# luigiba/OpenKEonSpark

Hardware: AMD Instinct MI355X
Metric: positive triples/sec (training step) (higher is better)
Workload: dtype f32

## Files before the change

### include/kge_mi355.h

```cpp
#ifndef KGE_MI355_H
#define KGE_MI355_H

#include <stddef.h>
#include <stdint.h>

#ifdef __cplusplus
extern "C" {
#endif

#ifndef INT
#define INT long
#endif
#ifndef REAL
#define REAL float
#endif

void setInPath(char *path);
void setOutPath(char *path);
void setWorkThreads(INT threads);
INT getWorkThreads(void);
void setBern(INT con);
void randReset(void);
void importTrainFiles(void);
INT getEntityTotal(void);
INT getRelationTotal(void);
INT getTripleTotal(void);
INT getTrainTotal(void);
INT getTrainTotal_(void);
INT getBatchTotal(void);
INT getTestTotal(void);
INT getValidTotal(void);
void sampling(INT *batch_h, INT *batch_t, INT *batch_r, REAL *batch_y, INT batchSize, INT negRate, INT negRelRate);

void importTestFiles(void);
void importTypeFiles(void);
void importOntologyFiles(void);
void getHeadBatch(INT index, INT *ph, INT *pt, INT *pr);
void getTailBatch(INT index, INT *ph, INT *pt, INT *pr);
INT *testHead(INT index, REAL *con);
INT *testTail(INT index, REAL *con);
void getTestBatch(INT *ph, INT *pt, INT *pr, INT *nh, INT *nt, INT *nr);
void getValidBatch(INT *ph, INT *pt, INT *pr, INT *nh, INT *nt, INT *nr);
void getBestThreshold(REAL *relThresh, REAL *score_pos, REAL *score_neg);
void test_triple_classification(REAL *relThresh, REAL *score_pos, REAL *score_neg, REAL *acc);
INT get_n_interval(INT r, REAL *score_pos, REAL *score_neg);
INT *get_TPFP(INT r, REAL *score_pos, REAL *score_neg, REAL *threshold, REAL *unused);

enum {
    KGE_OK = 0,
    KGE_NO_EVENT = 1,
    KGE_ERR_NO_DEVICE = -1,
    KGE_ERR_NO_DATASET = -2,
    KGE_ERR_BAD_ARG = -3,
    KGE_ERR_UNSUPPORTED = -4
};

enum { KGE_TRANSE = 0, KGE_TRANSH = 1, KGE_TRANSR = 2, KGE_TRANSD = 3 };

size_t kge_last_error(char *buf, size_t n);
void kge_clear_error(void);
int kge_device_available(void);
const char *kge_version(void);

int kge_set_option(const char *name, INT value);
int kge_last_kernel_ms(const char *name, float *ms);
int kge_kernel_ms_mean(const char *name, float *mean_ms, INT *launches);

int kge_import_train_arrays(INT ent_total, INT rel_total, INT n, const INT *h, const INT *t, const INT *r,
                            INT new_batch_total);

int64_t kge_index_copy(const char *what, void *dst, int64_t bytes);

int kge_get_stream_states(uint64_t *dst, INT n);
int kge_set_stream_states(const uint64_t *src, INT n);

int kge_sampling_device(int32_t *d_h, int32_t *d_t, int32_t *d_r, INT batchSize, INT negRate, INT negRelRate,
                        INT thread_lo, INT thread_hi, INT out_stride, INT *n_local, void *stream);

int kge_sampling_attach(int32_t *d_h, int32_t *d_t, int32_t *d_r, INT batchSize, INT negRate, INT negRelRate,
                        INT thread_lo, INT thread_hi, INT out_stride, INT *n_local, void *stream);
int kge_sampling_flush(void *stream);
INT kge_slice_positions(INT batchSize, INT thread_lo, INT thread_hi, INT *first_position);

typedef struct kge_model_desc {
    int32_t model;
    int32_t negative_rel;
    int64_t ent_total, rel_total;
    int32_t ent_dim, rel_dim;
    float margin;
    int32_t reserved;
} kge_model_desc;

#define KGE_MAX_TABLES 4
int kge_table_shape(const kge_model_desc *m, int table, int64_t *rows, int64_t *cols);

int kge_forward_backward(const kge_model_desc *m, const float *const tables[KGE_MAX_TABLES],
                         const int32_t *d_h, const int32_t *d_t, const int32_t *d_r,
                         INT n_pos, INT n_neg, INT stride, INT denom,
                         float *const grads[KGE_MAX_TABLES], float *d_loss, void *stream);

int kge_stream_wait_emit(void *stream);
int kge_forward_backward_sgd_rows(const kge_model_desc *m, float *const tables[KGE_MAX_TABLES], const int32_t *d_h, const int32_t *d_t,
                                  const int32_t *d_r, INT n_pos, INT n_neg, INT stride, INT denom, float lr, float *d_loss, void *stream);
int kge_sgd_rows_skipped(int32_t *n_negatives);
int kge_forward_backward_records(const kge_model_desc *m, const float *const tables[KGE_MAX_TABLES], const int32_t *d_h, const int32_t *d_t,
                                 const int32_t *d_r, INT n_pos, INT n_neg, INT stride, INT denom, INT n_pos_total, float *d_rec,
                                 int32_t *d_dst, INT rec_offset, INT rec_slice, float *d_loss, void *stream);
int kge_float_records_apply(const kge_model_desc *m, float *const tables[KGE_MAX_TABLES], const float *d_rec, int32_t *d_dst, INT n_records,
                            INT n_pos_total, INT n_neg, float lr, void *stream);
int kge_forward_backward_adam_rows(const kge_model_desc *m, float *const tables[KGE_MAX_TABLES], float *const adam_m[KGE_MAX_TABLES],
                                   float *const adam_v[KGE_MAX_TABLES], const int32_t *d_h, const int32_t *d_t, const int32_t *d_r, INT n_pos,
                                   INT n_neg, INT stride, INT denom, float lr_t, float beta1, float beta2, float eps, float *d_loss, void *stream);
int kge_float_records_apply_adam(const kge_model_desc *m, float *const tables[KGE_MAX_TABLES], float *const adam_m[KGE_MAX_TABLES],
                                 float *const adam_v[KGE_MAX_TABLES], const float *d_rec, int32_t *d_dst, INT n_records, INT n_pos_total,
                                 INT n_neg, float lr_t, float beta1, float beta2, float eps, void *stream);
int kge_pair_path_active(const kge_model_desc *m, INT n_pos, INT n_neg);
int kge_transr_group_layout_active(const kge_model_desc *m, INT n_pos, INT n_neg);

int kge_forward_backward_sampled(const kge_model_desc *m, const float *const tables[KGE_MAX_TABLES],
                                 const int32_t *d_h, const int32_t *d_t, const int32_t *d_r,
                                 INT n_pos, INT n_neg, INT stride, INT denom,
                                 float *const grads[KGE_MAX_TABLES], float *d_loss, void *stream);

int kge_loss_to_limbs(const float *d_loss, int32_t *d_limbs4, void *stream);
int kge_limbs_to_loss(const int32_t *d_limbs4, float *d_out, void *stream);
int kge_loss_limbs_target(int32_t *d_limbs4);

int kge_sgd_update(float *d_p, float *d_g, int64_t n, float lr, void *stream);
int kge_adam_update(float *d_p, float *d_m, float *d_v, float *d_g, int64_t n, float lr_t, float beta1,
                    float beta2, float eps, void *stream);

int kge_sgd_update_tables(int32_t n_tables, float *const d_p[KGE_MAX_TABLES], float *const d_g[KGE_MAX_TABLES],
                          const INT numel[KGE_MAX_TABLES], float lr, void *stream);
int kge_adam_update_tables(int32_t n_tables, float *const d_p[KGE_MAX_TABLES], float *const d_m[KGE_MAX_TABLES],
                           float *const d_v[KGE_MAX_TABLES], float *const d_g[KGE_MAX_TABLES], const INT numel[KGE_MAX_TABLES],
                           float lr_t, float beta1, float beta2, float eps, void *stream);

int kge_transe_counts_supported(const kge_model_desc *m, INT n_neg);
int kge_transe_forward_counts(const kge_model_desc *m, const float *d_ent, const float *d_rel, const int32_t *d_h,
                              const int32_t *d_t, const int32_t *d_r, INT n_pos, INT n_neg, INT stride, INT denom,
                              int32_t *d_counts, float *d_resid_ent, float *d_resid_rel, float *d_loss, void *stream);
int kge_transe_apply_counts(float *d_p, float *d_m, float *d_v, int32_t *d_counts, float *d_resid, int64_t rows, int32_t dim,
                            INT denom, int32_t adam, float lr, float beta1, float beta2, float eps, void *stream);
int kge_transe_train_step_counts(const kge_model_desc *m, float *const d_p[2], float *const d_m[2], float *const d_v[2], const int32_t *d_h,
                                 const int32_t *d_t, const int32_t *d_r, INT n_pos, INT n_neg, INT stride, INT denom, int32_t *d_counts,
                                 float *const d_resid[2], int32_t sampler_shaped, int32_t adam, float lr, float beta1, float beta2, float eps,
                                 float *d_loss, void *stream);
int kge_transe_apply_counts_tables(const kge_model_desc *m, float *const d_p[2], float *const d_m[2], float *const d_v[2],
                                   int32_t *d_counts, float *const d_resid[2], INT denom, int32_t adam, float lr, float beta1,
                                   float beta2, float eps, void *stream);

int kge_transe_apply_counts_range(const kge_model_desc *m, float *const d_p[2], float *const d_m[2], float *const d_v[2],
                                  int32_t *d_counts_chunk, float *const d_resid[2], INT row_lo, INT row_hi, INT denom, int32_t adam,
                                  float lr, float beta1, float beta2, float eps, void *stream);

INT kge_transe_record_dwords(const kge_model_desc *m);
int kge_transe_deferred_groups(int32_t *n_groups);
int kge_transe_step_scratch_read(int which, INT offset, INT count, void *host_out);
int kge_transe_emit_records(const kge_model_desc *m, const float *d_ent, const float *d_rel, const int32_t *d_h, const int32_t *d_t,
                            const int32_t *d_r, INT n_pos, INT n_neg, INT stride, INT denom, uint32_t *d_rec, int32_t *d_dst,
                            float *d_resid_ent, float *d_resid_rel, float *d_loss, void *stream);
int kge_transe_reduce_records(const kge_model_desc *m, const uint32_t *d_rec, int32_t *d_dst, INT n_records, int32_t *d_rows,
                              int32_t *d_row_counts, int32_t *d_n_rows, void *stream);
int kge_transe_apply_rows_sgd(const kge_model_desc *m, float *d_ent, float *d_rel, const int32_t *d_rows, const int32_t *d_row_counts,
                              const int32_t *d_n_rows, INT max_rows, INT denom, float lr, void *stream);
int kge_transe_lazy_row_live(const int32_t *d_row_live);
int kge_transe_apply_rows_adam_lazy(const kge_model_desc *m, float *d_ent, float *d_rel, float *d_m_ent, float *d_m_rel, float *d_v_ent,
                                    float *d_v_rel, const int32_t *d_rows, const int32_t *d_row_counts, const int32_t *d_n_rows,
                                    INT max_rows, INT denom, float lr_t, float beta1, float beta2, float eps, void *stream);
int kge_transe_reduce_apply_records_sgd(const kge_model_desc *m, const uint32_t *d_rec, int32_t *d_dst, INT n_records, float *d_ent,
                                        float *d_rel, int32_t *d_rows, int32_t *d_row_counts, int32_t *d_n_rows, INT denom, float lr,
                                        void *stream);

int kge_shard_requests(const int32_t *d_h, const int32_t *d_t, const int32_t *d_r, INT n_pos, INT n_neg, INT stride, int32_t *d_req,
                       void *stream);
int kge_shard_count(const int32_t *d_ids, INT n, INT chunk, INT n_owners, int32_t *d_counts, void *stream);
int kge_shard_scatter(const int32_t *d_ids, INT n, INT chunk, INT n_owners, const INT *h_counts, int32_t *d_cursor, int32_t *d_sorted,
                      int32_t *d_slot_of, void *stream);
int kge_shard_remap_batch(const int32_t *d_h, const int32_t *d_t, INT n_pos, INT n_neg, INT stride, const int32_t *d_slot_of, int32_t *d_h2,
                          int32_t *d_t2, void *stream);
int kge_shard_gather_rows(const float *d_table, const int32_t *d_ids, INT n, INT row_lo, INT rows, INT dim, float *d_out, void *stream);
int kge_shard_record_ids(const int32_t *d_dst, INT n_records, INT cache_rows, const int32_t *d_cache_ids, int32_t *d_ids, void *stream);
int kge_shard_pack_records(const uint32_t *d_rec, const int32_t *d_slot_of, INT n_records, INT dwords, uint32_t *d_out, void *stream);
int kge_shard_scatter_count_rows(const int32_t *d_rows, const int32_t *d_row_counts, const int32_t *d_n_rows, INT max_rows, INT base,
                                 INT rel_total, INT dim, int32_t *d_image, void *stream);
int kge_shard_relation_counts(const uint32_t *d_rec, const int32_t *d_dst, INT n_records, INT cache_rows, INT rel_total, INT dwords, INT dim,
                              int32_t *d_counts, void *stream);

int kge_train_steps_persistent(const kge_model_desc *m, float *const tables[KGE_MAX_TABLES], float *const grads[KGE_MAX_TABLES],
                               float *const adam_m[KGE_MAX_TABLES], float *const adam_v[KGE_MAX_TABLES], INT batchSize, INT negRate,
                               INT negRelRate, INT n_steps, int32_t adam, const float *h_lr, float beta1, float beta2, float eps,
                               float *d_losses, void *stream);
int kge_persistent_aborted(int32_t *flag);
int kge_persistent_trace(uint64_t *h_out, INT n_steps);

int kge_link_prediction(const kge_model_desc *m, const float *const tables[KGE_MAX_TABLES], INT first, INT count,
                        INT test_head, int64_t *h_out, void *stream);

int kge_link_prediction_range(const kge_model_desc *m, const float *const tables[KGE_MAX_TABLES], INT row_lo, INT rows,
                              const float *d_query_rows, INT first, INT count, INT test_head, int64_t *d_counts, int64_t *d_keys,
                              void *stream);
int kge_link_prediction_finish(INT first, INT count, INT test_head, const int64_t *d_counts, const int64_t *d_keys, int64_t *h_out,
                               void *stream);
int kge_test_entity_ids(INT first, INT count, int32_t *d_ids, void *stream);

int kge_rank_triples(const kge_model_desc *m, const float *const tables[KGE_MAX_TABLES], const int32_t *d_h, const int32_t *d_t,
                     const int32_t *d_r, INT n, INT test_head, int64_t *d_counts, void *stream);

#define KGE_TOPK_FILTERED 1
#define KGE_TOPK_TYPED 2
int kge_topk_entities(const kge_model_desc *m, const float *const tables[KGE_MAX_TABLES], const int32_t *d_fixed, const int32_t *d_rel,
                      const int32_t *d_head, INT n, INT k, INT flags, int32_t *d_ids, float *d_scores, void *stream);
#define KGE_TOPK_NO_KEY 0xFFFFFFFFFFFFFFFFull
int kge_topk_entities_range(const kge_model_desc *m, const float *const tables[KGE_MAX_TABLES], INT row_lo, INT rows,
                            const float *d_query_rows, const int32_t *d_fixed, const int32_t *d_rel, const int32_t *d_head, INT n,
                            INT k, INT flags, uint64_t *d_keys, void *stream);
int kge_topk_merge_keys(const uint64_t *d_keys, INT n, INT parts, INT k, int32_t *d_ids, float *d_scores, void *stream);

int kge_topk_relations(const kge_model_desc *m, const float *const tables[KGE_MAX_TABLES], const int32_t *d_h,
                       const int32_t *d_t, INT n, INT k, INT flags, int32_t *d_ids, float *d_scores, void *stream);
int kge_relation_prediction(const kge_model_desc *m, const float *const tables[KGE_MAX_TABLES], INT first, INT count,
                            int64_t *h_out, void *stream);
int kge_relation_prediction_rows(const kge_model_desc *m, const float *const tables[KGE_MAX_TABLES], const float *d_query_rows,
                                 INT first, INT count, int64_t *d_counts, void *stream);

int kge_tc_fit(const float *d_pos, const float *d_neg, INT n_valid, float *d_thresh, int32_t *d_n_interval, void *stream);
int kge_tc_apply(INT split, const float *d_thresh, const float *d_pos, const float *d_neg, INT n, int64_t *d_counts, int64_t *d_rel,
                 void *stream);

int kge_tc_roc(const float *d_vpos, const float *d_vneg, INT n_valid, INT split, const float *d_pos, const float *d_neg, INT n,
// ... 10 lines not shown
```

### openkeonspark_amd/Config.py

```python
import ctypes
import json
import os

import numpy as np

from . import _lib, shard_eval
from ._lib import KgeError


class Config(object):

    def __init__(self, cpp_lib_path=None, init_new_entities=False):
        self.init_new_entities = init_new_entities
        if init_new_entities == False:
            if cpp_lib_path is None:
                cpp_lib_path = _lib.LIB_PATH
            self.lib = _lib.load(os.path.abspath(cpp_lib_path))
            self.in_path = None
            self.out_path = None
            self.bern = 0
            self.hidden_size = 64
            self.ent_size = self.hidden_size
            self.rel_size = self.hidden_size
            self.train_times = 0
# ... 128 lines not shown

    def set_bern(self, bern):
        self.bern = bern

    def set_dimension(self, dim):
        self.hidden_size = dim
        self.ent_size = dim
        self.rel_size = dim

    def set_ent_dimension(self, dim):
        self.ent_size = dim

    def set_rel_dimension(self, dim):
        self.rel_size = dim

    def set_train_times(self, times):
        self.train_times = times

    def set_nbatches(self, nbatches):
        self.nbatches = nbatches

    def set_margin(self, margin):
        self.margin = margin

    def set_ent_neg_rate(self, rate):
        self.negative_ent = rate

    def set_rel_neg_rate(self, rate):
        self.negative_rel = rate

    def set_import_files(self, path):
        self.importName = path

    def set_export_files(self, path):
        self.exportName = path

    def set_work_threads(self, threads):
        self.workThreads = threads

    def set_model(self, model):
        self.model = model

    def sampling(self):
        self.lib.kge_clear_error()
        self.lib.sampling(self.batch_h_addr, self.batch_t_addr, self.batch_r_addr, self.batch_y_addr,
                          self.batch_size, self.negative_ent, self.negative_rel)
        _lib.raise_if_error(self.lib)

    def set_model_and_session(self, model):
        import torch
        self.model = model
        self._shard_plan = self._plan_entity_shard(model)
        self.trainModel = self.model(config=self, define=True)
        m = self.trainModel
        self._desc = m.descriptor()
        self._tables = [m.parameter_lists[n] for n in m.table_names]
        self._adam = self.opt_method in ("Adam", "adam")
        self._lazy_adam = self.opt_method in ("LazyAdam", "lazyadam", "lazy_adam")
        self._has_slots = self._adam or self._lazy_adam
        n_neg = self.negative_ent + self.negative_rel
        self.use_counts = bool(getattr(self, "use_counts", True)) and bool(
            self.lib.kge_transe_counts_supported(ctypes.byref(self._desc), n_neg))
        requested = getattr(self, "sparse_rows", None)
        table_bytes, sparse = self._wants_sparse_rows(n_neg)
        self.sparse_rows = (bool(sparse) or self._lazy_adam) and self.use_counts and not self._adam
        vector_model = m.model_id in (_lib.TRANSE, _lib.TRANSH, _lib.TRANSD)
        self.sparse_inplace = bool(not self.sparse_rows and vector_model and not self._adam and
                                   (self._lazy_adam or requested or (requested is None and table_bytes > (2 << 30))))
        if self._lazy_adam and not (self.sparse_rows or self.sparse_inplace):
            raise KgeError("LazyAdam (touched rows only, NON-PARITY) needs TransE, TransH or TransD: TransR's gradient is a whole "
                           "matrix per relation and has no record path")
        if requested and not (self.sparse_rows or self.sparse_inplace):
            raise KgeError("sparse_rows needs TransE / TransH / TransD with SGD or LazyAdam")
        self._grads = [] if (self.sparse_rows or self.sparse_inplace) else [torch.zeros_like(t) for t in self._tables]
        if self._has_slots:
            self._adam_m = [torch.zeros_like(t) for t in self._tables]
            self._adam_v = [torch.zeros_like(t) for t in self._tables]
            self._beta1_power = np.float32(self.adam_beta1)
            self._beta2_power = np.float32(self.adam_beta2)
        self._loss = torch.zeros(1, dtype=torch.float32, device=self.device)
        self._refresh_pointers()
        self._dist_ready = 0
        self._dev_batch = None
        self._dev_batch2 = None
        self._side_stream = None
        self._prefetched = None
        self.global_step = 0
        self._sparse_buf = None
        self.counts_min_records = int(getattr(self, "counts_min_records",
                                              os.environ.get("KGE_COUNTS_MIN_RECORDS", 1 << 16)))
        self.prefetch_sampling = getattr(self, "prefetch_sampling", None)
        self._prefetch_auto = self.prefetch_sampling is None
        if self._prefetch_auto:
            self.prefetch_sampling = self._prefetch_default()
        if self.use_counts and not self.sparse_rows:
            self._counts = torch.zeros((self.entTotal + self.relTotal, self.hidden_size), dtype=torch.int32,
                                       device=self.device)
        self._setup_partition()

    def _wants_sparse_rows(self, n_neg):
        table_bytes = (self.entTotal + self.relTotal) * self.hidden_size * 4
        sparse = getattr(self, "sparse_rows", None)
        if sparse is None:
            touched_bytes = self.batch_size * (3 + n_neg) * self.hidden_size * 4
            threshold = getattr(self, "sparse_threshold_bytes", None)
            if threshold is None:
                threshold = max(128 << 20, int(0.3 * touched_bytes))
            sparse = table_bytes > int(threshold)
        return table_bytes, sparse

    def _plan_entity_shard(self, model):
        try:
            import torch.distributed as dist
            if not (dist.is_available() and dist.is_initialized()):
                return None
            W, g = dist.get_world_size(), dist.get_rank()
        except Exception:
            return None
        if W <= 1 or W > 64 or self.hidden_size % 4:
            return None
        probe = model(config=self, define=False)
        if probe.model_id != _lib.TRANSE or self.opt_method in ("Adam", "adam"):
            return None
        n_neg = self.negative_ent + self.negative_rel
        desc = probe.descriptor()
        if not (bool(getattr(self, "use_counts", True)) and bool(self.lib.kge_transe_counts_supported(ctypes.byref(desc), n_neg))):
            return None
        lazy = self.opt_method in ("LazyAdam", "lazyadam", "lazy_adam")
        if not (bool(self._wants_sparse_rows(n_neg)[1]) or lazy):
            return None
        from .parallel import chunk_size
        chunk = chunk_size(self.entTotal, W)
        return dict(world=W, rank=g, chunk=chunk, lo=min(g * chunk, self.entTotal), hi=min((g + 1) * chunk, self.entTotal))

    def init_distributed(self, process_group=None):
        import torch.distributed as dist
        self._pg = process_group
        self.rank = dist.get_rank(process_group)
        self.world_size = dist.get_world_size(process_group)
        if self.trainModel is not None:
            self._setup_partition()
        if getattr(self, "_prefetch_auto", getattr(self, "prefetch_sampling", None) is None):
            self.prefetch_sampling = self._prefetch_default()

    def _prefetch_default(self):
        n_neg = self.negative_ent + self.negative_rel
        counts_path = bool(getattr(self, "use_counts", False)) and not getattr(self, "sparse_rows", False) and \
            self.batch_size * (3 + n_neg) >= int(getattr(self, "counts_min_records", 1 << 16)) * self.world_size
        pair_path = getattr(self, "_desc", None) is not None and \
            bool(self.lib.kge_pair_path_active(ctypes.byref(self._desc), max(self._n_local, 1) if hasattr(self, "_n_local") else self.batch_size, n_neg))
        transr = getattr(self, "trainModel", None) is not None and self.trainModel.model_id == _lib.TRANSR
        dense_one_gpu = not getattr(self, "sparse_rows", False) and not getattr(self, "sparse_inplace", False)
        return bool(self.world_size > 1 or counts_path or pair_path or transr or dense_one_gpu)

    @property
    def _dp(self):
        return self.world_size > 1 or bool(getattr(self, "force_data_parallel", False))

    def _setup_partition(self):
        from .parallel import thread_range
        lo, hi = thread_range(self.rank, self.world_size, self.workThreads)
        self._thread_lo, self._thread_hi = lo, hi
        first = ctypes.c_int64(0)
        self._n_local = self.lib.kge_slice_positions(self.batch_size, lo, hi, ctypes.byref(first))
        self._first_pos = first.value
        if self._dp and self.trainModel is not None and getattr(self, "_dist_ready", 0) != self.world_size:
# ... 48 lines not shown
            self._tables[i] = view
            self.trainModel.parameter_lists[name] = view
            setattr(self.trainModel, name, view)
            self._grads[i] = flat_g[offs[i]:offs[i] + numels[i]].view(shape)
            if self._adam:
                for flat, slots in ((flat_m, self._adam_m), (flat_v, self._adam_v)):
                    v = flat[offs[i]:offs[i] + numels[i]].view(shape)
                    v.copy_(slots[i])
                    slots[i] = v
        self._flat_p, self._flat_g, self._flat_m, self._flat_v = flat_p, flat_g, flat_m, flat_v
        self._chunk = chunk
        self._pieces = K
        seg, own = total // K, chunk // K
        self._piece_seg = [(k * seg, (k + 1) * seg) for k in range(K)]
        self._piece_own = [(k * seg + self.rank * own, k * seg + (self.rank + 1) * own) for k in range(K)]
        self._own_len = own
        self._grads_own = torch.zeros(chunk, dtype=torch.float32, device=dev)
        self._loss_tail = total - 1
        self._loss = flat_p[self._loss_tail:]
        if self.use_counts:
            rows_total = chunk_rows * W
            seg_r, own_r = rows_total // K, chunk_rows // K
            live = self.entTotal + self.relTotal
            self._counts = torch.zeros((rows_total, self.hidden_size), dtype=torch.int32, device=dev)
            self._counts_own = torch.zeros((chunk_rows, self.hidden_size), dtype=torch.int32, device=dev)
            self._piece_rows = [(min(k * seg_r + self.rank * own_r, live), min(k * seg_r + (self.rank + 1) * own_r, live)) for k in range(K)]
            self._own_rows_len = own_r
        self._opt_state_synced = True
        self._refresh_pointers()

    def _setup_shards(self):
        import torch
        from .parallel import chunk_size
        if self.hidden_size % 4:
            raise KgeError("the table-sharded sparse mode needs an embedding width that is a multiple of 4")
        if self.world_size > 64:
            raise KgeError("the table-sharded sparse mode supports up to 64 ranks")
        W, g, E, D = self.world_size, self.rank, self.entTotal, self.hidden_size
        chunk = chunk_size(E, W)
        lo, hi = min(g * chunk, E), min((g + 1) * chunk, E)
        if getattr(self, "_ent_is_shard", False):
            plan = self._shard_plan
            if (plan["world"], plan["rank"], plan["chunk"]) != (W, g, chunk) or self._tables[0].shape[0] != chunk:
                raise KgeError("the entity table was created as the shard of rank %d of %d, the process group has rank %d of %d"
                               % (plan["rank"], plan["world"], g, W))
            self._shard = dict(chunk=chunk, lo=lo, hi=hi)
            self._refresh_pointers()
            return
        full = self._tables[0]
        shard = torch.zeros((chunk, D), dtype=torch.float32, device=full.device)
        if hi > lo:
            shard[:hi - lo].copy_(full[lo:hi])
        self._tables[0] = shard
        self.trainModel.parameter_lists["ent_embeddings"] = shard
        self.trainModel.ent_embeddings = shard
        del full
        if self._lazy_adam:
            for slots in (self._adam_m, self._adam_v):
                old = slots[0]
                slots[0] = torch.zeros((chunk, D), dtype=torch.float32, device=shard.device)
                if hi > lo:
                    slots[0][:hi - lo].copy_(old[lo:hi])
                del old
        torch.cuda.empty_cache()
        self._shard = dict(chunk=chunk, lo=lo, hi=hi)
        self._refresh_pointers()

    def _stream(self):
        import torch
        if getattr(self, "_dev_index_of", None) != self.device:
            d = torch.device(self.device)
            self._dev_index = d.index if d.index is not None else torch.cuda.current_device()
            self._dev_index_of = self.device
        raw = getattr(torch._C, "_cuda_getCurrentRawStream", None)
        return ctypes.c_void_p(raw(self._dev_index) if raw is not None else torch.cuda.current_stream().cuda_stream)

    def _ensure_dev_batch(self, stride):
        import torch
        n = stride * (1 + self.negative_ent + self.negative_rel)
        if self._dev_batch is None or self._dev_batch.shape[2] != n:
            self._dev_batch = torch.zeros((2, 3, n), dtype=torch.int32, device=self.device)
        return self._dev_batch

    def sample_device(self, slot=0):
        stride = max(self._n_local, 1)
        buf = self._ensure_dev_batch(stride)[slot]
        nl = ctypes.c_int64(0)
        _lib.check(self.lib.kge_sampling_device(buf[0].data_ptr(), buf[1].data_ptr(), buf[2].data_ptr(),
                                                self.batch_size, self.negative_ent, self.negative_rel,
                                                self._thread_lo, self._thread_hi, stride, ctypes.byref(nl),
                                                self._stream()), self.lib)
        return buf, nl.value

    def _next_sampled_batch(self):
        import torch
        if self._side_stream is None:
            self._side_stream = torch.cuda.Stream()
            self._slot = 0
            self._prefetched = None
            self.lib.kge_set_option(b"record_emit_event", 1)
        if self._prefetched is None:
            dev, n_pos = self.sample_device(self._slot)
        else:
            dev, n_pos, ev = self._prefetched
            if ev is not None:
                torch.cuda.current_stream().wait_event(ev)
        return dev, n_pos

    def _attach_next_batch(self):
        stride = max(self._n_local, 1)
        self._slot ^= 1
        buf = self._ensure_dev_batch(stride)[self._slot]
        nl = ctypes.c_int64(0)
        _lib.check(self.lib.kge_sampling_attach(buf[0].data_ptr(), buf[1].data_ptr(), buf[2].data_ptr(), self.batch_size,
                                                self.negative_ent, self.negative_rel, self._thread_lo, self._thread_hi, stride,
                                                ctypes.byref(nl), self._stream()), self.lib)
        self._prefetched = (buf, nl.value, None)

    def _flush_next_batch(self):
        _lib.check(self.lib.kge_sampling_flush(self._stream()), self.lib)

    def _prefetch_next_batch(self, behind_emit=False):
        import torch
        main = torch.cuda.current_stream()
        done = None
        if not behind_emit:
            done = torch.cuda.Event()
            done.record(main)
        self._slot ^= 1
        with torch.cuda.stream(self._side_stream):
            if behind_emit:
                rc = _lib.check(self.lib.kge_stream_wait_emit(ctypes.c_void_p(self._side_stream.cuda_stream)), self.lib)
                if rc == _lib.NO_EVENT:
                    done = torch.cuda.Event()
                    done.record(main)
            if done is not None:
                self._side_stream.wait_event(done)
            dev, n_pos = self.sample_device(self._slot)
            ev = torch.cuda.Event()
            ev.record(self._side_stream)
        self._prefetched = (dev, n_pos, ev)

    def forward_backward(self, dev_batch, n_pos, stride, denom, sampler_shaped=False):
        fn = self.lib.kge_forward_backward_sampled if sampler_shaped else self.lib.kge_forward_backward
        _lib.check(fn(ctypes.byref(self._desc), self._tab_ptrs,
                                                 dev_batch[0].data_ptr(), dev_batch[1].data_ptr(),
                                                 dev_batch[2].data_ptr(), n_pos,
                                                 self.negative_ent + self.negative_rel, stride, denom,
                                                 self._grad_ptrs, self._loss.data_ptr(), self._stream()), self.lib)

    def _adam_lr_t(self):
        f = np.float32
        return f(f(self.alpha) * np.sqrt(f(1) - self._beta2_power, dtype=np.float32) / (f(1) - self._beta1_power))

    def _adam_advance(self):
        f = np.float32
        self._beta1_power = f(self._beta1_power * f(self.adam_beta1))
        self._beta2_power = f(self._beta2_power * f(self.adam_beta2))

    def apply_gradients(self, own=False, piece=0):
        st = self._stream()
        if own:
            lo, hi = self._piece_own[piece]
            n = hi - lo
            if hi > self._loss_tail:
                n -= 4
            p, g = self._flat_p.data_ptr() + 4 * lo, self._grads_own.data_ptr() + 4 * piece * self._own_len
            if self._adam:
                _lib.check(self.lib.kge_adam_update(p, self._flat_m.data_ptr() + 4 * lo, self._flat_v.data_ptr() + 4 * lo, g, n,
                                                    float(self._adam_lr_t()), self.adam_beta1, self.adam_beta2,
                                                    self.adam_epsilon, st), self.lib)
                self._opt_state_synced = False
            else:
                _lib.check(self.lib.kge_sgd_update(p, g, n, float(self.alpha), st), self.lib)
            return
        elif self._adam:
            _lib.check(self.lib.kge_adam_update_tables(len(self._tables), self._tab_ptrs, self._adam_m_ptrs, self._adam_v_ptrs,
                                                       self._grad_ptrs, self._numel, float(self._adam_lr_t()), self.adam_beta1,
                                                       self.adam_beta2, self.adam_epsilon, st), self.lib)
            self._adam_advance()
        else:
            _lib.check(self.lib.kge_sgd_update_tables(len(self._tables), self._tab_ptrs, self._grad_ptrs, self._numel,
                                                      float(self.alpha), st), self.lib)
        self.global_step += 1

    def _dp_exchange(self, image, own_image, apply_piece, counts):
        from .parallel import reduce_scatter_sum, all_gather_chunks
        st, W, K = self._stream(), self.world_size, self._pieces
        flat_img, flat_own = image.view(-1), own_image.view(-1)
        per_seg, per_own = flat_img.numel() // K, flat_own.numel() // K
        ride = flat_img.numel() >= 4 and (not counts or self.hidden_size >= 4)
        last = self.rank == W - 1
        nat = self._stream_rccl() if (K == 1 and ride) else None
        self.comm_fence("nat" if nat is not None else "pg")
        if nat is not None:
            if counts and not getattr(self, "_limbs_from_emit", False):
                _lib.check(self.lib.kge_loss_to_limbs(self._loss.data_ptr(), flat_img[flat_img.numel() - self.hidden_size:].data_ptr(), st), self.lib)
            elif not counts:
                flat_img[-1:].copy_(self._loss)
            nat.reduce_scatter_sum(flat_own, flat_img, st)
            if last:
                if counts:
                    _lib.check(self.lib.kge_limbs_to_loss(flat_own[flat_own.numel() - self.hidden_size:].data_ptr(), self._loss.data_ptr(), st), self.lib)
                else:
                    self._loss.copy_(flat_own[-1:])
            apply_piece(0)
            (slo, shi), (lo, hi) = self._piece_seg[0], self._piece_own[0]
            nat.all_gather_chunks(self._flat_p[slo:shi], self._flat_p[lo:hi], st)
            image.zero_()
            if self._adam:
                self._adam_advance()
            self.global_step += 1
            return
        if ride:
            if counts and not getattr(self, "_limbs_from_emit", False):
                _lib.check(self.lib.kge_loss_to_limbs(self._loss.data_ptr(), flat_img[flat_img.numel() - self.hidden_size:].data_ptr(), st), self.lib)
            else:
                flat_img[-1:].copy_(self._loss)
        rs = [reduce_scatter_sum(flat_own[k * per_own:(k + 1) * per_own], flat_img[k * per_seg:(k + 1) * per_seg], self._pg, async_op=True)
              for k in range(K)]
        if not ride:
            from .parallel import allreduce_sum
            allreduce_sum([self._loss], self._pg)
        ag = []
        for k in range(K):
            if rs[k] is not None:
                rs[k].wait()
            if ride and last and k == K - 1:
                if counts:
                    _lib.check(self.lib.kge_limbs_to_loss(flat_own[flat_own.numel() - self.hidden_size:].data_ptr(),
                                                          self._flat_p[self._loss_tail:].data_ptr(), st), self.lib)
                else:
                    self._loss.copy_(flat_own[-1:])
            apply_piece(k)
            (slo, shi), (lo, hi) = self._piece_seg[k], self._piece_own[k]
            ag.append(all_gather_chunks(self._flat_p[slo:shi], self._flat_p[lo:hi], self._pg, async_op=True))
        image.zero_()
        if self._adam:
            self._adam_advance()
        self.global_step += 1
        for w in ag:
            if w is not None:
                w.wait()

    def comm_fence(self, kind):
        last = getattr(self, "_last_comm", None)
        if last is not None and last != kind:
            import torch
            torch.cuda.synchronize(self.device)
        self._last_comm = kind

    def _stream_rccl(self):
        if getattr(self, "_nat_rccl", None) is None:
            import torch.distributed as dist
            want = getattr(self, "stream_rccl", os.environ.get("KGE_STREAM_RCCL", "1") != "0") and dist.is_initialized() and \
                dist.get_backend(self._pg) == "nccl"
            nat = False
            if want:
                import sys
                import torch
                from .parallel import StreamRccl
                self.comm_fence("pg")
                good = 0
                try:
                    nat = StreamRccl(self._pg)
                    torch.cuda.synchronize(self.device)
                    W, g, st = nat.world, nat.rank, self._stream()
                    src = torch.arange(4 * W, dtype=torch.int32, device=self.device) + g
                    own = torch.empty(4, dtype=torch.int32, device=self.device)
                    nat.reduce_scatter_sum(own, src, st)
                    full = torch.empty(4 * W, dtype=torch.int32, device=self.device)
                    full[4 * g:4 * g + 4] = own
                    nat.all_gather_chunks(full, full[4 * g:4 * g + 4], st)
                    torch.cuda.synchronize(self.device)
                    want_full = W * torch.arange(4 * W, dtype=torch.int32) + W * (W - 1) // 2
                    good = int(torch.equal(full.cpu(), want_full))
                    if not good:
                        print("StreamRccl probe gave wrong sums: collectives stay on the process group's stream", file=sys.stderr)
                except Exception as exc:
                    print("StreamRccl unavailable (%s): collectives stay on the process group's stream" % exc, file=sys.stderr)
                ok = torch.tensor([good], dtype=torch.int32, device=self.device)
                dist.all_reduce(ok, op=dist.ReduceOp.MIN, group=self._pg)
                if int(ok.item()) == 0:
                    if nat:
                        nat.close()
                    nat = False
            self._nat_rccl = nat
        return self._nat_rccl or None

    def sync_optimizer_state(self):
        if self._dp and self._adam and not self.sparse_rows and not getattr(self, "_opt_state_synced", True):
            from .parallel import all_gather_chunks
            self.comm_fence("pg")
            for (slo, shi), (lo, hi) in zip(self._piece_seg, self._piece_own):
                all_gather_chunks(self._flat_m[slo:shi], self._flat_m[lo:hi], self._pg)
                all_gather_chunks(self._flat_v[slo:shi], self._flat_v[lo:hi], self._pg)
            self._opt_state_synced = True

    def train_step(self, batch_h=None, batch_t=None, batch_r=None, batch_y=None, sync=True):
        import torch
        n_neg = self.negative_ent + self.negative_rel
        if getattr(self, "_ent_is_shard", False) and not hasattr(self, "_shard"):
            raise KgeError("the entity table was created as this rank's shard of a row-sharded table (the process belongs to a "
                           "torch.distributed world): call init_distributed() before training")
        if batch_h is None:
            dev, n_pos = self._next_sampled_batch() if self.prefetch_sampling else self.sample_device()
            stride = max(self._n_local, 1)
        else:
            if self._dp:
                raise KgeError("feeding a host batch is single-process only")
            host = np.stack([np.asarray(batch_h), np.asarray(batch_t), np.asarray(batch_r)]).astype(np.int32)
            self._check_ids(host)
            dev = torch.from_numpy(host).to(self.device)
            n_pos = host.shape[1] // (1 + n_neg)
            stride = n_pos
        denom = self.batch_size * n_neg if batch_h is None else n_pos * n_neg
        big = (self.batch_size if batch_h is None else n_pos) * (3 + n_neg) >= self.counts_min_records * self.world_size
        if self.sparse_inplace and self._dp:
            self._records_step(dev, n_pos, stride, denom)
            if batch_h is None and self.prefetch_sampling:
                self._prefetch_next_batch()
        elif self.sparse_inplace:
            if self._lazy_adam:
                _lib.check(self.lib.kge_forward_backward_adam_rows(
                    ctypes.byref(self._desc), self._tab_ptrs, self._adam_m_ptrs, self._adam_v_ptrs, dev[0].data_ptr(), dev[1].data_ptr(),
                    dev[2].data_ptr(), n_pos, n_neg, stride, denom, float(self._adam_lr_t()), self.adam_beta1, self.adam_beta2,
                    self.adam_epsilon, self._loss.data_ptr(), self._stream()), self.lib)
                self._adam_advance()
            else:
                _lib.check(self.lib.kge_forward_backward_sgd_rows(
                    ctypes.byref(self._desc), self._tab_ptrs, dev[0].data_ptr(), dev[1].data_ptr(), dev[2].data_ptr(), n_pos, n_neg,
                    stride, denom, float(self.alpha), self._loss.data_ptr(), self._stream()), self.lib)
            if batch_h is not None:
                skipped = ctypes.c_int32(0)
                _lib.check(self.lib.kge_sgd_rows_skipped(ctypes.byref(skipped)), self.lib)
                if skipped.value:
                    raise KgeError("sparse_rows: %d negatives are not single-slot corruptions of their positive and were left out "
                                   "of this step; train such batches with sparse_rows=False" % skipped.value)
            self.global_step += 1
            if batch_h is None and self.prefetch_sampling:
                self._prefetch_next_batch()
        elif self.sparse_rows:
            if self._dp:
                self._sharded_step(dev, n_pos, stride, denom)
            else:
                self._sparse_step(dev, n_pos, stride, denom, check_shape=batch_h is not None)
            if batch_h is None and self.prefetch_sampling:
                self._prefetch_next_batch()
        elif self.use_counts and big:
            ahead = batch_h is None and self.prefetch_sampling
            if ahead:
                self._attach_next_batch()
            self._limbs_from_emit = bool(self._dp and batch_h is None and self.hidden_size >= 4)
            target = self._counts.view(-1)[self._counts.numel() - self.hidden_size:].data_ptr() if self._limbs_from_emit else 0
            if target != getattr(self, "_limbs_target", 0):
                self.lib.kge_loss_limbs_target(ctypes.c_void_p(target) if target else None)
                self._limbs_target = target
            one_call = not self._dp and bool(getattr(self, "fused_counts", True))
            try:
                if one_call:
                    self.step_counts(dev, n_pos, stride, denom, sampler_shaped=batch_h is None)
                else:
                    self.forward_counts(dev, n_pos, stride, denom, sampler_shaped=batch_h is None)
            finally:
                if ahead:
                    self._flush_next_batch()
            if one_call:
                pass
            elif self._dp:
                self._dp_exchange(self._counts, self._counts_own, lambda k: self.apply_counts(denom, own=True, piece=k), counts=True)
                self.tables_changed()
            else:
                self.apply_counts(denom)
        else:
            ride = batch_h is None and self.prefetch_sampling and not self._dp
            if ride:
                self._attach_next_batch()
            try:
                self.forward_backward(dev, n_pos, stride, denom, sampler_shaped=batch_h is None)
            finally:
                if ride:
                    self._flush_next_batch()
            if batch_h is None and self.prefetch_sampling and not ride:
                self._prefetch_next_batch(behind_emit=bool(self.lib.kge_pair_path_active(ctypes.byref(self._desc), n_pos, n_neg)))
            if self._dp:
                self._dp_exchange(self._flat_g, self._grads_own, lambda k: self.apply_gradients(own=True, piece=k), counts=False)
            else:
                self.apply_gradients()
        self.trainModel.loss = self._loss
        return float(self._loss.item()) if sync else self._loss

    def persistent_supported(self):
        if self._dp or self.sparse_rows or self.sparse_inplace or self.hidden_size > 256:
            return False
        if self.trainModel.model_id not in (_lib.TRANSE, _lib.TRANSH, _lib.TRANSD):
            return False
        n_neg = self.negative_ent + self.negative_rel
        if self.use_counts and self.batch_size * (3 + n_neg) >= self.counts_min_records:
            return False
        slots = {_lib.TRANSE: 3 + n_neg, _lib.TRANSH: 4 + n_neg, _lib.TRANSD: 6 + 2 * n_neg}[self.trainModel.model_id]
        return self.batch_size * slots < int(getattr(self, "persistent_max_rows", 1 << 16))

    def persistent_preferred(self):
        return self.persistent_supported() and self.trainModel.model_id == _lib.TRANSE

    def train_steps(self, n_steps, persistent=None):
        import torch
        n_steps = int(n_steps)
        if n_steps <= 0:
            return np.zeros(0, np.float32)
        use = self.persistent_preferred() if persistent is None else bool(persistent)
        if use and not self.persistent_supported():
            raise KgeError("train_steps(persistent=True): this configuration has no persistent-launch path")
        if not use:
            out = [self.train_step(sync=False).clone() for _ in range(n_steps)]
            return torch.stack([o.reshape(()) for o in out]).cpu().numpy()
        if self._prefetched is not None:
            raise KgeError("train_steps: a batch was sampled ahead by train_step(); use one or the other in a run")
        f = np.float32
        lr = np.empty(n_steps, np.float32)
        powers = None
        if self._adam:
            saved = (self._beta1_power, self._beta2_power)
            for i in range(n_steps):
                lr[i] = self._adam_lr_t()
                self._adam_advance()
            powers = (self._beta1_power, self._beta2_power)
            self._beta1_power, self._beta2_power = saved
        else:
            lr[:] = f(self.alpha)
        losses = torch.empty(n_steps, dtype=torch.float32, device=self.device)
        _lib.check(self.lib.kge_train_steps_persistent(
            ctypes.byref(self._desc), self._tab_ptrs, self._grad_ptrs, self._adam_m_ptrs if self._adam else None,
            self._adam_v_ptrs if self._adam else None, self.batch_size, self.negative_ent, self.negative_rel, n_steps,
            1 if self._adam else 0, lr.ctypes.data, self.adam_beta1, self.adam_beta2, self.adam_epsilon, losses.data_ptr(),
            self._stream()), self.lib)
        out = losses.cpu().numpy()
        flag = ctypes.c_int32(0)
        _lib.check(self.lib.kge_persistent_aborted(ctypes.byref(flag)), self.lib)
        if flag.value:
            raise KgeError("persistent training launch aborted: a grid barrier did not complete (is another process holding "
                           "compute units of this GPU?); the tables are in an intermediate state")
        if powers is not None:
            self._beta1_power, self._beta2_power = powers
        self.global_step += n_steps
        self._loss.copy_(losses[-1:])
# ... 148 lines not shown
        _lib.check(L.kge_shard_gather_rows(self._tables[0].data_ptr(), b["recv_ids"].data_ptr(), n_recv, sh["lo"], chunk, D,
                                           b["rows_out"].data_ptr(), st), L)
        par.all_to_all_rows(b["cache"], b["rows_out"], send, recv, pg, max_rows=gmax)
        if self._dev_batch2 is None or self._dev_batch2.shape != dev_batch.shape:
            self._dev_batch2 = torch.zeros_like(dev_batch)
        h2, t2 = self._dev_batch2[0], self._dev_batch2[1]
        _lib.check(L.kge_shard_remap_batch(h.data_ptr(), t.data_ptr(), n_pos, n_neg, bstride, b["slot_of"].data_ptr(), h2.data_ptr(),
                                           t2.data_ptr(), st), L)
        desc2 = self._desc_with(ent_total=max(n_send, 1))
        _lib.check(L.kge_transe_emit_records(ctypes.byref(desc2), b["cache"].data_ptr(), self._tables[1].data_ptr(), h2.data_ptr(),
                                             t2.data_ptr(), r.data_ptr(), n_pos, n_neg, bstride, denom, b["rec"].data_ptr(),
                                             b["dst"].data_ptr(), None, None, self._loss.data_ptr(), st), L)
        b["rel_counts"].zero_()
        if self._lazy_adam:
            if "rel_live" not in b:
                b["rel_live"] = torch.zeros(self.relTotal + 1, dtype=torch.int32, device=self.device)
            b["rel_live"].zero_()
            if n_pos > 0:
                d = b["dst"][2 * n_pos:(M if self.negative_rel > 0 else 3 * n_pos)]
                idx = torch.where(d >= int(desc2.ent_total), d - int(desc2.ent_total), torch.full_like(d, self.relTotal))
                b["rel_live"].index_fill_(0, idx.long(), 1)
        if D % 4 == 0 and self.negative_rel == 0 and n_pos > 0:
            cap = min(n_pos, self.relTotal) + 8
            if b.get("relc_cap", 0) < cap:
                b.update(relc_cap=cap, relc_rows=torch.empty(cap, dtype=torch.int32, device=self.device),
                         relc_counts=torch.empty((cap, D), dtype=torch.int32, device=self.device))
            _lib.check(L.kge_transe_reduce_records(ctypes.byref(desc2), b["rec"][2 * n_pos:3 * n_pos].data_ptr(),
                                                   b["dst"][2 * n_pos:3 * n_pos].data_ptr(), n_pos, b["relc_rows"].data_ptr(),
                                                   b["relc_counts"].data_ptr(), b["n_rows"].data_ptr(), st), L)
            _lib.check(L.kge_shard_scatter_count_rows(b["relc_rows"].data_ptr(), b["relc_counts"].data_ptr(), b["n_rows"].data_ptr(),
                                                      cap, desc2.ent_total, self.relTotal, D, b["rel_counts"].data_ptr(), st), L)
        else:
            _lib.check(L.kge_shard_relation_counts(b["rec"].data_ptr(), b["dst"].data_ptr(), M, desc2.ent_total, self.relTotal, dw, D,
                                                   b["rel_counts"].data_ptr(), st), L)
        if self._lazy_adam:
            par.allreduce_sum([b["rel_counts"], self._loss, b["rel_live"]], pg)
        else:
            par.allreduce_sum([b["rel_counts"], self._loss], pg)
        _lib.check(L.kge_shard_record_ids(b["dst"].data_ptr(), M, n_send, b["send_ids"].data_ptr(), b["ids2"].data_ptr(), st), L)
        _lib.check(L.kge_shard_count(b["ids2"].data_ptr(), M, chunk, W, b["counts"].data_ptr(), st), L)
        send2, recv2, gmax2 = par.exchange_counts_max(b["counts"], pg)
        h_counts2 = (ctypes.c_int64 * W)(*send2)
        _lib.check(L.kge_shard_scatter(b["ids2"].data_ptr(), M, chunk, W, h_counts2, b["cursor"].data_ptr(), b["send_rows2"].data_ptr(),
                                       b["slot_of2"].data_ptr(), st), L)
        _lib.check(L.kge_shard_pack_records(b["rec"].data_ptr(), b["slot_of2"].data_ptr(), M, dw, b["send_rec"].data_ptr(), st), L)
        n_recv2 = sum(recv2)
        b = self._shard_buffers(M, n_recv, n_recv2)
        par.all_to_all_rows(b["recv_rows2"], b["send_rows2"], recv2, send2, pg, max_rows=gmax2)
        par.all_to_all_rows(b["recv_rec"], b["send_rec"], recv2, send2, pg, max_rows=gmax2)
        if n_recv2 > 0:
            b["recv_rows2"][:n_recv2].sub_(sh["lo"])
            desc3 = self._desc_with(ent_total=chunk, rel_total=0)
            if self._lazy_adam:
                _lib.check(L.kge_transe_reduce_records(ctypes.byref(desc3), b["recv_rec"].data_ptr(), b["recv_rows2"].data_ptr(), n_recv2,
                                                       b["rows"].data_ptr(), b["row_counts"].data_ptr(), b["n_rows"].data_ptr(), st), L)
                _lib.check(L.kge_transe_apply_rows_adam_lazy(
                    ctypes.byref(desc3), self._tables[0].data_ptr(), self._tables[1].data_ptr(), self._adam_m[0].data_ptr(),
                    self._adam_m[1].data_ptr(), self._adam_v[0].data_ptr(), self._adam_v[1].data_ptr(), b["rows"].data_ptr(),
                    b["row_counts"].data_ptr(), b["n_rows"].data_ptr(), n_recv2, denom, float(self._adam_lr_t()), self.adam_beta1,
                    self.adam_beta2, self.adam_epsilon, st), L)
            else:
                _lib.check(L.kge_transe_reduce_apply_records_sgd(
                    ctypes.byref(desc3), b["recv_rec"].data_ptr(), b["recv_rows2"].data_ptr(), n_recv2, self._tables[0].data_ptr(),
                    self._tables[1].data_ptr(), b["rows"].data_ptr(), b["row_counts"].data_ptr(), b["n_rows"].data_ptr(), denom,
                    float(self.alpha), st), L)
        if self._lazy_adam:
            _lib.check(L.kge_transe_lazy_row_live(b["rel_live"].data_ptr()), L)
            _lib.check(L.kge_transe_apply_rows_adam_lazy(
                ctypes.byref(self._desc), self._tables[0].data_ptr(), self._tables[1].data_ptr(), self._adam_m[0].data_ptr(),
                self._adam_m[1].data_ptr(), self._adam_v[0].data_ptr(), self._adam_v[1].data_ptr(), b["rel_rows"].data_ptr(),
                b["rel_counts"].data_ptr(), b["n_rel"].data_ptr(), self.relTotal, denom, float(self._adam_lr_t()), self.adam_beta1,
                self.adam_beta2, self.adam_epsilon, st), L)
            self._adam_advance()
        else:
            _lib.check(L.kge_transe_apply_rows_sgd(ctypes.byref(self._desc), self._tables[0].data_ptr(), self._tables[1].data_ptr(),
                                                   b["rel_rows"].data_ptr(), b["rel_counts"].data_ptr(), b["n_rel"].data_ptr(),
                                                   self.relTotal, denom, float(self.alpha), st), L)
        self.global_step += 1

    def sparse_row_gradients(self):
        n = int(self._sparse_buf["n_rows"].item())
        return self._sparse_buf["rows"][:n], self._sparse_buf["row_counts"][:n]

    def forward_counts(self, dev_batch, n_pos, stride, denom, sampler_shaped=False):
        resid = (None, None) if sampler_shaped else (self._grads[0].data_ptr(), self._grads[1].data_ptr())
        _lib.check(self.lib.kge_transe_forward_counts(
            ctypes.byref(self._desc), self._tables[0].data_ptr(), self._tables[1].data_ptr(),
            dev_batch[0].data_ptr(), dev_batch[1].data_ptr(), dev_batch[2].data_ptr(), n_pos,
            self.negative_ent + self.negative_rel, stride, denom, self._counts.data_ptr(),
            resid[0], resid[1], self._loss.data_ptr(), self._stream()), self.lib)

    def step_counts(self, dev_batch, n_pos, stride, denom, sampler_shaped=False):
        lr = float(self._adam_lr_t()) if self._adam else float(self.alpha)
        _lib.check(self.lib.kge_transe_train_step_counts(
            ctypes.byref(self._desc), self._tab_ptrs, self._adam_m_ptrs if self._adam else None, self._adam_v_ptrs if self._adam else None,
            dev_batch[0].data_ptr(), dev_batch[1].data_ptr(), dev_batch[2].data_ptr(), n_pos, self.negative_ent + self.negative_rel,
            stride, denom, self._counts.data_ptr(), self._grad_ptrs, 1 if sampler_shaped else 0, 1 if self._adam else 0, lr,
            self.adam_beta1, self.adam_beta2, self.adam_epsilon, self._loss.data_ptr(), self._stream()), self.lib)
        if self._adam:
            self._adam_advance()
        self.global_step += 1

    def apply_counts(self, denom, own=False, piece=0):
        st = self._stream()
        lr = float(self._adam_lr_t()) if self._adam else float(self.alpha)
        m_ptrs = self._adam_m_ptrs if self._adam else None
        v_ptrs = self._adam_v_ptrs if self._adam else None
        if own:
            row_lo, row_hi = self._piece_rows[piece]
            if row_hi > row_lo:
                img = self._counts_own.data_ptr() + 4 * piece * self._own_rows_len * self.hidden_size
                _lib.check(self.lib.kge_transe_apply_counts_range(
                    ctypes.byref(self._desc), self._tab_ptrs, m_ptrs, v_ptrs, img, self._grad_ptrs,
                    row_lo, row_hi, denom, 1 if self._adam else 0, lr, self.adam_beta1, self.adam_beta2,
                    self.adam_epsilon, st), self.lib)
            self._opt_state_synced = not self._adam
            return
        else:
            _lib.check(self.lib.kge_transe_apply_counts_tables(
                ctypes.byref(self._desc), self._tab_ptrs, m_ptrs, v_ptrs, self._counts.data_ptr(), self._grad_ptrs, denom,
                1 if self._adam else 0, lr, self.adam_beta1, self.adam_beta2, self.adam_epsilon, st), self.lib)
        if self._adam:
            self._adam_advance()
        self.global_step += 1

    def _check_ids(self, host):
        if host.shape[1] == 0:
            return
        if host.min() < 0 or host[:2].max() >= self.entTotal or host[2].max() >= self.relTotal:
            raise KgeError("entity / relation id out of range in the supplied batch")

    def test_step(self, test_h, test_t, test_r):
        import torch
        host = np.stack([np.asarray(test_h), np.asarray(test_t), np.asarray(test_r)]).astype(np.int32)
        self._check_ids(host)
        if self._sharded("ent_embeddings"):
            return shard_eval.test_step(self, host)
        dev = torch.from_numpy(host).to(self.device)
        out = torch.empty(host.shape[1], dtype=torch.float32, device=self.device)
        _lib.check(self.lib.kge_predict(ctypes.byref(self._desc), self._tab_ptrs, dev[0].data_ptr(), dev[1].data_ptr(),
                                        dev[2].data_ptr(), host.shape[1], out.data_ptr(), self._stream()), self.lib)
        self.trainModel.predict = out
        return out.cpu().numpy()

    def _tc_buffers(self, prefix, n):
        for side in ("pos", "neg"):
            for col in ("h", "t", "r"):
                arr = np.zeros(n, dtype=np.int64)
                setattr(self, "%s_%s_%s" % (prefix, side, col), arr)
                setattr(self, "%s_%s_%s_addr" % (prefix, side, col), arr.ctypes.data)

    def init_valid_triple_classification(self):
        self.lib.kge_clear_error()
        self.lib.importTestFiles()
        self.lib.importTypeFiles()
        _lib.raise_if_error(self.lib)
        self.testTotal = self.lib.getTestTotal()
        self.validTotal = self.lib.getValidTotal()
        self._tc_buffers("valid", self.validTotal)
        self.relThresh = np.zeros(self.lib.getRelationTotal(), dtype=np.float32)
        self.relThresh_addr = self.relThresh.ctypes.data
        self.acc = np.zeros(1, dtype=np.float32)
        self.acc_addr = self.acc.ctypes.data

    def init_triple_classification(self):
        self.init_valid_triple_classification()
        self._tc_buffers("test", self.testTotal)

    def _fit_thresholds(self):
        L = self.lib
        L.getValidBatch(self.valid_pos_h_addr, self.valid_pos_t_addr, self.valid_pos_r_addr,
                        self.valid_neg_h_addr, self.valid_neg_t_addr, self.valid_neg_r_addr)
        _lib.raise_if_error(L)
        res_pos = np.ascontiguousarray(self.test_step(self.valid_pos_h, self.valid_pos_t, self.valid_pos_r).reshape(-1), dtype=np.float32)
        res_neg = np.ascontiguousarray(self.test_step(self.valid_neg_h, self.valid_neg_t, self.valid_neg_r).reshape(-1), dtype=np.float32)
        L.getBestThreshold(self.relThresh_addr, res_pos.ctypes.data, res_neg.ctypes.data)

    def _test_triple_classification_host(self):
        if not hasattr(self, "test_pos_h"):
# ... 571 lines not shown
```

### openkeonspark_amd/_lib.py

```python
import ctypes
import os

_HERE = os.path.dirname(os.path.abspath(__file__))
LIB_PATH = os.path.join(_HERE, "csrc", "libkge_mi355.so")

TRANSE, TRANSH, TRANSR, TRANSD = 0, 1, 2, 3
NO_EVENT = 1
KGE_MAX_TABLES = 4
TOPK_FILTERED, TOPK_TYPED = 1, 2
TOPK_MAX_K = 1024


class KgeError(RuntimeError):
    pass


class ModelDesc(ctypes.Structure):
    _fields_ = [("model", ctypes.c_int32), ("negative_rel", ctypes.c_int32),
                ("ent_total", ctypes.c_int64), ("rel_total", ctypes.c_int64),
                ("ent_dim", ctypes.c_int32), ("rel_dim", ctypes.c_int32),
                ("margin", ctypes.c_float), ("reserved", ctypes.c_int32)]


def _declare(L):
    vp, i64, i32, f32 = ctypes.c_void_p, ctypes.c_int64, ctypes.c_int32, ctypes.c_float
    L.setInPath.argtypes = [ctypes.c_char_p]
    L.setOutPath.argtypes = [ctypes.c_char_p]
    L.setWorkThreads.argtypes = [i64]
    L.getWorkThreads.restype = i64
    L.setBern.argtypes = [i64]
    for fn in ("getEntityTotal", "getRelationTotal", "getTripleTotal", "getTrainTotal", "getTrainTotal_",
               "getBatchTotal", "getTestTotal", "getValidTotal"):
        getattr(L, fn).restype = i64
    L.sampling.argtypes = [vp, vp, vp, vp, i64, i64, i64]
    L.getTailBatch.argtypes = [i64, vp, vp, vp]
    L.getHeadBatch.argtypes = [i64, vp, vp, vp]
    L.testTail.argtypes = [i64, vp]
    L.testTail.restype = ctypes.POINTER(ctypes.c_int64 * 8)
    L.testHead.argtypes = [i64, vp]
    L.testHead.restype = ctypes.POINTER(ctypes.c_int64 * 8)
    L.kge_link_prediction.argtypes = [ctypes.POINTER(ModelDesc), ctypes.POINTER(vp), i64, i64, i64, vp, vp]
    L.getValidBatch.argtypes = [vp] * 6
    L.getTestBatch.argtypes = [vp] * 6
    L.getBestThreshold.argtypes = [vp] * 3
    L.test_triple_classification.argtypes = [vp] * 4
    L.kge_last_error.restype = ctypes.c_size_t
    L.kge_last_error.argtypes = [ctypes.c_char_p, ctypes.c_size_t]
    L.kge_device_available.restype = ctypes.c_int
    L.kge_version.restype = ctypes.c_char_p
    L.kge_import_train_arrays.argtypes = [i64, i64, i64, vp, vp, vp, i64]
    L.kge_set_option.argtypes = [ctypes.c_char_p, i64]
    L.kge_last_kernel_ms.argtypes = [ctypes.c_char_p, ctypes.POINTER(ctypes.c_float)]
    L.kge_kernel_ms_mean.argtypes = [ctypes.c_char_p, ctypes.POINTER(ctypes.c_float), ctypes.POINTER(i64)]
    L.kge_index_copy.restype = i64
    L.kge_index_copy.argtypes = [ctypes.c_char_p, vp, i64]
    L.kge_get_stream_states.argtypes = [vp, i64]
    L.kge_set_stream_states.argtypes = [vp, i64]
    L.kge_sampling_device.argtypes = [vp, vp, vp, i64, i64, i64, i64, i64, i64, ctypes.POINTER(i64), vp]
    L.kge_sampling_attach.argtypes = [vp, vp, vp, i64, i64, i64, i64, i64, i64, ctypes.POINTER(i64), vp]
    L.kge_sampling_flush.argtypes = [vp]
    L.kge_slice_positions.restype = i64
    L.kge_slice_positions.argtypes = [i64, i64, i64, ctypes.POINTER(i64)]
    L.kge_table_shape.argtypes = [ctypes.POINTER(ModelDesc), ctypes.c_int, ctypes.POINTER(i64), ctypes.POINTER(i64)]
    tabs = ctypes.POINTER(vp)
    L.kge_forward_backward.argtypes = [ctypes.POINTER(ModelDesc), tabs, vp, vp, vp, i64, i64, i64, i64, tabs, vp, vp]
    L.kge_stream_wait_emit.argtypes = [vp]
    L.kge_pair_path_active.argtypes = [ctypes.POINTER(ModelDesc), i64, i64]
    L.kge_transr_group_layout_active.argtypes = [ctypes.POINTER(ModelDesc), i64, i64]
    L.kge_loss_limbs_target.argtypes = [vp]
    L.kge_forward_backward_sgd_rows.argtypes = [ctypes.POINTER(ModelDesc), tabs, vp, vp, vp, i64, i64, i64, i64, f32, vp, vp]
    L.kge_forward_backward_records.argtypes = [ctypes.POINTER(ModelDesc), tabs, vp, vp, vp, i64, i64, i64, i64, i64, vp, vp, i64, i64, vp, vp]
    L.kge_float_records_apply.argtypes = [ctypes.POINTER(ModelDesc), tabs, vp, vp, i64, i64, i64, f32, vp]
    L.kge_forward_backward_adam_rows.argtypes = [ctypes.POINTER(ModelDesc), tabs, tabs, tabs, vp, vp, vp, i64, i64, i64, i64, f32, f32, f32, f32, vp, vp]
    L.kge_float_records_apply_adam.argtypes = [ctypes.POINTER(ModelDesc), tabs, tabs, tabs, vp, vp, i64, i64, i64, f32, f32, f32, f32, vp]
    L.kge_forward_backward_sampled.argtypes = [ctypes.POINTER(ModelDesc), tabs, vp, vp, vp, i64, i64, i64, i64, tabs, vp, vp]
    L.kge_loss_to_limbs.argtypes = [vp, vp, vp]
    L.kge_limbs_to_loss.argtypes = [vp, vp, vp]
    L.kge_sgd_update.argtypes = [vp, vp, i64, f32, vp]
    L.kge_adam_update.argtypes = [vp, vp, vp, vp, i64, f32, f32, f32, f32, vp]
    L.kge_sgd_update_tables.argtypes = [i32, vp, vp, vp, f32, vp]
    L.kge_adam_update_tables.argtypes = [i32, vp, vp, vp, vp, vp, f32, f32, f32, f32, vp]
    L.kge_predict.argtypes = [ctypes.POINTER(ModelDesc), tabs, vp, vp, vp, i64, vp, vp]
    L.kge_rank_triples.argtypes = [ctypes.POINTER(ModelDesc), tabs, vp, vp, vp, i64, i64, vp, vp]
    L.kge_topk_entities.argtypes = [ctypes.POINTER(ModelDesc), tabs, vp, vp, vp, i64, i64, i64, vp, vp, vp]
    L.kge_topk_entities_range.argtypes = [ctypes.POINTER(ModelDesc), tabs, i64, i64, vp, vp, vp, vp, i64, i64, i64, vp, vp]
    L.kge_topk_merge_keys.argtypes = [vp, i64, i64, i64, vp, vp, vp]
    L.kge_topk_relations.argtypes = [ctypes.POINTER(ModelDesc), tabs, vp, vp, i64, i64, i64, vp, vp, vp]
    L.kge_relation_prediction.argtypes = [ctypes.POINTER(ModelDesc), tabs, i64, i64, vp, vp]
    L.kge_relation_prediction_rows.argtypes = [ctypes.POINTER(ModelDesc), tabs, vp, i64, i64, vp, vp]
    L.kge_link_prediction_range.argtypes = [ctypes.POINTER(ModelDesc), tabs, i64, i64, vp, i64, i64, i64, vp, vp, vp]
    L.kge_link_prediction_finish.argtypes = [i64, i64, i64, vp, vp, vp, vp]
    L.kge_tc_fit.argtypes = [vp, vp, i64, vp, vp, vp]
    L.kge_tc_apply.argtypes = [i64, vp, vp, vp, i64, vp, vp, vp]
    L.kge_tc_roc.argtypes = [vp, vp, i64, i64, vp, vp, i64, vp, vp, i64, vp, vp]
    L.kge_test_entity_ids.argtypes = [i64, i64, vp, vp]
    L.kge_transe_counts_supported.argtypes = [ctypes.POINTER(ModelDesc), i64]
    L.kge_transe_forward_counts.argtypes = [ctypes.POINTER(ModelDesc), vp, vp, vp, vp, vp, i64, i64, i64, i64, vp, vp, vp, vp, vp]
    L.kge_transe_apply_counts.argtypes = [vp, vp, vp, vp, vp, i64, i32, i64, i32, f32, f32, f32, f32, vp]
    L.kge_transe_deferred_groups.argtypes = [ctypes.POINTER(ctypes.c_int32)]
    L.kge_transe_step_scratch_read.argtypes = [ctypes.c_int, i64, i64, vp]
    L.kge_transe_apply_counts_tables.argtypes = [ctypes.POINTER(ModelDesc), vp, vp, vp, vp, vp, i64, i32, f32, f32, f32, f32, vp]
    L.kge_transe_train_step_counts.argtypes = [ctypes.POINTER(ModelDesc), vp, vp, vp, vp, vp, vp, i64, i64, i64, i64, vp, vp, i32, i32,
                                               f32, f32, f32, f32, vp, vp]
    L.kge_transe_lazy_row_live.argtypes = [vp]
    L.kge_transe_record_dwords.restype = i64
    L.kge_transe_record_dwords.argtypes = [ctypes.POINTER(ModelDesc)]
    L.kge_transe_emit_records.argtypes = [ctypes.POINTER(ModelDesc), vp, vp, vp, vp, vp, i64, i64, i64, i64, vp, vp, vp, vp, vp, vp]
    L.kge_transe_reduce_records.argtypes = [ctypes.POINTER(ModelDesc), vp, vp, i64, vp, vp, vp, vp]
    L.kge_transe_apply_rows_sgd.argtypes = [ctypes.POINTER(ModelDesc), vp, vp, vp, vp, vp, i64, i64, f32, vp]
    L.kge_transe_apply_rows_adam_lazy.argtypes = [ctypes.POINTER(ModelDesc), vp, vp, vp, vp, vp, vp, vp, vp, vp, i64, i64, f32, f32, f32, f32, vp]
    L.kge_transe_reduce_apply_records_sgd.argtypes = [ctypes.POINTER(ModelDesc), vp, vp, i64, vp, vp, vp, vp, vp, i64, f32, vp]
    L.kge_transe_apply_counts_range.argtypes = [ctypes.POINTER(ModelDesc), vp, vp, vp, vp, vp, i64, i64, i64, i32, f32, f32, f32, f32, vp]
    L.kge_shard_requests.argtypes = [vp, vp, vp, i64, i64, i64, vp, vp]
    L.kge_shard_count.argtypes = [vp, i64, i64, i64, vp, vp]
    L.kge_shard_scatter.argtypes = [vp, i64, i64, i64, vp, vp, vp, vp, vp]
    L.kge_shard_remap_batch.argtypes = [vp, vp, i64, i64, i64, vp, vp, vp, vp]
    L.kge_shard_gather_rows.argtypes = [vp, vp, i64, i64, i64, i64, vp, vp]
    L.kge_shard_record_ids.argtypes = [vp, i64, i64, vp, vp, vp]
    L.kge_shard_pack_records.argtypes = [vp, vp, i64, i64, vp, vp]
    L.kge_shard_relation_counts.argtypes = [vp, vp, i64, i64, i64, i64, i64, vp, vp]
    L.kge_shard_scatter_count_rows.argtypes = [vp, vp, vp, i64, i64, i64, i64, vp, vp]
    L.kge_train_steps_persistent.argtypes = [ctypes.POINTER(ModelDesc), vp, vp, vp, vp, i64, i64, i64, i64, i32, vp, f32, f32, f32, vp, vp]
    L.kge_persistent_aborted.argtypes = [ctypes.POINTER(ctypes.c_int32)]
    L.kge_persistent_trace.argtypes = [vp, i64]
    return L


def load(path=None):
    path = path or LIB_PATH
    try:
        import torch
    except ImportError:
        pass
    if not os.path.exists(path):
        raise ImportError(
            "%s not found: build it first (python -c 'import __graft_entry__ as g; g.build()' or "
            "make -C openkeonspark_amd/csrc).  There is no CPU fallback." % path)
    return _declare(ctypes.CDLL(path))


_LIB = None


def lib():
    global _LIB
    if _LIB is None:
        _LIB = load()
    return _LIB


def last_error(L=None):
    L = L or lib()
    buf = ctypes.create_string_buffer(1024)
    L.kge_last_error(buf, 1024)
    return buf.value.decode(errors="replace")


def check(rc, L=None):
    if rc is not None and rc < 0:
        raise KgeError("kge_mi355 error %d: %s" % (rc, last_error(L)))
    return rc


def raise_if_error(L=None):
    L = L or lib()
    msg = last_error(L)
    if msg:
        L.kge_clear_error()
        raise KgeError(msg)


def table_ptrs(ptrs):
    arr = (ctypes.c_void_p * KGE_MAX_TABLES)()
    for i, p in enumerate(ptrs):
        arr[i] = p
    return arr
```

### openkeonspark_amd/csrc/abi.hip

```cpp
#include <cstdio>
#include <cstring>
#include <iostream>

#include "engine.hpp"

namespace kge {

Engine &engine() {
    static Engine e;
    return e;
}

void set_error(const std::string &msg) {
    engine().last_error = msg;
    std::fprintf(stderr, "[kge_mi355] error: %s\n", msg.c_str());
}

int fail(int code, const std::string &msg) {
    set_error(msg);
    return code;
}

int hip_check(hipError_t e, const char *what) {
    if (e == hipSuccess) return KGE_OK;
// ... 12 lines not shown
}

template <typename T>
static int upload(T *&dst, const void *src, size_t count, const char *what) {
    if (dst) { (void)hipFree(dst); dst = nullptr; }
    size_t bytes = sizeof(T) * (count ? count : 1);
    int rc = hip_check(hipMalloc(&dst, bytes), what);
    if (rc) return rc;
    if (count) rc = hip_check(hipMemcpy(dst, src, sizeof(T) * count, hipMemcpyHostToDevice), what);
    return rc;
}

int ensure_device_index() {
    Engine &e = engine();
    if (!e.index.loaded) return fail(KGE_ERR_NO_DATASET, "no training set imported (importTrainFiles / kge_import_train_arrays)");
    if (!device_ok()) return fail(KGE_ERR_NO_DEVICE, "no usable HIP device: the sampler has no CPU fallback");
    int rc = KGE_OK;
    if (!e.dev.uploaded) {
        const KgIndex &ix = e.index;
        if ((rc = upload(e.dev.pos, ix.pos.data(), ix.pos.size(), "upload pos"))) return rc;
        if ((rc = upload(e.dev.grp, ix.grp.data(), ix.grp.size(), "upload grp"))) return rc;
        if ((rc = upload(e.dev.ht, ix.ht.data(), ix.ht.size(), "upload ht"))) return rc;
        if ((rc = upload(e.dev.tails_hr, ix.tails_hr.data(), ix.tails_hr.size(), "upload tails"))) return rc;
        if ((rc = upload(e.dev.heads_tr, ix.heads_tr.data(), ix.heads_tr.size(), "upload heads"))) return rc;
        if ((rc = upload(e.dev.rels_ht, ix.rels_ht.data(), ix.rels_ht.size(), "upload rels"))) return rc;
        if ((rc = upload(e.dev.bern_prob, ix.bern_prob.data(), ix.bern_prob.size(), "upload bern"))) return rc;
        e.dev.uploaded = true;
    }
    if ((int64_t)e.streams.size() != e.work_threads) {
        e.streams.assign((size_t)e.work_threads, 0);
        e.dev.streams_sync = 0;
    }
    if (e.dev.streams_sync == 0) {
        if (e.dev.streams_cap < e.work_threads) {
            uint64_t *base = e.dev.streams < e.dev.streams_next ? e.dev.streams : e.dev.streams_next;
            if (base) (void)hipFree(base);
            e.dev.streams = e.dev.streams_next = nullptr;
            if ((rc = hip_check(hipMalloc(&e.dev.streams, sizeof(uint64_t) * 2 * (size_t)e.work_threads), "alloc streams"))) return rc;
            e.dev.streams_next = e.dev.streams + e.work_threads;
            e.dev.streams_cap = e.work_threads;
        }
        if ((rc = hip_check(hipMemcpy(e.dev.streams, e.streams.data(), sizeof(uint64_t) * (size_t)e.work_threads,
                                      hipMemcpyHostToDevice), "upload streams"))) return rc;
        e.dev.streams_sync = 1;
    }
    return KGE_OK;
}

static int pull_streams() {
    Engine &e = engine();
    { int rc = flush_attached_sampler(nullptr); if (rc) return rc; }
    if (e.dev.streams_sync == 2) {
        int rc = hip_check(hipMemcpy(e.streams.data(), e.dev.streams, sizeof(uint64_t) * e.streams.size(),
                                     hipMemcpyDeviceToHost), "download streams");
        if (rc) return rc;
        e.dev.streams_sync = 1;
    }
    return KGE_OK;
}

static void adopt_index(KgIndex &&ix) {
    Engine &e = engine();
    e.index = std::move(ix);
    e.dev.uploaded = false;
}

static std::string build_and_adopt(int64_t E, int64_t R, int64_t nb, int64_t n, const int64_t *h, const int64_t *t, const int64_t *r) {
    Engine &e = engine();
    if (device_ok()) { (void)flush_attached_sampler(nullptr); (void)hipDeviceSynchronize(); }
    if (e.index_device_min >= 0 && n >= e.index_device_min && device_ok() && device_index_build_supported(E, R, n)) {
        KgIndex ix;
        std::string err = build_index_device(ix, e.dev, E, R, nb, n, h, t, r);
        if (!err.empty()) { e.dev.uploaded = false; return err; }
        e.index = std::move(ix);
        return "";
    }
    KgIndex ix;
    std::string err = build_index(ix, E, R, nb, n, h, t, r);
    if (!err.empty()) return err;
    adopt_index(std::move(ix));
    return "";
}

}

using namespace kge;

extern "C" {

void setInPath(char *path) {
    engine().in_path = path ? path : "";
    std::printf("Input Files Path : %s\n", engine().in_path.c_str());
}

void setOutPath(char *path) {
    engine().out_path = path ? path : "";
    std::printf("Output Files Path : %s\n", engine().out_path.c_str());
}

void setWorkThreads(INT threads) { engine().work_threads = threads < 1 ? 1 : threads; }
INT getWorkThreads(void) { return engine().work_threads; }
void setBern(INT con) { engine().bern = con; }

void randReset(void) {
    Engine &e = engine();
    e.streams.resize((size_t)e.work_threads);
    for (auto &s : e.streams) s = (uint64_t)(int64_t)e.libc.next();
    e.dev.streams_sync = 0;
}

void importTrainFiles(void) {
    Engine &e = engine();
    std::printf("The toolkit is importing datasets.\n");
    int64_t E = 0, R = 0, nb = 0;
    std::vector<int64_t> h, t, r;
    std::string err = load_openke_dir(e.in_path, E, R, nb, h, t, r);
    if (!err.empty()) {
        std::cout << err << std::endl;
        set_error(err);
        return;
    }
    std::printf("The total of relations is %ld.\n", (long)R);
    std::printf("The total of entities is %ld.\n", (long)E);
    if (nb > 0) std::printf("The total number of new batch triples is: %ld\n", (long)nb);
    std::printf("The total of train triples is %ld.\n", (long)h.size());
    err = build_and_adopt(E, R, nb, (int64_t)h.size(), h.data(), t.data(), r.data());
    if (!err.empty()) { set_error(err); return; }
    std::fflush(stdout);
}

INT getEntityTotal(void) { return engine().index.ent_total; }
INT getRelationTotal(void) { return engine().index.rel_total; }
INT kge_eval_test_total(void); INT kge_eval_valid_total(void); INT kge_eval_triple_total(void);
INT getTripleTotal(void) { return kge_eval_triple_total(); }
INT getTrainTotal(void) { return engine().index.train_uniq; }
INT getTrainTotal_(void) { return engine().index.train_dup; }
INT getBatchTotal(void) { return engine().index.new_batch; }
INT getTestTotal(void) { return kge_eval_test_total(); }
INT getValidTotal(void) { return kge_eval_valid_total(); }

void sampling(INT *batch_h, INT *batch_t, INT *batch_r, REAL *batch_y, INT batchSize, INT negRate, INT negRelRate) {
    Engine &e = engine();
    if (ensure_device_index()) return;
    if (batchSize <= 0 || negRate < 0 || negRelRate < 0) { set_error("sampling: bad sizes"); return; }
    const int64_t total = batchSize * (1 + negRate + negRelRate);
    if (e.dev.stage_cap < total) {
        if (e.dev.stage_i32) (void)hipFree(e.dev.stage_i32);
        if (e.dev.stage_i64) (void)hipFree(e.dev.stage_i64);
        e.dev.stage_i32 = nullptr; e.dev.stage_i64 = nullptr; e.dev.stage_cap = 0;
        if (hip_check(hipMalloc(&e.dev.stage_i32, sizeof(int32_t) * 3 * (size_t)total), "alloc stage")) return;
        if (hip_check(hipMalloc(&e.dev.stage_i64, (sizeof(int64_t) * 3 + sizeof(float)) * (size_t)total), "alloc stage")) return;
        e.dev.stage_cap = total;
    }
    int32_t *s = e.dev.stage_i32;
    if (launch_sampler(s, s + total, s + 2 * total, batchSize, negRate, negRelRate, 0, e.work_threads, batchSize, nullptr, nullptr)) return;
    if (launch_widen(s, e.dev.stage_i64, batchSize, total, nullptr)) return;
    const int64_t *w = e.dev.stage_i64;
    if (hip_check(hipMemcpy(batch_h, w, sizeof(int64_t) * total, hipMemcpyDeviceToHost), "copy batch_h")) return;
    if (hip_check(hipMemcpy(batch_t, w + total, sizeof(int64_t) * total, hipMemcpyDeviceToHost), "copy batch_t")) return;
    if (hip_check(hipMemcpy(batch_r, w + 2 * total, sizeof(int64_t) * total, hipMemcpyDeviceToHost), "copy batch_r")) return;
    hip_check(hipMemcpy(batch_y, w + 3 * total, sizeof(float) * total, hipMemcpyDeviceToHost), "copy batch_y");
}

size_t kge_last_error(char *buf, size_t n) {
    const std::string &s = engine().last_error;
    if (buf && n) {
        size_t k = s.size() < n - 1 ? s.size() : n - 1;
        std::memcpy(buf, s.data(), k);
        buf[k] = 0;
    }
    return s.size();
}

void kge_clear_error(void) { engine().last_error.clear(); }
int kge_device_available(void) { return device_ok() ? 1 : 0; }
const char *kge_version(void) { return "kge_mi355 0.1 (gfx950)"; }

int kge_set_option(const char *name, INT value) {
    std::string n = name ? name : "";
    if (n == "counts_force_sort") { engine().counts_force_sort = value != 0; return KGE_OK; }
    if (n == "ride_shares") { engine().ride_shares = (int)value; return KGE_OK; }
    if (n == "transr_bf16x3") { engine().transr_bf16x3 = value != 0; return KGE_OK; }
    if (n == "transr_groups") { engine().transr_groups = (int)value; return KGE_OK; }
    if (n == "transr_fuse_vec") { engine().transr_fuse_vec = value != 0; return KGE_OK; }
    if (n == "counts_fused") { engine().counts_fused = value != 0; return KGE_OK; }
    if (n == "counts_fused_diag") { engine().counts_fused_diag = (int)value; return KGE_OK; }
    if (n == "counts_fused_cap") { engine().counts_fused_cap = value > 0 ? (int)value : 0; return KGE_OK; }
    if (n == "inv_table_max_bytes") { engine().inv_table_max_bytes = value; return KGE_OK; }
    if (n == "tables_changed") { tables_written(); return KGE_OK; }
    if (n == "counts_krel") { int k = 1; while (k * 2 <= value && k < 64) k *= 2; engine().counts_krel = k; return KGE_OK; }
    if (n == "inv_carry") { engine().inv_carry = value != 0; tables_written(); return KGE_OK; }
    if (n == "emit_rounds") { engine().emit_rounds = value != 0; return KGE_OK; }
    if (n == "float_records") { engine().float_records = value != 0; return KGE_OK; }
    if (n == "float_records_min") { engine().float_records_min = value; return KGE_OK; }
    if (n == "index_device_min") { engine().index_device_min = value; return KGE_OK; }
    if (n == "hub_copies") { engine().hub_copies = value != 0; return KGE_OK; }
    if (n == "pair_counts") { engine().pair_counts = value != 0; return KGE_OK; }
    if (n == "record_emit_event") { engine().record_emit_event = value != 0; return KGE_OK; }
    if (n == "transr_dgrad_records") { engine().transr_dgrad_records = value != 0; return KGE_OK; }
    if (n == "transr_dgrad_records_min") { engine().transr_dgrad_records_min = value; return KGE_OK; }
    if (n == "transr_lean") { engine().transr_lean = value != 0; return KGE_OK; }
    if (n == "pair_counts_min_neg") { engine().pair_counts_min_neg = (int)value; return KGE_OK; }
    if (n == "topk_table_max_bytes") { engine().topk_table_max_bytes = value; return KGE_OK; }
    if (n == "relpred_chunk_bytes") { engine().relpred_chunk_bytes = value; return KGE_OK; }
    if (n == "lp_v1") { engine().lp_v1 = value != 0; return KGE_OK; }
    if (n == "rank_slices") { engine().rank_slices = value > 0 ? (int)value : 0; return KGE_OK; }
    if (n == "transr_v1") { engine().transr_v1 = (int)value; return KGE_OK; }
    if (n == "time_emit") { engine().time_emit = value > 0 ? (int)value : 0; if (value > 0) { engine().emit_launches = 0; engine().emit_seen = 0; } return KGE_OK; }
    if (n == "fb_occ4") { engine().fb_occ4 = value != 0; return KGE_OK; }
    if (n == "persist_ahead") { engine().persist_ahead = value != 0; return KGE_OK; }
    if (n == "persist_touch") { engine().persist_touch = value != 0; return KGE_OK; }
    if (n == "persist_trace") { engine().persist_trace = value != 0; return KGE_OK; }
    if (n == "persist_threads") { engine().persist_threads = value == 1024 ? 1024 : 512; return KGE_OK; }
    if (n == "libc_rand_restart") { engine().libc = LibcRand(); return KGE_OK; }
    return fail(KGE_ERR_BAD_ARG, "kge_set_option: unknown option " + n);
}

int kge_last_kernel_ms(const char *name, float *ms) {
    Engine &e = engine();
    std::string n = name ? name : "";
    if (n != "transe_emit" || !ms) return fail(KGE_ERR_BAD_ARG, "kge_last_kernel_ms: unknown kernel " + n);
    if (e.emit_launches <= 0) return fail(KGE_ERR_BAD_ARG, "kge_last_kernel_ms: enable option time_emit and run a step first");
    const int slot = (int)((e.emit_launches - 1) % Engine::kEmitRing);
    if (hip_check(hipEventSynchronize(e.ev_emit1[slot]), "event sync")) return KGE_ERR_NO_DEVICE;
    return hip_check(hipEventElapsedTime(ms, e.ev_emit0[slot], e.ev_emit1[slot]), "event elapsed");
}

int kge_kernel_ms_mean(const char *name, float *mean_ms, INT *launches) {
    Engine &e = engine();
    std::string n = name ? name : "";
    if (n != "transe_emit" || !mean_ms) return fail(KGE_ERR_BAD_ARG, "kge_kernel_ms_mean: unknown kernel " + n);
    const long long have = e.emit_launches < Engine::kEmitRing ? e.emit_launches : (long long)Engine::kEmitRing;
    if (have <= 0) return fail(KGE_ERR_BAD_ARG, "kge_kernel_ms_mean: enable option time_emit and run steps first");
    double sum = 0.0;
    for (long long i = 0; i < have; i++) {
        const int slot = (int)((e.emit_launches - 1 - i) % Engine::kEmitRing);
        float ms = 0.f;
        if (hip_check(hipEventSynchronize(e.ev_emit1[slot]), "event sync")) return KGE_ERR_NO_DEVICE;
        if (hip_check(hipEventElapsedTime(&ms, e.ev_emit0[slot], e.ev_emit1[slot]), "event elapsed")) return KGE_ERR_NO_DEVICE;
        sum += ms;
    }
    *mean_ms = (float)(sum / (double)have);
    if (launches) *launches = have;
    return KGE_OK;
}

int kge_import_train_arrays(INT ent_total, INT rel_total, INT n, const INT *h, const INT *t, const INT *r,
                            INT new_batch_total) {
    std::string err = build_and_adopt(ent_total, rel_total, new_batch_total, n, (const int64_t *)h, (const int64_t *)t,
                                      (const int64_t *)r);
    if (!err.empty()) return fail(KGE_ERR_BAD_ARG, err);
    return KGE_OK;
}

int64_t kge_index_copy(const char *what, void *dst, int64_t bytes) {
    const KgIndex &ix = engine().index;
    if (!ix.loaded) return fail(KGE_ERR_NO_DATASET, "kge_index_copy: no dataset");
    const void *src = nullptr;
    int64_t have = 0;
    std::string w = what ? what : "";
#define KGE_ARR(name, vec) if (w == name) { src = (vec).data(); have = (int64_t)((vec).size() * sizeof((vec)[0])); }
    KGE_ARR("tails_hr", ix.tails_hr) KGE_ARR("heads_tr", ix.heads_tr) KGE_ARR("rels_ht", ix.rels_ht)
    KGE_ARR("pos", ix.pos) KGE_ARR("grp", ix.grp) KGE_ARR("ht", ix.ht)
    KGE_ARR("left_mean", ix.left_mean) KGE_ARR("right_mean", ix.right_mean) KGE_ARR("bern_prob", ix.bern_prob)
#undef KGE_ARR
    if (!src && have == 0 && w != "tails_hr" && w != "heads_tr" && w != "rels_ht" && w != "pos" && w != "grp" && w != "ht" &&
        w != "left_mean" && w != "right_mean" && w != "bern_prob")
        return fail(KGE_ERR_BAD_ARG, "kge_index_copy: unknown array " + w);
    if (dst && bytes > 0 && have > 0) std::memcpy(dst, src, (size_t)(bytes < have ? bytes : have));
    return have;
}

int kge_get_stream_states(uint64_t *dst, INT n) {
    Engine &e = engine();
    int rc = pull_streams();
    if (rc) return rc;
    for (INT i = 0; i < n && i < (INT)e.streams.size(); i++) dst[i] = e.streams[(size_t)i];
    return KGE_OK;
}

int kge_set_stream_states(const uint64_t *src, INT n) {
    Engine &e = engine();
    if (n != e.work_threads) return fail(KGE_ERR_BAD_ARG, "kge_set_stream_states: n must equal workThreads");
    if (e.dev.streams && device_ok()) { (void)flush_attached_sampler(nullptr); (void)hipDeviceSynchronize(); }
    e.streams.assign(src, src + n);
    e.dev.streams_sync = 0;
    return KGE_OK;
}

INT kge_slice_positions(INT batchSize, INT thread_lo, INT thread_hi, INT *first_position) {
    const int64_t W = engine().work_threads;
    if (batchSize <= 0 || thread_lo < 0 || thread_hi > W || thread_lo >= thread_hi) {
        if (first_position) *first_position = 0;
        return 0;
    }
    int64_t lo, hi, tmp;
    thread_slice(batchSize, W, thread_lo, lo, tmp);
    thread_slice(batchSize, W, thread_hi - 1, tmp, hi);
    if (first_position) *first_position = lo;
    return hi - lo;
}

int kge_sampling_attach(int32_t *d_h, int32_t *d_t, int32_t *d_r, INT batchSize, INT negRate, INT negRelRate,
                        INT thread_lo, INT thread_hi, INT out_stride, INT *n_local, void *stream) {
    int64_t nl = 0;
    int rc = attach_sampler(d_h, d_t, d_r, batchSize, negRate, negRelRate, thread_lo, thread_hi, out_stride, &nl, (hipStream_t)stream);
    if (n_local) *n_local = nl;
    return rc;
}

int kge_sampling_flush(void *stream) { return flush_attached_sampler((hipStream_t)stream); }

int kge_sampling_device(int32_t *d_h, int32_t *d_t, int32_t *d_r, INT batchSize, INT negRate, INT negRelRate,
                        INT thread_lo, INT thread_hi, INT out_stride, INT *n_local, void *stream) {
    int64_t nl = 0;
    int rc = launch_sampler(d_h, d_t, d_r, batchSize, negRate, negRelRate, thread_lo, thread_hi, out_stride, &nl,
                            (hipStream_t)stream);
    if (n_local) *n_local = nl;
    return rc;
}

int kge_table_shape(const kge_model_desc *m, int table, int64_t *rows, int64_t *cols) {
    if (!m || !rows || !cols) return KGE_ERR_BAD_ARG;
    *rows = 0; *cols = 0;
    switch (table) {
        case 0: *rows = m->ent_total; *cols = m->ent_dim; break;
        case 1: *rows = m->rel_total; *cols = m->rel_dim; break;
        case 2:
            if (m->model == KGE_TRANSH || m->model == KGE_TRANSD) { *rows = m->rel_total; *cols = m->rel_dim; }
            if (m->model == KGE_TRANSR) { *rows = m->rel_total; *cols = (int64_t)m->ent_dim * m->rel_dim; }
            break;
        case 3:
            if (m->model == KGE_TRANSD) { *rows = m->ent_total; *cols = m->ent_dim; }
            break;
        default: return KGE_ERR_BAD_ARG;
    }
    return KGE_OK;
}

int kge_forward_backward(const kge_model_desc *m, const float *const tables[KGE_MAX_TABLES], const int32_t *d_h,
                         const int32_t *d_t, const int32_t *d_r, INT n_pos, INT n_neg, INT stride, INT denom,
                         float *const grads[KGE_MAX_TABLES], float *d_loss, void *stream) {
    if (!m || !tables || !grads || !d_loss) return fail(KGE_ERR_BAD_ARG, "kge_forward_backward: null argument");
    return launch_forward_backward(*m, tables, d_h, d_t, d_r, n_pos, n_neg, stride, denom, grads, d_loss, (hipStream_t)stream, false);
}

int kge_forward_backward_sgd_rows(const kge_model_desc *m, float *const tables[KGE_MAX_TABLES], const int32_t *d_h, const int32_t *d_t,
                                  const int32_t *d_r, INT n_pos, INT n_neg, INT stride, INT denom, float lr, float *d_loss, void *stream) {
    if (!m || !tables || !d_loss) return fail(KGE_ERR_BAD_ARG, "kge_forward_backward_sgd_rows: null argument");
    if (!(lr > 0.f)) return fail(KGE_ERR_BAD_ARG, "kge_forward_backward_sgd_rows: learning rate must be positive");
    return launch_forward_backward(*m, tables, d_h, d_t, d_r, n_pos, n_neg, stride, denom, tables, d_loss, (hipStream_t)stream, false, lr);
}

int kge_forward_backward_records(const kge_model_desc *m, const float *const tables[KGE_MAX_TABLES], const int32_t *d_h, const int32_t *d_t,
                                 const int32_t *d_r, INT n_pos, INT n_neg, INT stride, INT denom, INT n_pos_total, float *d_rec,
                                 int32_t *d_dst, INT rec_offset, INT rec_slice, float *d_loss, void *stream) {
    if (!m || !tables || !d_loss) return fail(KGE_ERR_BAD_ARG, "kge_forward_backward_records: null argument");
    return launch_forward_backward_records(*m, tables, d_h, d_t, d_r, n_pos, n_neg, stride, denom, n_pos_total, d_rec, d_dst, rec_offset,
                                           rec_slice, d_loss, (hipStream_t)stream);
}

int kge_float_records_apply(const kge_model_desc *m, float *const tables[KGE_MAX_TABLES], const float *d_rec, int32_t *d_dst, INT n_records,
                            INT n_pos_total, INT n_neg, float lr, void *stream) {
    if (!m || !tables) return fail(KGE_ERR_BAD_ARG, "kge_float_records_apply: null argument");
    return launch_float_records_apply(*m, tables, d_rec, d_dst, n_records, n_pos_total, n_neg, lr, (hipStream_t)stream);
}

static bool adam_rows_of(const kge_model_desc &m, float *const tables[KGE_MAX_TABLES], float *const adam_m[KGE_MAX_TABLES],
                         float *const adam_v[KGE_MAX_TABLES], float lr_t, float beta1, float beta2, float eps, AdamRows &ad) {
    ad = {};
    for (int t = 0; t < 4; t++) {
        if (!tables[t]) continue;
        if (!adam_m[t] || !adam_v[t]) return false;
        ad.m[t] = adam_m[t]; ad.v[t] = adam_v[t];
    }
    ad.lr_t = lr_t; ad.b1 = beta1; ad.b2 = beta2; ad.eps = eps;
    return true;
}

int kge_forward_backward_adam_rows(const kge_model_desc *m, float *const tables[KGE_MAX_TABLES], float *const adam_m[KGE_MAX_TABLES],
                                   float *const adam_v[KGE_MAX_TABLES], const int32_t *d_h, const int32_t *d_t, const int32_t *d_r, INT n_pos,
                                   INT n_neg, INT stride, INT denom, float lr_t, float beta1, float beta2, float eps, float *d_loss, void *stream) {
    if (!m || !tables || !adam_m || !adam_v || !d_loss) return fail(KGE_ERR_BAD_ARG, "kge_forward_backward_adam_rows: null argument");
    if (m->model == KGE_TRANSR) return fail(KGE_ERR_UNSUPPORTED, "lazy Adam on the touched rows: TransE / TransH / TransD only");
    AdamRows ad;
    if (!adam_rows_of(*m, tables, adam_m, adam_v, lr_t, beta1, beta2, eps, ad))
        return fail(KGE_ERR_BAD_ARG, "kge_forward_backward_adam_rows: every table needs its two moment tables");
    return launch_forward_backward(*m, tables, d_h, d_t, d_r, n_pos, n_neg, stride, denom, tables, d_loss, (hipStream_t)stream, false, 0.f, &ad);
}

int kge_float_records_apply_adam(const kge_model_desc *m, float *const tables[KGE_MAX_TABLES], float *const adam_m[KGE_MAX_TABLES],
                                 float *const adam_v[KGE_MAX_TABLES], const float *d_rec, int32_t *d_dst, INT n_records, INT n_pos_total,
                                 INT n_neg, float lr_t, float beta1, float beta2, float eps, void *stream) {
    if (!m || !tables || !adam_m || !adam_v) return fail(KGE_ERR_BAD_ARG, "kge_float_records_apply_adam: null argument");
    AdamRows ad;
    if (!adam_rows_of(*m, tables, adam_m, adam_v, lr_t, beta1, beta2, eps, ad))
        return fail(KGE_ERR_BAD_ARG, "kge_float_records_apply_adam: every table needs its two moment tables");
    return launch_float_records_apply_adam(*m, tables, ad, d_rec, d_dst, n_records, n_pos_total, n_neg, (hipStream_t)stream);
}

// ... 62 lines not shown
```

### openkeonspark_amd/csrc/engine.hpp

```cpp
#pragma once
#include <hip/hip_runtime.h>

#include <cstdint>
#include <mutex>
#include <string>
#include <vector>

#include "../../include/kge_mi355.h"
#include "kg_index.hpp"

namespace kge {

struct DeviceIndex {
    bool uploaded = false;
    int4 *pos = nullptr;
    int4 *grp = nullptr;
    int2 *ht = nullptr;
    int32_t *tails_hr = nullptr, *heads_tr = nullptr, *rels_ht = nullptr;
    float *bern_prob = nullptr;
    uint64_t *streams = nullptr;
    uint64_t *streams_next = nullptr;
    int64_t streams_cap = 0;
    int streams_sync = 0;
    int32_t *stage_i32 = nullptr;
    int64_t *stage_i64 = nullptr;
    int64_t stage_cap = 0;
    float *loss_partials = nullptr;
    unsigned *loss_ticket = nullptr;
};

struct Engine {
    std::mutex mu;
    std::string in_path = "../data/FB15K/";
    std::string out_path = "../data/FB15K/";
    int64_t work_threads = 1;
    int64_t bern = 0;
    KgIndex index;
    LibcRand libc;
    std::vector<uint64_t> streams;
    LcgJumpTable jump = make_jump_table();
    DeviceIndex dev;
    std::string last_error;
    int device_state = 0;
    int record_emit_event = 0;
    hipEvent_t emit_done = nullptr;
    unsigned long long emit_seq = 0, emit_waited = 0;
    int time_emit = 0;
    static constexpr int kEmitRing = 512;
    hipEvent_t ev_emit0[kEmitRing] = {}, ev_emit1[kEmitRing] = {};
    long long emit_launches = 0;
    long long emit_seen = 0;
    float *inv_norm = nullptr;
    int64_t inv_cap = 0;
    const float *inv_for_ent = nullptr, *inv_for_rel = nullptr;
    int inv_valid = 0;
    int32_t *loss_limbs = nullptr;
    int counts_krel = 4;
    int inv_carry = 1;
    int emit_rounds = 1;
    int64_t inv_table_max_bytes = int64_t(256) << 20;
    int float_records = 1;
    int64_t float_records_min = 1 << 16;
    int64_t index_device_min = int64_t(1) << 22;
    int transr_dgrad_records = 1;
    int64_t transr_dgrad_records_min = 1 << 15;
    int transr_bf16x3 = 1;
    int transr_groups = 1;
    int transr_fuse_vec = 1;
    int transr_lean = 1;
    int pair_counts = 1;
    int pair_counts_min_neg = 0;
    int hub_copies = 1;
    int64_t topk_table_max_bytes = int64_t(1) << 30;
    int64_t relpred_chunk_bytes = int64_t(256) << 20;
    int lp_v1 = 0;
    int rank_slices = 0;
    int transr_v1 = 0;
    int fb_occ4 = 1;
    int persist_ahead = 1;
    int persist_touch = 0;
    int persist_trace = 0;
    int persist_threads = 512;
    int counts_force_sort = 0;
    int ride_shares = 100 << 8;
    int counts_fused = 1;
    int counts_fused_diag = 0;
    int counts_fused_cap = 0;
};

Engine &engine();
inline void tables_written() { engine().inv_valid = 0; }
struct SamplerArgs;
bool take_attached_sampler(SamplerArgs &a, unsigned &blocks, float share = 1.0f);
int flush_attached_sampler(hipStream_t stream);
int attach_sampler(int32_t *d_h, int32_t *d_t, int32_t *d_r, int64_t B, int64_t neg, int64_t negrel, int64_t thread_lo,
                   int64_t thread_hi, int64_t out_stride, int64_t *n_local_out, hipStream_t stream);
void set_error(const std::string &msg);
int fail(int code, const std::string &msg);
bool device_ok();
int ensure_device_index();
int hip_check(hipError_t e, const char *what);

constexpr int kMaxLossBlocks = 4096;

struct NegClass { bool same_h, same_t, same_r, fast; };
template <int MODEL>
__host__ __device__ inline NegClass classify_negative(long long h, long long t, long long r, long long nh,
                                                               long long nt, long long nr, int negative_rel) {
    NegClass c;
    c.same_r = nr == r;
    const bool ctx_same = MODEL == KGE_TRANSE ? true : (MODEL == KGE_TRANSR ? (negative_rel == 0 || c.same_r) : c.same_r);
    c.same_h = nh == h && ctx_same;
    c.same_t = nt == t && ctx_same;
    c.fast = ((int)!c.same_h + (int)!c.same_t + (int)!c.same_r) == 1;
    return c;
}



struct FloatRowSpace {
    float *g_ent, *g_rel, *g_auxr, *g_auxe;
    long long E, R;
    long long hub_base, hub_rows;
    long long rows;
    float scale = 1.0f;
};
bool pair_path_active(const kge_model_desc &m, int64_t n_pos, int64_t n_neg);
bool transr_group_layout_active(const kge_model_desc &m, int64_t n_pos, int64_t n_neg);
int sgd_rows_skipped(int32_t *out);
int float_records_workspace(int64_t M, int D, float *&rec, int32_t *&dst);
int float_records_reduce(int64_t M, int D, const FloatRowSpace &rs, hipStream_t stream, const float *rec_ext = nullptr, int32_t *dst_ext = nullptr,
                         bool deterministic = false);
struct AdamRows {
    float *m[4], *v[4];
    float lr_t, b1, b2, eps;
};
int float_records_reduce_adam(int64_t M, int D, const FloatRowSpace &rs, const AdamRows &ad, hipStream_t stream, const float *rec_ext = nullptr,
                              int32_t *dst_ext = nullptr);
int launch_forward_backward_records(const kge_model_desc &m, const float *const tables[4], const int32_t *d_h, const int32_t *d_t,
                                    const int32_t *d_r, int64_t n_pos, int64_t n_neg, int64_t stride, int64_t denom, int64_t n_pos_total,
                                    float *d_rec, int32_t *d_dst, int64_t rec_offset, int64_t rec_slice, float *d_loss, hipStream_t stream);
int launch_float_records_apply_adam(const kge_model_desc &m, float *const tables[4], const AdamRows &ad, const float *d_rec, int32_t *d_dst,
                                    int64_t M_total, int64_t n_pos_total, int64_t n_neg, hipStream_t stream);
int launch_float_records_apply(const kge_model_desc &m, float *const tables[4], const float *d_rec, int32_t *d_dst, int64_t M_total,
                               int64_t n_pos_total, int64_t n_neg, float lr, hipStream_t stream);

bool device_index_build_supported(int64_t E, int64_t R, int64_t n);
std::string build_index_device(KgIndex &ix, DeviceIndex &dev, int64_t E, int64_t R, int64_t new_batch, int64_t n, const int64_t *h,
                               const int64_t *t, const int64_t *r);

int launch_sampler(int32_t *d_h, int32_t *d_t, int32_t *d_r, int64_t B, int64_t neg, int64_t negrel, int64_t thread_lo,
                   int64_t thread_hi, int64_t out_stride, int64_t *n_local, hipStream_t stream);
int launch_widen(const int32_t *src3, int64_t *dst3_and_y, int64_t B, int64_t total, hipStream_t stream);
int launch_forward_backward(const kge_model_desc &m, const float *const tables[4], const int32_t *d_h, const int32_t *d_t,
                            const int32_t *d_r, int64_t n_pos, int64_t n_neg, int64_t stride, int64_t denom,
                            float *const grads[4], float *d_loss, hipStream_t stream, bool sampler_shaped = false, float inplace_lr = 0.f,
                            const AdamRows *inplace_adam = nullptr);
int launch_predict(const kge_model_desc &m, const float *const tables[4], const int32_t *d_h, const int32_t *d_t,
                   const int32_t *d_r, int64_t n, float *d_out, hipStream_t stream);
int launch_lp_table(const kge_model_desc &m, const float *const tables[4], const float *P_all, int64_t r, float *T, hipStream_t stream);
int launch_lp_scores(const kge_model_desc &m, const float *const tables[4], const float *T, int64_t r, const int32_t *d_req_fixed,
                     const int32_t *d_req_head, int64_t n_req, float *d_scores, hipStream_t stream);
int transr_project_all(const kge_model_desc &m, const float *const tables[4], int64_t r, float *P_out, hipStream_t stream);
int launch_sgd(float *p, float *g, int64_t n, float lr, hipStream_t stream);
int launch_sgd_tables(int n_tables, float *const *p, float *const *g, const int64_t *numel, float lr, hipStream_t stream);
int launch_adam_tables(int n_tables, float *const *p, float *const *m, float *const *v, float *const *g, const int64_t *numel,
                       float lr_t, float b1, float b2, float eps, hipStream_t stream);
int launch_adam(float *p, float *m, float *v, float *g, int64_t n, float lr_t, float b1, float b2, float eps,
                hipStream_t stream);

}
```

### openkeonspark_amd/csrc/models.hip

```cpp
#include "models_dev.hpp"
#include "sampler_dev.hpp"
#include "team_shape.hpp"

namespace kge {

__global__ void loss_finalize_kernel(const float *partials, int n, float unit, float *out) {
    __shared__ float sh[256];
    float s = 0.f;
    for (int i = threadIdx.x; i < n; i += 256) s += partials[i];
    sh[threadIdx.x] = s;
    __syncthreads();
    for (int w = 128; w > 0; w >>= 1) {
        if ((int)threadIdx.x < w) sh[threadIdx.x] += sh[threadIdx.x + w];
        __syncthreads();
    }
    if (threadIdx.x == 0) out[0] = sh[0] * unit;
}

__device__ __forceinline__ uint32_t padd8(uint32_t x, uint32_t y) {
    return ((x & 0x7F7F7F7Fu) + (y & 0x7F7F7F7Fu)) ^ ((x ^ y) & 0x80808080u);
}
__device__ __forceinline__ uint32_t pneg8(uint32_t x) { return padd8(~x, 0x01010101u); }
__device__ __forceinline__ uint32_t pmul_sign8(uint32_t s, uint32_t cnt) {
    const uint32_t nz = s & 0x01010101u, neg = (s >> 7) & 0x01010101u;
// ... 292 lines not shown
                        f[u] = code[u] == 1 ? -iv : iv;
                    }
                }
                float sc[K];
#pragma unroll
                for (int u = 0; u < K; u++) {
                    float acc = 0.f;
                    auto apply = [&](const float4 (&Bs)[Q]) {
#pragma unroll
                        for (int q = 0; q < Q; q++) {
                            x[u][q].x = fmaf(f[u], x[u][q].x, Bs[q].x); x[u][q].y = fmaf(f[u], x[u][q].y, Bs[q].y);
                            x[u][q].z = fmaf(f[u], x[u][q].z, Bs[q].z); x[u][q].w = fmaf(f[u], x[u][q].w, Bs[q].w);
                            acc += fabsf(x[u][q].x) + fabsf(x[u][q].y) + fabsf(x[u][q].z) + fabsf(x[u][q].w);
                        }
                    };
                    if (code[u] == 0) apply(B0); else if (code[u] == 1) apply(B1); else apply(B2);
                    sc[u] = acc;
                }
#pragma unroll
                for (int u = 0; u < K; u++) sc[u] = team_sum<L>(sc[u]);
#pragma unroll
                for (int u = 0; u < K; u++) {
                    if (kk + u >= in_round) continue;
                    const float v = p - sc[u] + a.margin;
                    if (v >= 0.f) {
                        cnt++; lsum += v;
                        const long long m = (long long)(3 + k0 + kk + u) * a.n_pos + b;
                        uint32_t rec[Q];
                        const int c = code[u];
                        const s16x2 kh = pack16(c == 0 ? 0 : -1, c == 0 ? 0 : -1), kt = pack16(c == 1 ? 0 : 1, c == 1 ? 0 : 1);
                        const s16x2 kr = pack16(c == 2 ? 0 : -1, c == 2 ? 0 : -1), kx = pack16(c == 1 ? 1 : -1, c == 1 ? 1 : -1);
#pragma unroll
                        for (int q = 0; q < Q; q++) {
                            const s16x2 s_lo = pack16(sign_of_bits(x[u][q].x), sign_of_bits(x[u][q].y));
                            const s16x2 s_hi = pack16(sign_of_bits(x[u][q].z), sign_of_bits(x[u][q].w));
                            rec[q] = bytes_of(s_lo * kx, s_hi * kx);
                            Ah_lo[q] += s_lo * kh; Ah_hi[q] += s_hi * kh;
                            At_lo[q] += s_lo * kt; At_hi[q] += s_hi * kt;
                            Ar_lo[q] += s_lo * kr; Ar_hi[q] += s_hi * kr;
                        }
                        if constexpr (REC2) {
                            uint8_t *p2 = a.rec2 + ((long long)(k0 + kk + u) * a.n_pos + b) * (long long)(L * Q);
#pragma unroll
                            for (int q = 0; q < Q; q++) {
                                const uint32_t f = ((rec[q] & 0x03030303u) + 0x01010101u) & 0x03030303u;
                                if (valid[q]) p2[lane + L * q] = (uint8_t)((f * 0x01041040u) >> 24);
                            }
                        } else {
                            store_record<L, Q>(a, lane, m, rec);
                        }
                        if (lane == kk + u) my_dst = REC2 ? 2 * (code[u] == 2 ? rel_row0 + row[u] : row[u]) + 1 : (code[u] == 2 ? rel_row0 + row[u] : row[u]);
                    }
                }
            }
            if (k0 + lane < (int)a.n_neg) a.dst[(long long)(3 + k0 + lane) * a.n_pos + b] = my_dst;
        }
        if (cnt > 0) {
            uint32_t rh[Q], rt[Q], rr[Q];
            const s16x2 c2 = pack16(cnt, cnt);
#pragma unroll
            for (int q = 0; q < Q; q++) {
                const s16x2 v_lo = sp_lo[q] * c2, v_hi = sp_hi[q] * c2;
                rh[q] = bytes_of(Ah_lo[q] + v_lo, Ah_hi[q] + v_hi);
                rt[q] = bytes_of(At_lo[q] - v_lo, At_hi[q] - v_hi);
                rr[q] = bytes_of(Ar_lo[q] + v_lo, Ar_hi[q] + v_hi);
            }
            store_record<L, Q>(a, lane, b, rh);
            store_record<L, Q>(a, lane, a.n_pos + b, rt);
            store_record<L, Q>(a, lane, 2 * a.n_pos + b, rr);
        }
        if (lane == 0) {
            constexpr int KM = REC2 ? 2 : 1;
            a.dst[b] = cnt > 0 ? (int32_t)(KM * h) : -1;
            a.dst[a.n_pos + b] = cnt > 0 ? (int32_t)(KM * t) : -1;
            a.dst[2 * a.n_pos + b] = cnt > 0 ? (int32_t)(KM * (rel_row0 + r)) : -1;
        }
    }
    finish_loss<TEAMS>(a, red, lsum, lane, team_in_block);
}

typedef float f32x4 __attribute__((ext_vector_type(4)));
template <int V> struct IntC { static constexpr int value = V; };

template <bool INV_TAB, bool REC2>
__device__ __forceinline__ void transe_emit_rounds_body(const FbArgs &a) {
    constexpr int L = 64, TEAMS = 256 / L;
    __shared__ float red[TEAMS];
    const int lane = threadIdx.x % L;
    const int team_in_block = __builtin_amdgcn_readfirstlane(threadIdx.x / L);
    const int D = a.D;
    const int n_neg = (int)a.n_neg;
    const float *inv_ent = a.inv_norm, *inv_rel = a.inv_norm + a.ent_total;
    const bool valid = 4 * lane < D;
    const bool odd = lane & 1, hi2 = lane & 2;
    auto load_row = [&](const float *tab, long long row) {
        const __amdgpu_buffer_rsrc_t rsrc = __builtin_amdgcn_make_buffer_rsrc(const_cast<float *>(tab + row * D), 0, D * 4, 0x00020000);
        const f32x4 v = __builtin_bit_cast(f32x4, __builtin_amdgcn_raw_buffer_load_b128(rsrc, lane * 16, 0, 0));
        return make_float4(v.x, v.y, v.z, v.w);
    };
    auto ssq = [](const float4 &x) { return add_rn(add_rn(add_rn(mul_rn(x.x, x.x), mul_rn(x.y, x.y)), mul_rn(x.z, x.z)), mul_rn(x.w, x.w)); };
    float lsum = 0.f;
    for (long long b = (long long)blockIdx.x * TEAMS + team_in_block; b < a.n_pos; b += (long long)gridDim.x * TEAMS) {
        const int h = a.bh[b], t = a.bt[b], r = a.br[b];
        const int rel_row0 = a.ent_total + ((int)b & (a.krel - 1)) * a.rel_total;
        int my_code = 0, my_row = 0;
        float my_f = 0.f;
        bool bad = false;
        for (int k = lane; k < n_neg; k += L) {
            const long long j = b + (long long)(k + 1) * a.stride;
            const int nh = a.bh[j], nt = a.bt[j], nr = a.br[j];
            const NegClass nc = classify_negative<KGE_TRANSE>(h, t, r, nh, nt, nr, a.negative_rel);
            if (!nc.fast) bad = true;
            if (k < L) {
                my_code = !nc.same_h ? 0 : (!nc.same_t ? 1 : 2);
                my_row = !nc.same_h ? nh : (!nc.same_t ? nt : nr);
            }
        }
        if (__builtin_amdgcn_ballot_w64(bad) != 0) {
            if (lane == 0) {
                for (long long sl = 0; sl < 3 + a.n_neg; sl++) a.dst[sl * a.n_pos + b] = -1;
                if (a.group_list) a.group_list[atomicAdd(a.group_count, 1)] = (int32_t)b;
            }
            continue;
        }
        if constexpr (INV_TAB) {
            if (lane < n_neg) { const float iv = my_code == 2 ? inv_rel[my_row] : inv_ent[my_row]; my_f = my_code == 1 ? -iv : iv; }
        }
        float4 B0, B1, B2;
        float p;
        s16x2 sp_lo, sp_hi;
        {
            const float4 hn = load_row(a.ent, h), tn = load_row(a.ent, t), rn = load_row(a.rel, r);
            float ih, it, ir;
            if constexpr (INV_TAB) { ih = inv_ent[h]; it = inv_ent[t]; ir = inv_rel[r]; }
            else {
                const float sh = team_sum<L>(ssq(hn)), st = team_sum<L>(ssq(tn)), sr = team_sum<L>(ssq(rn));
                ih = 1.0f / sqrtf(sh >= 1e-12f ? sh : 1e-12f); it = 1.0f / sqrtf(st >= 1e-12f ? st : 1e-12f);
                ir = 1.0f / sqrtf(sr >= 1e-12f ? sr : 1e-12f);
            }
            auto one = [&](float hx, float tx, float rx, float &b0, float &b1, float &b2) {
                const float Rv = mul_rn(rx, ir), Hv = mul_rn(hx, ih), Tv = mul_rn(tx, it);
                const float HR = __builtin_fmaf(hx, ih, Rv);
                b0 = add_rn(sub_rn(Rv, Tv), 0.0f); b1 = add_rn(HR, 0.0f); b2 = add_rn(sub_rn(Hv, Tv), 0.0f);
                return add_rn(__builtin_fmaf(-tx, it, HR), 0.0f);
            };
            const float e0 = one(hn.x, tn.x, rn.x, B0.x, B1.x, B2.x), e1 = one(hn.y, tn.y, rn.y, B0.y, B1.y, B2.y);
            const float e2 = one(hn.z, tn.z, rn.z, B0.z, B1.z, B2.z), e3 = one(hn.w, tn.w, rn.w, B0.w, B1.w, B2.w);
            const float acc = add_rn(add_rn(add_rn(fabsf(e0), fabsf(e1)), fabsf(e2)), fabsf(e3));
            sp_lo = pack16(sign_of_bits(e0), sign_of_bits(e1));
            sp_hi = pack16(sign_of_bits(e2), sign_of_bits(e3));
            p = team_sum<L>(acc);
        }
        s16x2 Ah_lo = 0, Ah_hi = 0, At_lo = 0, At_hi = 0, Ar_lo = 0, Ar_hi = 0;
        int cnt = 0;
        for (int k0 = 0; k0 < n_neg; k0 += L) {
            if (k0 > 0) {
                const int my_k = k0 + lane;
                my_code = 0; my_row = 0; my_f = 0.f;
                if (my_k < n_neg) {
                    const long long j = b + (long long)(my_k + 1) * a.stride;
                    const int nh = a.bh[j], nt = a.bt[j], nr = a.br[j];
                    const NegClass nc = classify_negative<KGE_TRANSE>(h, t, r, nh, nt, nr, a.negative_rel);
                    my_code = !nc.same_h ? 0 : (!nc.same_t ? 1 : 2);
                    my_row = !nc.same_h ? nh : (!nc.same_t ? nt : nr);
                    if constexpr (INV_TAB) {
                        const float iv = my_code == 2 ? inv_rel[my_row] : inv_ent[my_row];
                        my_f = my_code == 1 ? -iv : iv;
                    }
                }
            }
            const bool mine = k0 + lane < n_neg;
            unsigned long long act = 0;
            float parked = 0.f;
            auto round = [&](auto code_c, auto n_c, unsigned long long &m) {
                constexpr int CODE = decltype(code_c)::value, N = decltype(n_c)::value;
                int kl[N], row[N];
                float f[N];
                float4 x[N];
#pragma unroll
                for (int u = 0; u < N; u++) {
                    kl[u] = __builtin_ctzll(m); m &= m - 1;
                    row[u] = __builtin_amdgcn_readlane(my_row, kl[u]);
                    if constexpr (INV_TAB) f[u] = __builtin_bit_cast(float, __builtin_amdgcn_readlane(__builtin_bit_cast(int, my_f), kl[u]));
                }
#pragma unroll
                for (int u = 0; u < N; u++) x[u] = load_row(CODE == 2 ? a.rel : a.ent, row[u]);
                if constexpr (!INV_TAB) {
                    float q2[4] = {0.f, 0.f, 0.f, 0.f};
#pragma unroll
                    for (int u = 0; u < N; u++) q2[u] = ssq(x[u]);
                    const int s4 = __builtin_bit_cast(int, team_sum4(q2[0], q2[1], q2[2], q2[3], odd, hi2));
#pragma unroll
                    for (int u = 0; u < N; u++) {
                        const float ss = __builtin_bit_cast(float, __builtin_amdgcn_readlane(s4, 60 + u));
                        const float iv = 1.0f / sqrtf(ss >= 1e-12f ? ss : 1e-12f);
                        f[u] = CODE == 1 ? -iv : iv;
                    }
                }
                const float4 &Bs = CODE == 0 ? B0 : (CODE == 1 ? B1 : B2);
                float sc[4] = {0.f, 0.f, 0.f, 0.f};
#pragma unroll
                for (int u = 0; u < N; u++) {
                    x[u].x = fmaf(f[u], x[u].x, Bs.x); x[u].y = fmaf(f[u], x[u].y, Bs.y);
                    x[u].z = fmaf(f[u], x[u].z, Bs.z); x[u].w = fmaf(f[u], x[u].w, Bs.w);
                    sc[u] = add_rn(add_rn(add_rn(fabsf(x[u].x), fabsf(x[u].y)), fabsf(x[u].z)), fabsf(x[u].w));
                }
                const float v = add_rn(sub_rn(p, team_sum4(sc[0], sc[1], sc[2], sc[3], odd, hi2)), a.margin);
                const unsigned hits = (unsigned)(__builtin_amdgcn_ballot_w64(v >= 0.f) >> 60) & ((1u << N) - 1u);
#pragma unroll
                for (int u = 0; u < N; u++) {
                    if (!((hits >> u) & 1u)) continue;
                    cnt++;
                    act |= 1ull << kl[u];
                    if (lane == kl[u]) parked = __builtin_bit_cast(float, __builtin_amdgcn_readlane(__builtin_bit_cast(int, v), 60 + u));
                    const s16x2 s_lo = pack16(sign_of_bits(x[u].x), sign_of_bits(x[u].y));
                    const s16x2 s_hi = pack16(sign_of_bits(x[u].z), sign_of_bits(x[u].w));
                    const uint32_t rec = CODE == 1 ? bytes_of(s_lo, s_hi) : bytes_of(-s_lo, -s_hi);
                    if constexpr (CODE != 0) { Ah_lo -= s_lo; Ah_hi -= s_hi; }
                    if constexpr (CODE != 1) { At_lo += s_lo; At_hi += s_hi; }
                    if constexpr (CODE != 2) { Ar_lo -= s_lo; Ar_hi -= s_hi; }
                    if constexpr (REC2) {
                        uint8_t *p2 = a.rec2 + ((long long)(k0 + kl[u]) * a.n_pos + b) * (long long)L;
                        const uint32_t fl = ((rec & 0x03030303u) + 0x01010101u) & 0x03030303u;
                        if (valid) p2[lane] = (uint8_t)((fl * 0x01041040u) >> 24);
                    } else {
                        a.rec[((long long)(3 + k0 + kl[u]) * a.n_pos + b) * (long long)L + lane] = rec;
                    }
                }
            };
            auto kind = [&](auto code_c, unsigned long long m) {
                while (__builtin_popcountll(m) >= 4) round(code_c, IntC<4>{}, m);
                const int left = __builtin_popcountll(m);
                if (left == 3) round(code_c, IntC<3>{}, m);
                else if (left == 2) round(code_c, IntC<2>{}, m);
                else if (left == 1) round(code_c, IntC<1>{}, m);
            };
            kind(IntC<0>{}, __builtin_amdgcn_ballot_w64(mine && my_code == 0));
            kind(IntC<1>{}, __builtin_amdgcn_ballot_w64(mine && my_code == 1));
            kind(IntC<2>{}, __builtin_amdgcn_ballot_w64(mine && my_code == 2));
            for (unsigned long long m = act; m; m &= m - 1)
                lsum += __builtin_bit_cast(float, __builtin_amdgcn_readlane(__builtin_bit_cast(int, parked), __builtin_ctzll(m)));
            if (mine) {
                const int key = my_code == 2 ? rel_row0 + my_row : my_row;
                a.dst[(long long)(3 + k0 + lane) * a.n_pos + b] = ((act >> lane) & 1ull) ? (REC2 ? 2 * key + 1 : key) : -1;
            }
        }
        if (cnt > 0) {
            const s16x2 c2 = pack16(cnt, cnt);
            const s16x2 v_lo = sp_lo * c2, v_hi = sp_hi * c2;
            a.rec[b * (long long)L + lane] = bytes_of(Ah_lo + v_lo, Ah_hi + v_hi);
            a.rec[(a.n_pos + b) * (long long)L + lane] = bytes_of(At_lo - v_lo, At_hi - v_hi);
            a.rec[(2 * a.n_pos + b) * (long long)L + lane] = bytes_of(Ar_lo + v_lo, Ar_hi + v_hi);
        }
        if (lane == 0) {
            constexpr int KM = REC2 ? 2 : 1;
            a.dst[b] = cnt > 0 ? (int32_t)(KM * h) : -1;
            a.dst[a.n_pos + b] = cnt > 0 ? (int32_t)(KM * t) : -1;
            a.dst[2 * a.n_pos + b] = cnt > 0 ? (int32_t)(KM * (rel_row0 + r)) : -1;
        }
    }
    finish_loss<TEAMS>(a, red, lsum, lane, team_in_block);
}

template <int L, int Q, int K, int WPE, bool INV_TAB, bool REC2 = false>
__global__ __launch_bounds__(256, WPE) void transe_emit_vec_kernel(FbArgs a) {
    if constexpr (L == 64 && Q == 1) transe_emit_rounds_body<INV_TAB, REC2>(a);
    else transe_emit_vec_body<L, Q, K, INV_TAB, REC2>(a);
}

template <int L, int Q, int K, int WPE, bool INV_TAB, bool REC2 = false>
__global__ __launch_bounds__(256, WPE) void transe_emit_vec_v1_kernel(FbArgs a) { transe_emit_vec_body<L, Q, K, INV_TAB, REC2>(a); }


template <int L, int C>
__global__ __launch_bounds__(256) void row_inv_norm_kernel(const float *__restrict__ ent_, const float *__restrict__ rel_, long long E, long long R,
                                                           int D, float *__restrict__ out) {
    constexpr int TEAMS = 256 / L;
    const int lane = threadIdx.x % L;
    for (long long row = (long long)blockIdx.x * TEAMS + threadIdx.x / L; row < E + R; row += (long long)gridDim.x * TEAMS) {
        float x[C];
        const float *p = row < E ? ent_ + row * D : rel_ + (row - E) * D;
#pragma unroll
        for (int c = 0; c < C; c++) { const int e = lane + L * c; x[c] = e < D ? p[e] : 0.f; }
        const float inv = row_inv_norm<L, C>(x);
        if (lane == 0) out[row] = inv;
    }
}

static void record_emit_done(hipStream_t stream) {
    Engine &eng = engine();
    if (!eng.record_emit_event) return;
    if (!eng.emit_done) (void)hipEventCreateWithFlags(&eng.emit_done, hipEventDisableTiming);
    (void)hipEventRecord(eng.emit_done, stream);
    eng.emit_seq++;
}

constexpr int kDeferBlocks = 128;

template <int L, int C>
static void launch_emit(const FbArgs &a_in, float *d_loss, hipStream_t stream) {
    constexpr int TEAMS = 256 / L;
    FbArgs a = a_in;
    const bool defer_pass = a.g_ent && a.g_rel;
    guard_loss_stream(stream);
    if (!defer_pass) { a.loss_out = d_loss; a.loss_ticket = engine().dev.loss_ticket; }
    long long blocks = (a.n_pos + TEAMS - 1) / TEAMS;
    if (blocks > kMaxLossBlocks) blocks = kMaxLossBlocks;
    if (blocks < 1) blocks = 1;
    if (a.D % 4 == 0) {
        const bool inv_tab = a.inv_norm != nullptr;
        Engine &eng0 = engine();
        const bool carried = eng0.inv_carry && eng0.inv_valid && eng0.inv_for_ent == a.ent && eng0.inv_for_rel == a.rel;
        if (inv_tab && !carried) {
            long long nb = (a.ent_total + a.rel_total + TEAMS - 1) / TEAMS;
            if (nb > 2048) nb = 2048;
            hipLaunchKernelGGL((row_inv_norm_kernel<L, C>), dim3((unsigned)nb), dim3(256), 0, stream, a.ent, a.rel,
                               (long long)a.ent_total, (long long)a.rel_total, a.D, const_cast<float *>(a.inv_norm));
            eng0.inv_for_ent = a.ent; eng0.inv_for_rel = a.rel; eng0.inv_valid = 1;
        }
        Engine &eng = engine();
        const int slot = (int)(eng.emit_launches % Engine::kEmitRing);
        const bool timed = eng.time_emit > 0 && (eng.emit_seen++ % eng.time_emit) == 0;
        if (timed) {
            if (!eng.ev_emit0[slot]) { (void)hipEventCreate(&eng.ev_emit0[slot]); (void)hipEventCreate(&eng.ev_emit1[slot]); }
            (void)hipEventRecord(eng.ev_emit0[slot], stream);
        }
        constexpr int Q = (C + 3) / 4;
        const dim3 grid((unsigned)blocks), block(256);
        bool v1 = false;
        if constexpr (L == 64 && Q == 1) {
            if (!eng.emit_rounds) {
                v1 = true;
                if (a.rec2) {
                    if (inv_tab) hipLaunchKernelGGL((transe_emit_vec_v1_kernel<L, Q, 4, 1, true, true>), grid, block, 0, stream, a);
                    else hipLaunchKernelGGL((transe_emit_vec_v1_kernel<L, Q, 4, 1, false, true>), grid, block, 0, stream, a);
                } else if (inv_tab) hipLaunchKernelGGL((transe_emit_vec_v1_kernel<L, Q, 4, 1, true>), grid, block, 0, stream, a);
                else hipLaunchKernelGGL((transe_emit_vec_v1_kernel<L, Q, 4, 1, false>), grid, block, 0, stream, a);
            }
        }
        if (v1) {
        } else if (a.rec2) {
            if (inv_tab) hipLaunchKernelGGL((transe_emit_vec_kernel<L, Q, 4, 1, true, true>), grid, block, 0, stream, a);
            else hipLaunchKernelGGL((transe_emit_vec_kernel<L, Q, 4, 1, false, true>), grid, block, 0, stream, a);
        } else if (inv_tab) hipLaunchKernelGGL((transe_emit_vec_kernel<L, Q, 4, 1, true>), grid, block, 0, stream, a);
        else hipLaunchKernelGGL((transe_emit_vec_kernel<L, Q, 4, 1, false>), grid, block, 0, stream, a);
        if (timed) { (void)hipEventRecord(eng.ev_emit1[slot], stream); eng.emit_launches++; }
        record_emit_done(stream);
    } else {
        hipLaunchKernelGGL((transe_emit_kernel<L, C>), dim3((unsigned)blocks), dim3(256), 0, stream, a);
        record_emit_done(stream);
    }
    if (!defer_pass) return;
    FbArgs d = a;
    d.loss_partials = a.loss_partials + blocks;
    hipLaunchKernelGGL((fwdbwd_kernel<KGE_TRANSE, L, C>), dim3(kDeferBlocks), dim3(256), 0, stream, d);
    hipLaunchKernelGGL(loss_finalize_kernel, dim3(1), dim3(256), 0, stream, a.loss_partials, (int)blocks + kDeferBlocks, a.unit, d_loss);
}

void guard_loss_stream(hipStream_t stream) {
    static hipStream_t last = nullptr;
    static bool have = false;
    if (have && last != stream) (void)hipStreamSynchronize(last);
    last = stream; have = true;
}

int ensure_loss_buffers() {
    Engine &e = engine();
    if (!e.dev.loss_partials) {
        int rc = hip_check(hipMalloc(&e.dev.loss_partials, sizeof(float) * (kMaxLossBlocks + 256)), "alloc loss partials");
        if (rc) return rc;
    }
    if (!e.dev.loss_ticket) {
        const size_t n = 1 + (kMaxLossBlocks + 31) / 32;
        int rc = hip_check(hipMalloc(&e.dev.loss_ticket, sizeof(unsigned) * n), "alloc loss ticket");
        if (rc) return rc;
        if ((rc = hip_check(hipMemset(e.dev.loss_ticket, 0, sizeof(unsigned) * n), "zero loss ticket"))) return rc;
    }
    return KGE_OK;
}

void transe_team_shape(int D, int &L, int &C) {
    for_transe_team_shape_or_last(D, [&](auto t) { L = decltype(t)::L; C = decltype(t)::C; });
}

static int32_t *g_defer_list = nullptr, *g_defer_count = nullptr;
static int64_t g_defer_cap = 0;

static int32_t *g_skipped = nullptr;
int sgd_rows_skipped(int32_t *out) {
    *out = 0;
    if (!g_skipped) return KGE_OK;
    return hip_check(hipMemcpy(out, g_skipped, sizeof(int32_t), hipMemcpyDeviceToHost), "read skipped-negatives counter");
}

int transe_deferred_groups(int32_t *out) {
    *out = 0;
    if (!g_defer_count) return KGE_OK;
    return hip_check(hipMemcpy(out, g_defer_count, sizeof(int32_t), hipMemcpyDeviceToHost), "read deferred count");
}

int launch_transe_emit(const kge_model_desc &m, const float *ent, const float *rel, float *resid_ent, float *resid_rel,
                       const int32_t *d_h, const int32_t *d_t, const int32_t *d_r, int64_t n_pos, int64_t n_neg, int64_t stride,
                       int64_t denom, uint32_t *rec, int32_t *dst, int krel, float *d_loss, hipStream_t stream, bool track_deferred,
                       uint8_t *rec2) {
    Engine &e = engine();
    { int rc = ensure_loss_buffers(); if (rc) return rc; }
    int32_t *&defer_list = g_defer_list, *&defer_count = g_defer_count;
    int64_t &defer_cap = g_defer_cap;
    if (n_pos > defer_cap) {
        if (defer_list) (void)hipFree(defer_list);
        defer_list = nullptr;
        int rc = hip_check(hipMalloc(&defer_list, sizeof(int32_t) * (size_t)n_pos), "alloc deferred groups");
        if (rc) return rc;
        if (!defer_count && (rc = hip_check(hipMalloc(&defer_count, sizeof(int32_t)), "alloc deferred count"))) return rc;
        defer_cap = n_pos;
    }
    if (track_deferred) {
        int rc = hip_check(hipMemsetAsync(defer_count, 0, sizeof(int32_t), stream), "zero deferred count");
        if (rc) return rc;
    }
    const bool use_inv_table = (m.ent_total + m.rel_total) * (int64_t)m.ent_dim * 4 <= e.inv_table_max_bytes;
    if (use_inv_table && m.ent_total + m.rel_total > e.inv_cap) {
        if (e.inv_norm) (void)hipFree(e.inv_norm);
        e.inv_norm = nullptr; e.inv_valid = 0;
        int rc = hip_check(hipMalloc(&e.inv_norm, sizeof(float) * (size_t)(m.ent_total + m.rel_total)), "alloc row inverse norms");
        if (rc) return rc;
        e.inv_cap = m.ent_total + m.rel_total;
    }
    FbArgs a = {};
    a.inv_norm = use_inv_table ? e.inv_norm : nullptr;
    a.group_list = track_deferred ? defer_list : nullptr; a.group_count = defer_count;
    a.ent = ent; a.rel = rel; a.g_ent = resid_ent; a.g_rel = resid_rel;
    a.bh = d_h; a.bt = d_t; a.br = d_r;
    a.n_pos = n_pos; a.n_neg = n_neg; a.stride = stride;
    a.D = m.ent_dim; a.margin = m.margin; a.unit = 1.0f / (float)denom;
    a.loss_partials = e.dev.loss_partials;
    a.negative_rel = m.negative_rel;
    a.rec = rec; a.rec2 = (m.ent_dim % 4 == 0) ? rec2 : nullptr; a.dst = dst; a.ent_total = (int)m.ent_total; a.rel_total = (int)m.rel_total; a.krel = 1;
    a.loss_limbs = track_deferred ? nullptr : e.loss_limbs;
    while (a.krel * 2 <= krel) a.krel *= 2;
    if (!for_transe_team_shape(a.D, [&](auto t) { launch_emit<decltype(t)::L, decltype(t)::C>(a, d_loss, stream); }))
        return fail(KGE_ERR_UNSUPPORTED, "embedding dimension > 1024");
    return hip_check(hipGetLastError(), "transe emit launch");
}

template <int MODEL, int L, int C>
__global__ __launch_bounds__(256) void fwdbwd_ride_kernel(FbArgs a, SamplerArgs ride, int n_ride) {
    if ((int)blockIdx.x >= a.loss_blocks) {
        __shared__ float bern_lds[kBernLds];
        sample_block_ride(ride, (long long)blockIdx.x - a.loss_blocks, bern_lds);
        return;
    }
    fwdbwd_body<MODEL, L, C, false>(a);
}
template <int MODEL, int L, int C>
__global__ __launch_bounds__(256, 4) void fwdbwd_ride_kernel_occ4(FbArgs a, SamplerArgs ride, int n_ride) {
    if ((int)blockIdx.x >= a.loss_blocks) {
        __shared__ float bern_lds[kBernLds];
        sample_block_ride(ride, (long long)blockIdx.x - a.loss_blocks, bern_lds);
        return;
    }
    fwdbwd_body<MODEL, L, C, false>(a);
}

template <int MODEL, int L, int C>
static void launch_fb(const FbArgs &a, float *d_loss, hipStream_t stream) {
    constexpr int TEAMS = 256 / L;
    long long blocks = (a.n_pos + TEAMS - 1) / TEAMS;
    if (blocks > kMaxLossBlocks) blocks = kMaxLossBlocks;
    if (blocks < 1) blocks = 1;
    FbArgs f = a;
    guard_loss_stream(stream);
    f.loss_out = d_loss; f.loss_ticket = engine().dev.loss_ticket;
    if constexpr (MODEL != KGE_TRANSR) {
        SamplerArgs ride = {};
        unsigned n_ride = 0;
        if (upload_jump_table() == KGE_OK && take_attached_sampler(ride, n_ride) && n_ride > 0) {
            f.loss_blocks = (int)blocks;
            if constexpr (MODEL != KGE_TRANSE && C <= 4) {
                if (engine().fb_occ4) {
                    hipLaunchKernelGGL((fwdbwd_ride_kernel_occ4<MODEL, L, C>), dim3((unsigned)blocks + n_ride), dim3(256), 0, stream, f, ride, (int)n_ride);
                    return;
                }
            }
            hipLaunchKernelGGL((fwdbwd_ride_kernel<MODEL, L, C>), dim3((unsigned)blocks + n_ride), dim3(256), 0, stream, f, ride, (int)n_ride);
            return;
        }
    }
    if constexpr (MODEL != KGE_TRANSE && C <= 4) {
        if (engine().fb_occ4) { hipLaunchKernelGGL((fwdbwd_kernel_occ4<MODEL, L, C>), dim3((unsigned)blocks), dim3(256), 0, stream, f); return; }
    }
    hipLaunchKernelGGL((fwdbwd_kernel<MODEL, L, C>), dim3((unsigned)blocks), dim3(256), 0, stream, f);
}

template <int MODEL, int L, int C>
static void launch_fb_records(const FbArgs &a, float *d_loss, hipStream_t stream) {
    constexpr int TEAMS = 256 / L;
    long long blocks = (a.n_pos + TEAMS - 1) / TEAMS;
    if (blocks > kMaxLossBlocks) blocks = kMaxLossBlocks;
    if (blocks < 1) blocks = 1;
    FbArgs f = a;
    guard_loss_stream(stream);
    f.loss_out = d_loss; f.loss_ticket = engine().dev.loss_ticket;
    if constexpr ((MODEL == KGE_TRANSH || MODEL == KGE_TRANSD) && C <= 4) {
        if (engine().fb_occ4) { hipLaunchKernelGGL((fwdbwd_kernel_occ4<MODEL, L, C, true>), dim3((unsigned)blocks), dim3(256), 0, stream, f); return; }
    }
    hipLaunchKernelGGL((fwdbwd_kernel<MODEL, L, C, true>), dim3((unsigned)blocks), dim3(256), 0, stream, f);
}

template <int MODEL>
static int dispatch_fb_records(const FbArgs &a, float *d_loss, hipStream_t stream) {
    if (!for_team_shape(a.D, [&](auto t) { launch_fb_records<MODEL, decltype(t)::L, decltype(t)::C>(a, d_loss, stream); }))
        return fail(KGE_ERR_UNSUPPORTED, "embedding dimension > 1024 is not supported by the vector-model kernels");
    return KGE_OK;
}

__global__ __launch_bounds__(256) void hub_fold_kernel(float *__restrict__ copies_rel, float *__restrict__ copies_auxr,
                                                       float *__restrict__ g_rel, float *__restrict__ g_auxr, int K, long long RD) {
    for (long long i = (long long)blockIdx.x * blockDim.x + threadIdx.x; i < 2 * RD; i += (long long)gridDim.x * blockDim.x) {
        float *c = i < RD ? copies_rel : copies_auxr;
        float *g = i < RD ? g_rel : g_auxr;
        if (!c) continue;
        const long long j = i < RD ? i : i - RD;
// ... 640 lines not shown
```

### openkeonspark_amd/csrc/models_dev.hpp

```cpp
#pragma once
#include "engine.hpp"
#include "team.hpp"

namespace kge {

struct FbArgs {
    const float *ent, *rel, *auxr, *auxe;
    float *g_ent, *g_rel, *g_auxr, *g_auxe;
    const int32_t *bh, *bt, *br;
    long long n_pos, n_neg, stride;
    int D;
    float margin, unit;
    float *loss_partials;
    const float *P;
    float *GP;
    int negative_rel;
    uint32_t *rec;
    int32_t *dst;
    uint8_t *rec2;
    int ent_total, rel_total, krel;
    int32_t *group_list;
    int32_t *group_count;
    const float *inv_norm;
    float *loss_out;
    unsigned *loss_ticket;
    float *frec;
    int32_t *fdst;
    long long hub_base;
    int hub_k, hub_rows;
    float *copies_rel, *copies_auxr;
    float2 *pair_aux;
    int32_t *skipped;
    int32_t *loss_limbs;
    int loss_blocks;
};

int ensure_loss_buffers();
void guard_loss_stream(hipStream_t stream);

template <int TEAMS>
__device__ __forceinline__ void finish_loss_sh(const FbArgs &a, float *red, float lsum, int lane, int team_in_block, float *sh) {
    __shared__ int is_last;
    const unsigned nblk = a.loss_blocks ? (unsigned)a.loss_blocks : gridDim.x;
    if (lane == 0) red[team_in_block] = lsum;
    __syncthreads();
    if (threadIdx.x == 0) {
        float s = 0.f;
#pragma unroll
        for (int i = 0; i < TEAMS; i++) s += red[i];
        is_last = 0;
        if (a.loss_out) {
            unsigned *slot = reinterpret_cast<unsigned *>(a.loss_partials) + blockIdx.x;
            (void)__hip_atomic_exchange(slot, __float_as_uint(s), __ATOMIC_RELAXED, __HIP_MEMORY_SCOPE_AGENT);
            __builtin_amdgcn_s_waitcnt(0x0F70);
            const unsigned group = blockIdx.x >> 5, n_groups = (nblk + 31) >> 5;
            const unsigned in_group = min(32u, nblk - (group << 5));
            if (__hip_atomic_fetch_add(a.loss_ticket + 1 + group, 1u, __ATOMIC_RELAXED, __HIP_MEMORY_SCOPE_AGENT) == in_group - 1) {
                __hip_atomic_store(a.loss_ticket + 1 + group, 0u, __ATOMIC_RELAXED, __HIP_MEMORY_SCOPE_AGENT);
                is_last = __hip_atomic_fetch_add(a.loss_ticket, 1u, __ATOMIC_RELAXED, __HIP_MEMORY_SCOPE_AGENT) == n_groups - 1 ? 1 : 0;
            }
        } else {
            a.loss_partials[blockIdx.x] = s;
        }
    }
    if (!a.loss_out) return;
    __syncthreads();
    if (!is_last) return;
    const unsigned *part = reinterpret_cast<const unsigned *>(a.loss_partials);
    float s = 0.f;
    for (int i = threadIdx.x; i < (int)nblk; i += 256)
        s += __uint_as_float(__hip_atomic_load(part + i, __ATOMIC_RELAXED, __HIP_MEMORY_SCOPE_AGENT));
    sh[threadIdx.x] = s;
    __syncthreads();
    for (int w = 128; w > 0; w >>= 1) {
        if ((int)threadIdx.x < w) sh[threadIdx.x] += sh[threadIdx.x + w];
        __syncthreads();
    }
    if (threadIdx.x == 0) {
        a.loss_out[0] = sh[0] * a.unit;
        if (a.loss_limbs) {
            const double x = (double)(sh[0] * a.unit) * 4294967296.0;
            const long long v = x >= 0.0 ? (long long)(x + 0.5) : 0;
            for (int i = 0; i < 4; i++) a.loss_limbs[i] = (int32_t)((v >> (16 * i)) & 0xFFFF);
        }
        __hip_atomic_store(a.loss_ticket, 0u, __ATOMIC_RELAXED, __HIP_MEMORY_SCOPE_AGENT);
    }
}

template <int TEAMS>
__device__ __forceinline__ void finish_loss(const FbArgs &a, float *red, float lsum, int lane, int team_in_block) {
    __shared__ float sh[256];
    finish_loss_sh<TEAMS>(a, red, lsum, lane, team_in_block, sh);
}

template <bool REC, int L, int C>
__device__ __forceinline__ void put_row(const Team<L, C> &tm, const FbArgs &a, float *gtab, long long row, long long vrow, long long m,
                                        const float (&v)[C]) {
    if (REC && m >= 0) {
        float *p = a.frec + m * a.D;
#pragma unroll
        for (int c = 0; c < C; c++) { const int e = tm.lane + L * c; if (e < a.D) p[e] = v[c]; }
        if (tm.lane == 0) a.fdst[m] = (int32_t)vrow;
    } else {
        tm.add(gtab, row, v);
    }
}

typedef short s16x2 __attribute__((ext_vector_type(2)));

__device__ __forceinline__ int sign_of_bits(float e) {
    int r;
    asm("v_med3_i32 %0, %1, -1, 1" : "=v"(r) : "v"(__builtin_bit_cast(int, e)));
    return r;
}
__device__ __forceinline__ s16x2 pack16(int lo, int hi) { s16x2 r; r.x = (short)lo; r.y = (short)hi; return r; }
__device__ __forceinline__ uint32_t bytes_of(s16x2 lo, s16x2 hi) {
    return __builtin_amdgcn_perm(__builtin_bit_cast(uint32_t, hi), __builtin_bit_cast(uint32_t, lo), 0x06040200u);
// ... 302 lines not shown
```

### openkeonspark_amd/csrc/sampler.hip

```cpp
#include "sampler_dev.hpp"

namespace kge {

__global__ __launch_bounds__(256) void sample_kernel_wide(SamplerArgs a) { sample_block_wide(a, blockIdx.x, gridDim.x); }

__global__ __launch_bounds__(256) void sample_kernel(SamplerArgs a) {
    __shared__ float bern_lds[kBernLds];
    sample_block(a, blockIdx.x, gridDim.x, bern_lds);
}

__global__ __launch_bounds__(256) void sample_kernel_part(SamplerArgs a) {
    __shared__ float bern_lds[kBernLds];
    sample_block_ride(a, blockIdx.x, bern_lds);
}

__global__ void advance_streams_kernel(uint64_t *streams, long long W, long long B, long long per_thread,
                                       unsigned long long draws) {
    long long id = (long long)blockIdx.x * blockDim.x + threadIdx.x;
    if (id >= W) return;
    long long lef = id * per_thread, rig = lef + per_thread;
    if (rig > B) rig = B;
    if (lef > B) lef = B;
    streams[id] = lcg_skip(streams[id], (unsigned long long)(rig - lef) * draws);
}

__global__ void widen_kernel(const int32_t *__restrict__ src, long long *__restrict__ dst, float *__restrict__ y,
                             long long B, long long total) {
    for (long long i = (long long)blockIdx.x * blockDim.x + threadIdx.x; i < total; i += (long long)gridDim.x * blockDim.x) {
        dst[i] = src[i];
        dst[total + i] = src[total + i];
        dst[2 * total + i] = src[2 * total + i];
        y[i] = i < B ? 1.0f : -1.0f;
    }
}

static int build_sampler(int32_t *d_h, int32_t *d_t, int32_t *d_r, int64_t B, int64_t neg, int64_t negrel, int64_t thread_lo,
                         int64_t thread_hi, int64_t out_stride, int64_t *n_local_out, SamplerArgs &a, unsigned &blocks, bool &wide) {
    Engine &e = engine();
    int rc = ensure_device_index();
    if (rc) return rc;
    const int64_t W = e.work_threads;
    if (B <= 0 || neg < 0 || negrel < 0 || thread_lo < 0 || thread_hi > W || thread_lo > thread_hi)
        return fail(KGE_ERR_BAD_ARG, "kge_sampling_device: bad batch/thread range");
    if (e.index.train_dup <= 0) return fail(KGE_ERR_NO_DATASET, "sampling: empty training set");
    if ((rc = upload_jump_table())) return rc;
    int64_t lo, hi, tmp;
    if (thread_lo == thread_hi) { lo = hi = 0; }
    else { thread_slice(B, W, thread_lo, lo, tmp); thread_slice(B, W, thread_hi - 1, tmp, hi); }
    const int64_t n_local = hi - lo;
    if (n_local_out) *n_local_out = n_local;
    if (out_stride < n_local) return fail(KGE_ERR_BAD_ARG, "kge_sampling_device: out_stride smaller than the slice");
    const int64_t per_thread = (B % W == 0) ? B / W : B / W + 1;
    a = SamplerArgs();
    a.pos = e.dev.pos; a.grp = e.dev.grp; a.ht = e.dev.ht;
    a.tails_hr = e.dev.tails_hr; a.heads_tr = e.dev.heads_tr; a.rels_ht = e.dev.rels_ht;
    a.bern_prob = e.dev.bern_prob; a.streams = e.dev.streams;
    a.out_h = d_h; a.out_t = d_t; a.out_r = d_r;
    a.per_thread = per_thread; a.pos_lo = lo; a.n_local = n_local; a.out_stride = out_stride;
    a.train_dup = e.index.train_dup; a.new_batch = e.index.new_batch;
    a.ent_total = (int)e.index.ent_total; a.rel_total = (int)e.index.rel_total;
    a.neg = (int)neg; a.negrel = (int)negrel; a.bern = e.bern ? 1 : 0;
    a.pick_div = (unsigned long long)(a.new_batch > 0 ? a.new_batch : a.train_dup);
    a.pick_magic = ~0ull / a.pick_div;
    int kshift = 0;
    while ((1 << kshift) < 1 + neg + negrel) kshift++;
    a.kshift = kshift;
    a.streams_next = e.dev.streams_next; a.W = W; a.B = B;
    wide = kshift > 6;
    int64_t nb = n_local > 0 ? ((n_local << kshift) + 255) / 256 : 0;
    if (nb > (1 << 20)) nb = 1 << 20;
    blocks = (unsigned)nb;
    return KGE_OK;
}

static bool g_att_armed = false, g_att_wide = false;
static SamplerArgs g_att;
static unsigned g_att_blocks = 0, g_att_next = 0;

bool take_attached_sampler(SamplerArgs &a, unsigned &blocks, float share) {
    if (!g_att_armed || g_att_wide || g_att_blocks == 0) return false;
    const unsigned left = g_att_blocks - g_att_next;
    unsigned want = share >= 1.0f ? left : (unsigned)(share * (float)g_att_blocks + 0.5f);
    if (want > left) want = left;
    if (want == 0) return false;
    a = g_att; a.ride_first = g_att_next; a.ride_total = g_att_blocks;
    blocks = want;
    g_att_next += want;
    if (g_att_next >= g_att_blocks) g_att_armed = false;
    return true;
}

int flush_attached_sampler(hipStream_t stream) {
    if (!g_att_armed) return KGE_OK;
    g_att_armed = false;
    if (g_att_wide) hipLaunchKernelGGL(sample_kernel_wide, dim3(g_att_blocks), dim3(256), 0, stream, g_att);
    else if (g_att_next == 0) hipLaunchKernelGGL(sample_kernel, dim3(g_att_blocks), dim3(256), 0, stream, g_att);
    else {
        SamplerArgs a = g_att;
        a.ride_first = g_att_next; a.ride_total = g_att_blocks;
        hipLaunchKernelGGL(sample_kernel_part, dim3(g_att_blocks - g_att_next), dim3(256), 0, stream, a);
    }
    return hip_check(hipGetLastError(), "sampler launch");
}

int attach_sampler(int32_t *d_h, int32_t *d_t, int32_t *d_r, int64_t B, int64_t neg, int64_t negrel, int64_t thread_lo,
                   int64_t thread_hi, int64_t out_stride, int64_t *n_local_out, hipStream_t stream) {
    Engine &e = engine();
    int rc = flush_attached_sampler(stream);
    if (rc) return rc;
    SamplerArgs a; unsigned blocks; bool wide;
    if ((rc = build_sampler(d_h, d_t, d_r, B, neg, negrel, thread_lo, thread_hi, out_stride, n_local_out, a, blocks, wide))) return rc;
    if (blocks == 0) {
        hipLaunchKernelGGL(advance_streams_kernel, dim3((unsigned)((a.W + 63) / 64)), dim3(64), 0, stream, e.dev.streams,
                           (long long)a.W, (long long)B, (long long)a.per_thread, (unsigned long long)(1 + 2 * neg + negrel));
        e.dev.streams_sync = 2;
        return hip_check(hipGetLastError(), "sampler launch");
    }
    g_att = a; g_att_blocks = blocks; g_att_next = 0; g_att_wide = wide; g_att_armed = true;
    std::swap(e.dev.streams, e.dev.streams_next);
    e.dev.streams_sync = 2;
    return KGE_OK;
}

int launch_sampler(int32_t *d_h, int32_t *d_t, int32_t *d_r, int64_t B, int64_t neg, int64_t negrel, int64_t thread_lo,
                   int64_t thread_hi, int64_t out_stride, int64_t *n_local_out, hipStream_t stream) {
    Engine &e = engine();
    int rc = flush_attached_sampler(stream);
    if (rc) return rc;
    SamplerArgs a; unsigned blocks; bool wide;
    if ((rc = build_sampler(d_h, d_t, d_r, B, neg, negrel, thread_lo, thread_hi, out_stride, n_local_out, a, blocks, wide))) return rc;
    if (blocks > 0) {
        if (!wide) hipLaunchKernelGGL(sample_kernel, dim3(blocks), dim3(256), 0, stream, a);
        else hipLaunchKernelGGL(sample_kernel_wide, dim3(blocks), dim3(256), 0, stream, a);
        std::swap(e.dev.streams, e.dev.streams_next);
    } else
        hipLaunchKernelGGL(advance_streams_kernel, dim3((unsigned)((a.W + 63) / 64)), dim3(64), 0, stream, e.dev.streams,
                           (long long)a.W, (long long)B, (long long)a.per_thread,
                           (unsigned long long)(1 + 2 * neg + negrel));
    e.dev.streams_sync = 2;
    return hip_check(hipGetLastError(), "sampler launch");
}

int launch_widen(const int32_t *src3, int64_t *dst3_and_y, int64_t B, int64_t total, hipStream_t stream) {
    int64_t blocks = (total + 255) / 256;
    if (blocks > 4096) blocks = 4096;
    if (blocks < 1) blocks = 1;
    hipLaunchKernelGGL(widen_kernel, dim3((unsigned)blocks), dim3(256), 0, stream, src3, (long long *)dst3_and_y,
                       (float *)(dst3_and_y + 3 * total), (long long)B, (long long)total);
    return hip_check(hipGetLastError(), "widen launch");
}

}
```

### openkeonspark_amd/csrc/sampler_dev.hpp

```cpp
#pragma once
#include "engine.hpp"

namespace kge {

static __constant__ LcgJumpTable c_jump;
static bool g_jump_uploaded = false;

static inline int upload_jump_table() {
    if (g_jump_uploaded) return KGE_OK;
    int rc = hip_check(hipMemcpyToSymbol(HIP_SYMBOL(c_jump), &engine().jump, sizeof(LcgJumpTable)), "upload jump table");
    if (rc == KGE_OK) g_jump_uploaded = true;
    return rc;
}

struct SamplerArgs {
    const int4 *pos;
    const int4 *grp;
    const int2 *ht;
    const int32_t *tails_hr, *heads_tr, *rels_ht;
    const float *bern_prob;
    const uint64_t *streams;
    uint64_t *streams_next;
    long long W, B;
    int32_t *out_h, *out_t, *out_r;
    long long per_thread;
    long long pos_lo;
    long long n_local;
    long long out_stride;
    long long train_dup, new_batch;
    unsigned long long pick_div, pick_magic;
    int ent_total, rel_total;
    int neg, negrel, bern;
    int kshift;
    unsigned ride_first, ride_total;
};

__device__ __forceinline__ uint64_t lcg_step(uint64_t s) { return s * kLcgMul + kLcgAdd; }

__device__ __forceinline__ uint64_t lcg_skip(uint64_t s, uint64_t n) {
    for (int j = 0; n != 0; ++j, n >>= 1)
        if (n & 1) s = c_jump.mulA[j] * s + c_jump.addC[j];
    return s;
}

__device__ __forceinline__ uint64_t mod_magic(uint64_t s, uint64_t d, uint64_t m) {
    uint64_t r = s - __umul64hi(s, m) * d;
    while (r >= d) r -= d;
    return r;
}
__device__ __forceinline__ uint32_t mod_u64_u32(uint64_t s, uint32_t d) {
    if (d == 0) return 0;
    const double rcp = 1.0 / (double)d;
    const uint32_t hi = (uint32_t)(s >> 32), lo = (uint32_t)s;
    uint32_t q1 = (uint32_t)((double)hi * rcp);
    int64_t r1 = (int64_t)hi - (int64_t)q1 * d;
    if (r1 < 0) r1 += d;
    if (r1 >= (int64_t)d) r1 -= d;
    const uint64_t x = ((uint64_t)r1 << 32) | lo;
    const double xd = (double)(uint32_t)r1 * 4294967296.0 + (double)lo;
    uint64_t q2 = (uint64_t)(xd * rcp);
    int64_t r2 = (int64_t)(x - q2 * d);
    if (r2 < 0) r2 += d;
    if (r2 < 0) r2 += d;
    if (r2 >= (int64_t)d) r2 -= d;
    if (r2 >= (int64_t)d) r2 -= d;
    return (uint32_t)r2;
}

__device__ __forceinline__ int filtered_pick(const int32_t *__restrict__ vals, int len, long long tmp) {
    int lo = 0, hi = len;
    while (lo < hi) {
        int mid = (lo + hi) >> 1;
        if ((long long)vals[mid] - mid <= tmp) lo = mid + 1; else hi = mid;
    }
    return (int)(tmp + lo);
}

__device__ __forceinline__ int filtered_pick_short(const int32_t *__restrict__ vals, int len, long long tmp) {
    if (len > 4) return filtered_pick(vals, len, tmp);
    if (len <= 0) return (int)tmp;
    int v[4];
#pragma unroll
    for (int j = 0; j < 4; j++) v[j] = vals[j < len ? j : len - 1];
    int lo = 0;
#pragma unroll
    for (int j = 0; j < 4; j++) lo += (j < len && (long long)v[j] - j <= tmp) ? 1 : 0;
    return (int)(tmp + lo);
}

__device__ __forceinline__ uint64_t lcg_skip_lanes(uint64_t s, unsigned n) {
#pragma unroll
    for (int j = 0; j < 16; j++) {
        if (!__any((n >> j) != 0u)) break;
        const uint64_t t = c_jump.mulA[j] * s + c_jump.addC[j];
        s = ((n >> j) & 1u) ? t : s;
    }
    return s;
}

__device__ __forceinline__ void sample_slot(const SamplerArgs &a, long long p, long long k, unsigned long long skip_draws, int &oh, int &ot,
                                            int &orr) {
    const long long id = (long long)((unsigned)p / (unsigned)a.per_thread);
    const long long off = p - id * a.per_thread;
    const unsigned long long draws = 1ull + 2ull * a.neg + a.negrel;
    uint64_t s = lcg_skip(a.streams[id], skip_draws + (unsigned long long)off * draws);
    s = lcg_step(s);
    long long i = (long long)mod_magic(s, a.pick_div, a.pick_magic) + (a.new_batch > 0 ? a.train_dup - a.new_batch : 0);
// ... 24 lines not shown

__device__ __forceinline__ void write_next_streams(const SamplerArgs &a, int kp, long long block, long long n_blocks) {
    for (long long id = block * 256 + threadIdx.x; id < a.W; id += n_blocks * 256) {
        long long lef = id * a.per_thread, rig = lef + a.per_thread;
        if (rig > a.B) rig = a.B;
        if (lef > a.B) lef = a.B;
        a.streams_next[id] = lcg_skip(a.streams[id], (unsigned long long)(rig - lef) * (unsigned long long)(kp + a.neg));
    }
}

__device__ __forceinline__ void sample_block_wide(const SamplerArgs &a, long long block, long long n_blocks) {
    const int kshift = a.kshift, kp = 1 + a.neg + a.negrel;
    write_next_streams(a, kp, block, n_blocks);
    for (long long g = block * 256 + threadIdx.x; (g >> kshift) < a.n_local; g += n_blocks * 256) {
        const long long b = g >> kshift;
        const long long k = g & ((1 << kshift) - 1);
        if (k >= kp) continue;
        int oh, ot, orr;
        sample_slot(a, a.pos_lo + b, k, 0ull, oh, ot, orr);
        const long long o = b + k * a.out_stride;
        a.out_h[o] = oh; a.out_t[o] = ot; a.out_r[o] = orr;
    }
}

constexpr int kBernLds = 2048;

__device__ __forceinline__ void sample_block(const SamplerArgs &a, long long block, long long n_blocks, float *bern_lds) {
    const int kshift = a.kshift, kp = 1 + a.neg + a.negrel, kmask = (1 << kshift) - 1;
    const unsigned long long draws = 1ull + 2ull * a.neg + a.negrel;
    write_next_streams(a, kp, block, n_blocks);
    const bool bern_in_lds = a.bern && a.rel_total <= kBernLds;
    if (bern_in_lds) {
        for (int i = threadIdx.x; i < a.rel_total; i += 256) bern_lds[i] = a.bern_prob[i];
        __syncthreads();
    }
    const int lane = threadIdx.x & 63;
    const long long total = a.n_local << kshift;
    const long long wave0 = block * 256 + (__builtin_amdgcn_readfirstlane(threadIdx.x) & ~63);
    for (long long g0 = wave0; g0 < total; g0 += n_blocks * 256) {
        const long long p0 = a.pos_lo + (g0 >> kshift);
        const long long id0 = (long long)((unsigned)p0 / (unsigned)a.per_thread);
        const long long off0 = p0 - id0 * a.per_thread;
        const uint64_t base0 = lcg_skip(a.streams[id0], (unsigned long long)off0 * draws);
        const long long g = g0 + lane;
        long long b = g >> kshift;
        const int k = (int)(g & kmask);
        const bool live = b < a.n_local && k < kp;
        if (b >= a.n_local) b = a.n_local - 1;
        const int kk = k < kp ? k : kp - 1;
        const long long p = a.pos_lo + b;
        const long long id = (long long)((unsigned)p / (unsigned)a.per_thread);
        const long long off = p - id * a.per_thread;
        const bool same = id == id0;
        uint64_t s = same ? base0 : a.streams[id];
        unsigned ahead = (unsigned)((same ? off - off0 : off) * (long long)draws);
        if (kk >= 1) ahead += kk <= a.neg ? 1u + 2u * (unsigned)(kk - 1) : 1u + 2u * (unsigned)a.neg + (unsigned)(kk - 1 - a.neg);
        s = lcg_skip_lanes(s, ahead);
        s = lcg_step(s);
        const long long pick = (long long)mod_magic(s, a.pick_div, a.pick_magic) + (a.new_batch > 0 ? a.train_dup - a.new_batch : 0);
        const long long i = __shfl((int)pick, lane & ~kmask);
        const int4 tr = a.pos[i];
        const int4 gq = a.grp[i];
        int oh = tr.x, ot = tr.y, orr = tr.z;
        if (kk >= 1 && kk <= a.neg) {
            const float prob = a.bern ? (bern_in_lds ? bern_lds[orr] : a.bern_prob[orr]) : 500.0f;
            const bool keep_head = (float)(s % 1000ull) < prob;
            s = lcg_step(s);
            if (keep_head) {
                const long long tmp = (long long)mod_u64_u32(s, (uint32_t)(a.ent_total - gq.y));
                ot = min(filtered_pick_short(a.tails_hr + gq.x, gq.y, tmp), a.ent_total - 1);
            } else {
                const long long tmp = (long long)mod_u64_u32(s, (uint32_t)(a.ent_total - gq.w));
                oh = min(filtered_pick_short(a.heads_tr + gq.z, gq.w, tmp), a.ent_total - 1);
            }
        } else if (kk > a.neg) {
            const int2 gr = a.ht[i];
            const long long tmp = (long long)mod_u64_u32(s, (uint32_t)(a.rel_total - gr.y));
            orr = min(filtered_pick_short(a.rels_ht + gr.x, gr.y, tmp), a.rel_total - 1);
        }
        if (live) {
            const long long o = b + (long long)k * a.out_stride;
            a.out_h[o] = oh; a.out_t[o] = ot; a.out_r[o] = orr;
        }
    }
}


__device__ __forceinline__ void sample_block_ride(const SamplerArgs &a, long long i, float *bern_lds) {
    sample_block(a, (long long)a.ride_first + i, (long long)a.ride_total, bern_lds);
}

}
```

### openkeonspark_amd/csrc/transe_counts.hip

```cpp
#include <cstring>
#include <string.h>

#include <rocprim/rocprim.hpp>

#include "engine.hpp"
#include "team.hpp"
#include "team_shape.hpp"
#include "sampler_dev.hpp"
#include "optim_dev.hpp"

namespace kge {

void transe_team_shape(int D, int &L, int &C);
int launch_transe_emit(const kge_model_desc &m, const float *ent, const float *rel, float *resid_ent, float *resid_rel,
                       const int32_t *d_h, const int32_t *d_t, const int32_t *d_r, int64_t n_pos, int64_t n_neg, int64_t stride,
                       int64_t denom, uint32_t *rec, int32_t *dst, int krel, float *d_loss, hipStream_t stream, bool track_deferred,
                       uint8_t *rec2 = nullptr);

int transe_deferred_groups(int32_t *out);

namespace {

int bits_for_rows(int64_t v) { int b = 1; while ((int64_t(1) << b) <= v) b++; return b; }

struct CtWork {
    uint32_t *rec = nullptr;
    float *hub_sums = nullptr;
    size_t hub_sums_cap = 0;
    int32_t *hub_marks = nullptr;
    size_t hub_marks_cap = 0;
    int32_t *dst = nullptr, *dst_sorted = nullptr, *ids = nullptr, *ids_sorted = nullptr;
    int32_t *n_valid = nullptr;
    int32_t *tile_hist = nullptr, *bucket_start = nullptr;
    int32_t *pairs = nullptr;
    float2 *pair_aux = nullptr;
    int64_t pair_aux_cap = 0;
    int64_t cap_hist = 0;
    void *sort_tmp = nullptr;
    size_t sort_tmp_bytes = 0, rec_elems = 0;
    int64_t cap_idx = 0;
    int32_t *bflag = nullptr;
    int64_t bflag_cap = 0;
    int4 *pieces = nullptr;
    int64_t pieces_cap = 0;
    int32_t *n_pieces = nullptr;
    int2 *row_span = nullptr;
    int64_t row_span_cap = 0;
};
CtWork g_c;

template <typename T>
int regrow(T *&p, size_t count, const char *what) {
    if (p) (void)hipFree(p);
    p = nullptr;
    return hip_check(hipMalloc(&p, sizeof(T) * (count ? count : 1)), what);
}

int ensure_counts_work(int64_t M, size_t rec_dwords) {
    int rc;
    if (M > g_c.cap_idx) {
        const int64_t cap = M;
        if ((rc = regrow(g_c.dst, (size_t)cap, "counts dst"))) return rc;
        if ((rc = regrow(g_c.dst_sorted, (size_t)cap, "counts dst_sorted"))) return rc;
        if ((rc = regrow(g_c.ids, (size_t)cap, "counts ids"))) return rc;
        if ((rc = regrow(g_c.ids_sorted, (size_t)cap, "counts ids_sorted"))) return rc;
        if ((rc = regrow(g_c.pairs, (size_t)cap * 2, "counts pairs"))) return rc;
        if (!g_c.n_valid && (rc = regrow(g_c.n_valid, 1, "counts n_valid"))) return rc;
        size_t bytes = 0;
        (void)rocprim::radix_sort_pairs(nullptr, bytes, g_c.dst, g_c.dst_sorted, g_c.ids, g_c.ids_sorted, (size_t)cap, 0, 32, nullptr);
        if (bytes > g_c.sort_tmp_bytes) {
            if (g_c.sort_tmp) (void)hipFree(g_c.sort_tmp);
            g_c.sort_tmp = nullptr;
            if ((rc = hip_check(hipMalloc(&g_c.sort_tmp, bytes), "counts sort temp"))) return rc;
            g_c.sort_tmp_bytes = bytes;
        }
        std::vector<int32_t> iota((size_t)cap);
        for (int64_t i = 0; i < cap; i++) iota[(size_t)i] = (int32_t)i;
        if ((rc = hip_check(hipMemcpy(g_c.ids, iota.data(), sizeof(int32_t) * (size_t)cap, hipMemcpyHostToDevice), "counts iota"))) return rc;
        g_c.cap_idx = cap;
    }
    if (rec_dwords > 0 && (size_t)M * rec_dwords > g_c.rec_elems) {
        if ((rc = regrow(g_c.rec, (size_t)M * rec_dwords, "counts records"))) return rc;
        g_c.rec_elems = (size_t)M * rec_dwords;
    }
    return KGE_OK;
}

__global__ void fix_keys_kernel(int32_t *dst, long long M, int sentinel) {
    for (long long i = (long long)blockIdx.x * blockDim.x + threadIdx.x; i < M; i += (long long)gridDim.x * blockDim.x)
        if (dst[i] < 0) dst[i] = sentinel;
}

__global__ void count_valid_kernel(const int32_t *__restrict__ sorted, int M, int sentinel, int32_t *n_valid) {
    if (threadIdx.x == 0 && blockIdx.x == 0) {
        int lo = 0, hi = M;
        while (lo < hi) { int mid = (lo + hi) >> 1; if (sorted[mid] < sentinel) lo = mid + 1; else hi = mid; }
        n_valid[0] = lo;
    }
}

// ... 1332 lines not shown
    }
#pragma unroll
    for (int q = 0; q < Q; q++) {
#pragma unroll
        for (int j = 0; j < 4; j++) acc[4 * q + j] += (int)((pk[q] >> (8 * j)) & 0xFFu) - n2;
    }
#pragma unroll
    for (int q = 0; q < Q; q++)
        *reinterpret_cast<int4 *>(stage + 4 * (lane + L * q)) = make_int4(acc[4 * q], acc[4 * q + 1], acc[4 * q + 2], acc[4 * q + 3]);
    int si[C];
#pragma unroll
    for (int c = 0; c < C; c++) { const int e = lane + L * c; si[c] = e < ap.D ? stage[e] : 0; }
    if (sa.diag & 2) return;
    if (direct) {
        float sf[C], rs[C];
        float *rp = ap.resid ? ap.resid + (long long)row * ap.D : nullptr;
#pragma unroll
        for (int c = 0; c < C; c++) { const int e = lane + L * c; sf[c] = (float)si[c]; rs[c] = (rp && e < ap.D) ? rp[e] : 0.f; }
        apply_row_update<L, C, false>(tm, ap, ap.p, ap.m, ap.v, row, row, sf, rs, x, mo, vo, true, nullptr, rp);
    } else {
        const long long irow = row < ap.E ? row : ap.E + (row - ap.E) % sa.fold_R;
        int32_t *p = sa.S + irow * ap.D;
#pragma unroll
        for (int c = 0; c < C; c++) { const int e = lane + L * c; if (e < ap.D && si[c] != 0) atomicAdd(p + e, si[c]); }
    }
}

template <int L, int C>
void launch_segsum(bool nat, int64_t M, const uint32_t *rec, const int32_t *n_valid_p, const int32_t *uidx, int32_t *S, int D,
                   const FuseArgs &fold, hipStream_t stream) {
    const long long chunks = (M + CHUNK - 1) / CHUNK;
    const long long nb = (chunks + (256 / L) - 1) / (256 / L);
    if (nat) hipLaunchKernelGGL((segsum_kernel<L, C, true>), dim3((unsigned)nb), dim3(256), 0, stream, rec, g_c.dst_sorted, g_c.ids_sorted,
                                n_valid_p, uidx, S, D, fold);
    else hipLaunchKernelGGL((segsum_kernel<L, C, false>), dim3((unsigned)nb), dim3(256), 0, stream, rec, g_c.dst_sorted, g_c.ids_sorted,
                            n_valid_p, uidx, S, D, fold);
}

void launch_apply_listed_rows(const ApplyArgs &a, long long max_rows, hipStream_t stream) {
    for_transe_team_shape_or_last(a.D, [&](auto t) {
        constexpr int L = decltype(t)::L, C = decltype(t)::C;
        long long nb = (max_rows + (256 / L) - 1) / (256 / L);
        if (nb > 8192) nb = 8192;
        hipLaunchKernelGGL((apply_counts_kernel<L, C, true>), dim3((unsigned)nb), dim3(256), 0, stream, a);
    });
}

float *inv_table_kept(bool whole_row_space, const float *ent, const float *rel, long long all_rows) {
    Engine &e = engine();
    const bool keeps = e.inv_carry && e.inv_valid && e.inv_norm && whole_row_space && e.inv_for_ent == ent && e.inv_for_rel == rel &&
                       e.inv_cap >= all_rows;
    if (!keeps) tables_written();
    return keeps ? e.inv_norm : nullptr;
}


}

}

using namespace kge;

extern "C" {

int kge_transe_counts_supported(const kge_model_desc *m, INT n_neg) {
    if (!m) return 0;
    return m->model == KGE_TRANSE && m->ent_dim == m->rel_dim && m->ent_dim <= 1024 && n_neg >= 1 && n_neg <= 63 &&
           m->ent_total + m->rel_total < (int64_t(1) << 30);
}

}

namespace kge { namespace {
struct FusedOpt {
    float *p[2], *m[2], *v[2];
    int adam;
    float lr, b1, b2, eps;
    bool done = false;
};
} }

static int forward_counts_impl(const kge_model_desc *m, const float *d_ent, const float *d_rel, const int32_t *d_h,
                               const int32_t *d_t, const int32_t *d_r, INT n_pos, INT n_neg, INT stride, INT denom,
                               int32_t *d_counts, float *d_resid_ent, float *d_resid_rel, float *d_loss, void *stream_, FusedOpt *fo) {
    hipStream_t stream = (hipStream_t)stream_;
    if (!device_ok()) return fail(KGE_ERR_NO_DEVICE, "kge_transe_forward_counts: no usable HIP device");
    if (!m || !kge_transe_counts_supported(m, n_neg)) return fail(KGE_ERR_UNSUPPORTED, "sign-count path: TransE, dim <= 1024, 1..63 negatives");
    if (n_pos < 0 || stride < n_pos || denom <= 0) return fail(KGE_ERR_BAD_ARG, "kge_transe_forward_counts: bad sizes");
    if (n_pos == 0) return hip_check(hipMemsetAsync(d_loss, 0, sizeof(float), stream), "zero loss");
    int L, C;
    transe_team_shape(m->ent_dim, L, C);
    const size_t rd = (size_t)L * ((C + 3) / 4);
    const int64_t M = n_pos * (3 + n_neg);
    if (M >= (int64_t(1) << 31)) return fail(KGE_ERR_UNSUPPORTED, "batch too large for the sign-count path");
    int rc = ensure_counts_work(M, rd);
    if (rc) return rc;
    int krel = 1;
    if (n_pos >= 4096 && m->rel_total > 0 && engine().counts_krel > 1) {
        krel = engine().counts_krel;
        while (krel > 1 && (int64_t)krel * m->rel_total > 2 * (m->ent_total + m->rel_total)) krel >>= 1;
    }
    const int rows = (int)(m->ent_total + (int64_t)krel * m->rel_total);
    const int D = m->ent_dim;
    const bool nat = D % 4 == 0;
    const int rpb = (rows + NB - 1) / NB;
    const int rows2 = 2 * rows, rpb2 = 2 * ((rows + NB - 1) / NB);
    const bool fused = fo && nat && rpb2 <= 4096 && !engine().counts_force_sort && engine().counts_fused &&
                       (uint64_t)M * rd * 4 < (uint64_t(1) << 32) && rows2 < (1 << 30);
    uint8_t *rec2 = fused ? reinterpret_cast<uint8_t *>(g_c.rec + (size_t)3 * (size_t)n_pos * rd) : nullptr;
    rc = launch_transe_emit(*m, d_ent, d_rel, d_resid_ent, d_resid_rel, d_h, d_t, d_r, n_pos, n_neg, stride, denom, g_c.rec, g_c.dst,
                            krel, d_loss, stream, d_resid_ent != nullptr && d_resid_rel != nullptr, rec2);
    if (rc) return rc;
    FuseArgs fold = FuseArgs();
    if (krel > 1) { fold.fold_E = (int)m->ent_total; fold.fold_R = (int)m->rel_total; }
    if (fused) {
        const int cap = std::min(engine().counts_fused_cap > 0 ? engine().counts_fused_cap : 64, std::min(127, 4 * L));
        const int64_t max_pieces = 3 * (M / cap + 1) + 16;
        if (max_pieces > g_c.pieces_cap) {
            if ((rc = regrow(g_c.pieces, (size_t)max_pieces, "fused step piece table"))) return rc;
            g_c.pieces_cap = max_pieces;
        }
        if (!g_c.n_pieces) {
            if ((rc = regrow(g_c.n_pieces, 1, "fused step piece counter"))) return rc;
            if ((rc = hip_check(hipMemset(g_c.n_pieces, 0, sizeof(int32_t)), "zero piece counter"))) return rc;
        }
        if (rows2 > g_c.row_span_cap) {
            if ((rc = regrow(g_c.row_span, (size_t)rows2, "fused step row spans"))) return rc;
            g_c.row_span_cap = rows2;
        }
        SegPlan plan;
        plan.row_span = g_c.row_span; plan.pieces = g_c.pieces; plan.n_pieces = g_c.n_pieces; plan.cap = cap;
        const int32_t *n_valid_p;
        if ((rc = bucket_sort_records(g_c.dst, M, rows2, rpb2, &plan, stream, n_valid_p))) return rc;
        const long long all_rows = m->ent_total + m->rel_total;
        SegApplyArgs sa = {};
        sa.rec = g_c.rec; sa.rec2_off = (unsigned)((size_t)3 * (size_t)n_pos * rd * 4); sa.ids = g_c.ids_sorted; sa.row_span = g_c.row_span;
        sa.pieces = g_c.pieces; sa.n_pieces = g_c.n_pieces;
        sa.n8 = (int)(3 * n_pos); sa.m_last = (int)M - 1; sa.n_rows_v = rows; sa.RD = (int)rd; sa.cap = cap; sa.S = d_counts; sa.fold_R = (int)m->rel_total; sa.diag = engine().counts_fused_diag;
        ApplyArgs &a = sa.ap;
        a.p = fo->p[0]; a.p2 = fo->p[1]; a.resid = d_resid_ent; a.resid2 = d_resid_rel;
        if (fo->adam) { a.m = fo->m[0]; a.m2 = fo->m[1]; a.v = fo->v[0]; a.v2 = fo->v[1]; }
        a.S = d_counts; a.rows = all_rows; a.row_lo = 0; a.E = m->ent_total; a.D = D;
        a.unit = 1.0f / (float)denom; a.lr = fo->lr; a.b1 = fo->b1; a.b2 = fo->b2; a.eps = fo->eps; a.adam = fo->adam;
        a.row_span = g_c.row_span; a.span_cap = cap;
        a.inv_out = inv_table_kept(true, fo->p[0], fo->p[1], all_rows);
        const bool shaped = for_transe_team_shape(D, [&](auto t) {
            constexpr int L = decltype(t)::L, C = decltype(t)::C;
            if constexpr (C >= 4) {
                const long long nb = ((long long)rows + max_pieces + (256 / L) - 1) / (256 / L);
                hipLaunchKernelGGL((segapply_kernel<L, C>), dim3((unsigned)nb), dim3(256), 0, stream, sa);
                long long nb2 = (all_rows + (256 / L) - 1) / (256 / L);
                if (nb2 > 8192) nb2 = 8192;
                SamplerArgs ride = {};
                const unsigned n_ride = take_ride(ride, 3);
                hipLaunchKernelGGL((apply_counts_kernel<L, C, false>), dim3((unsigned)nb2 + n_ride), dim3(256), 0, stream, a, ride, (int)nb2);
            }
        });
        if (!shaped) return fail(KGE_ERR_UNSUPPORTED, "sign-count path: TransE, dim <= 1024, 1..63 negatives");
        fo->done = true;
        return hip_check(hipGetLastError(), "fused counts step launch");
    }
    const bool bucket = rpb <= 8192 && !engine().counts_force_sort;
    const int32_t *n_valid_p;
    if (bucket) rc = bucket_sort_records(g_c.dst, M, rows, rpb, nullptr, stream, n_valid_p);
    else rc = radix_sort_records(g_c.dst, M, rows, false, "counts sort", stream, n_valid_p);
    if (rc) return rc;
    if (!for_transe_team_shape(D, [&](auto t) {
            launch_segsum<decltype(t)::L, decltype(t)::C>(nat, M, g_c.rec, n_valid_p, nullptr, d_counts, D, fold, stream);
        }))
        return fail(KGE_ERR_UNSUPPORTED, "sign-count path: TransE, dim <= 1024, 1..63 negatives");
    return hip_check(hipGetLastError(), bucket ? "counts bucket reduce launch" : "counts reduce launch");
}

extern "C" {

int kge_transe_forward_counts(const kge_model_desc *m, const float *d_ent, const float *d_rel, const int32_t *d_h,
                              const int32_t *d_t, const int32_t *d_r, INT n_pos, INT n_neg, INT stride, INT denom,
                              int32_t *d_counts, float *d_resid_ent, float *d_resid_rel, float *d_loss, void *stream_) {
    return forward_counts_impl(m, d_ent, d_rel, d_h, d_t, d_r, n_pos, n_neg, stride, denom, d_counts, d_resid_ent, d_resid_rel, d_loss,
                               stream_, nullptr);
}

int kge_transe_train_step_counts(const kge_model_desc *m, float *const d_p[2], float *const d_m[2], float *const d_v[2], const int32_t *d_h,
                                 const int32_t *d_t, const int32_t *d_r, INT n_pos, INT n_neg, INT stride, INT denom, int32_t *d_counts,
                                 float *const d_resid[2], int32_t sampler_shaped, int32_t adam, float lr, float beta1, float beta2, float eps,
                                 float *d_loss, void *stream_) {
    if (!m || !d_p || !d_p[0] || !d_p[1] || !d_counts || !d_resid || !d_resid[0] || !d_resid[1] || denom <= 0)
        return fail(KGE_ERR_BAD_ARG, "kge_transe_train_step_counts: bad arguments");
    if (adam && (!d_m || !d_v || !d_m[0] || !d_m[1] || !d_v[0] || !d_v[1]))
        return fail(KGE_ERR_BAD_ARG, "kge_transe_train_step_counts: Adam needs the moment tables");
    FusedOpt fo;
    fo.p[0] = d_p[0]; fo.p[1] = d_p[1];
    fo.m[0] = adam ? d_m[0] : nullptr; fo.m[1] = adam ? d_m[1] : nullptr; fo.v[0] = adam ? d_v[0] : nullptr; fo.v[1] = adam ? d_v[1] : nullptr;
    fo.adam = adam; fo.lr = lr; fo.b1 = beta1; fo.b2 = beta2; fo.eps = eps;
    const bool fed = !sampler_shaped;
    int rc = forward_counts_impl(m, d_p[0], d_p[1], d_h, d_t, d_r, n_pos, n_neg, stride, denom, d_counts, fed ? d_resid[0] : nullptr,
                                 fed ? d_resid[1] : nullptr, d_loss, stream_, &fo);
    if (rc || fo.done) return rc;
    return kge_transe_apply_counts_range(m, d_p, d_m, d_v, d_counts, d_resid, 0, m->ent_total + m->rel_total, denom, adam, lr, beta1, beta2,
                                         eps, stream_);
}

INT kge_transe_record_dwords(const kge_model_desc *m) {
    if (!m) return 0;
    int L, C;
    transe_team_shape(m->ent_dim, L, C);
    return (INT)L * ((C + 3) / 4);
}

int kge_transe_emit_records(const kge_model_desc *m, const float *d_ent, const float *d_rel, const int32_t *d_h, const int32_t *d_t,
                            const int32_t *d_r, INT n_pos, INT n_neg, INT stride, INT denom, uint32_t *d_rec, int32_t *d_dst,
                            float *d_resid_ent, float *d_resid_rel, float *d_loss, void *stream_) {
    hipStream_t stream = (hipStream_t)stream_;
    if (!device_ok()) return fail(KGE_ERR_NO_DEVICE, "kge_transe_emit_records: no usable HIP device");
    if (!m || !kge_transe_counts_supported(m, n_neg)) return fail(KGE_ERR_UNSUPPORTED, "sign-count path: TransE, dim <= 1024, 1..63 negatives");
    if (n_pos < 0 || stride < n_pos || denom <= 0 || !d_rec || !d_dst) return fail(KGE_ERR_BAD_ARG, "kge_transe_emit_records: bad arguments");
    if (n_pos == 0) return hip_check(hipMemsetAsync(d_loss, 0, sizeof(float), stream), "zero loss");
    return launch_transe_emit(*m, d_ent, d_rel, d_resid_ent, d_resid_rel, d_h, d_t, d_r, n_pos, n_neg, stride, denom, d_rec, d_dst, 1,
                              d_loss, stream, true);
}

int kge_transe_step_scratch_read(int which, INT offset, INT count, void *host_out) {
    if (!device_ok()) return fail(KGE_ERR_NO_DEVICE, "kge_transe_step_scratch_read: no usable HIP device");
    const size_t have = which == 0 ? g_c.rec_elems : (which == 1 ? (size_t)g_c.cap_idx : 0);
    const void *base = which == 0 ? (const void *)g_c.rec : (const void *)g_c.dst;
    if (!host_out || offset < 0 || count < 0 || (size_t)offset + (size_t)count > have || !base)
        return fail(KGE_ERR_BAD_ARG, "kge_transe_step_scratch_read: bad arguments");
    int rc = hip_check(hipDeviceSynchronize(), "kge_transe_step_scratch_read: synchronize");
    if (rc) return rc;
    return hip_check(hipMemcpy(host_out, (const char *)base + 4 * (size_t)offset, 4 * (size_t)count, hipMemcpyDeviceToHost), "kge_transe_step_scratch_read: copy");
}

int kge_transe_deferred_groups(int32_t *n_groups) {
    if (!n_groups) return fail(KGE_ERR_BAD_ARG, "kge_transe_deferred_groups: null output");
    return transe_deferred_groups(n_groups);
}

static int reduce_records_impl(const kge_model_desc *m, const uint32_t *d_rec, int32_t *d_dst, INT n_records, int32_t *d_rows,
                               int32_t *d_row_counts, int32_t *d_n_rows, const FuseArgs *fuse, hipStream_t stream) {
    if (!device_ok()) return fail(KGE_ERR_NO_DEVICE, "kge_transe_reduce_records: no usable HIP device");
    if (!m || !d_rec || !d_dst || !d_rows || !d_row_counts || !d_n_rows || n_records < 0 || n_records >= (INT(1) << 31))
        return fail(KGE_ERR_BAD_ARG, "kge_transe_reduce_records: bad arguments");
    if (n_records == 0) return hip_check(hipMemsetAsync(d_n_rows, 0, sizeof(int32_t), stream), "zero n_rows");
    int L, C;
    transe_team_shape(m->ent_dim, L, C);
    const int64_t M = n_records;
    int rc = ensure_counts_work(M, 0);
    if (rc) return rc;
    const int rows = (int)(m->ent_total + m->rel_total);
    const int D = m->ent_dim;
    const bool nat = D % 4 == 0;
    int blocks = (int)((M + 255) / 256);
    if (blocks > 4096) blocks = 4096;
    const int32_t *n_valid_p;
    if ((rc = radix_sort_records(d_dst, M, rows, false, "records sort", stream, n_valid_p))) return rc;
    int32_t *uidx = g_c.pairs;
    hipLaunchKernelGGL(run_flags_kernel, dim3(blocks), dim3(256), 0, stream, g_c.dst_sorted, g_c.n_valid, (int)M, uidx);
    size_t scan_bytes = 0;
    (void)rocprim::inclusive_scan(nullptr, scan_bytes, uidx, uidx, (size_t)M, rocprim::plus<int32_t>(), stream);
    if (scan_bytes > g_c.sort_tmp_bytes) {
        if (g_c.sort_tmp) (void)hipFree(g_c.sort_tmp);
        g_c.sort_tmp = nullptr;
        if ((rc = hip_check(hipMalloc(&g_c.sort_tmp, scan_bytes), "scan temp"))) return rc;
        g_c.sort_tmp_bytes = scan_bytes;
    }
    rc = hip_check(rocprim::inclusive_scan(g_c.sort_tmp, scan_bytes, uidx, uidx, (size_t)M, rocprim::plus<int32_t>(), stream), "run scan");
    if (rc) return rc;
    int32_t *bflag = nullptr;
    if (fuse) {
        if (!nat) return fail(KGE_ERR_UNSUPPORTED, "fused reduce+apply needs an embedding width that is a multiple of 4");
        if ((int64_t)g_c.bflag_cap < M) {
            if ((rc = regrow(g_c.bflag, (size_t)M, "boundary flags"))) return rc;
            g_c.bflag_cap = M;
        }
        bflag = g_c.bflag;
        if ((rc = hip_check(hipMemsetAsync(bflag, 0, sizeof(int32_t) * (size_t)M, stream), "zero boundary flags"))) return rc;
    }
    hipLaunchKernelGGL(unique_rows_kernel, dim3(blocks), dim3(256), 0, stream, g_c.dst_sorted, g_c.n_valid, uidx, d_rows, d_n_rows,
                       d_row_counts, D, bflag);
    {
// ... 148 lines not shown
```

Baseline: 148.0 million.

## Precompute packed negative classification in sampler for TransE emit kernel

The device sampler now also writes a packed word per negative, holding the corrupted row, the corruption code and a fast-path flag. The TransE counts emit kernel can consume these words instead of reloading the positive and negative triples and reclassifying them. This is meant to cut index loads and classification work in the forward-counts pass. The cost is an extra buffer write in the sampler and a second code path in emit, used only when the shape constraints hold (dim divisible by 4, team width 64).

```diff
diff --git a/include/kge_mi355.h b/include/kge_mi355.h
--- a/include/kge_mi355.h
+++ b/include/kge_mi355.h
@@ -80,6 +80,11 @@
 int kge_sampling_attach(int32_t *d_h, int32_t *d_t, int32_t *d_r, INT batchSize, INT negRate, INT negRelRate,
                         INT thread_lo, INT thread_hi, INT out_stride, INT *n_local, void *stream);
 int kge_sampling_flush(void *stream);
+int kge_sampling_device_packed(int32_t *d_h, int32_t *d_t, int32_t *d_r, int32_t *d_pack, INT batchSize, INT negRate, INT negRelRate,
+                               INT thread_lo, INT thread_hi, INT out_stride, INT *n_local, void *stream);
+int kge_sampling_attach_packed(int32_t *d_h, int32_t *d_t, int32_t *d_r, int32_t *d_pack, INT batchSize, INT negRate, INT negRelRate,
+                               INT thread_lo, INT thread_hi, INT out_stride, INT *n_local, void *stream);
+INT kge_emit_pack_words(INT n_positions, INT negRate, INT negRelRate, INT dim);
 INT kge_slice_positions(INT batchSize, INT thread_lo, INT thread_hi, INT *first_position);
 
 typedef struct kge_model_desc {
@@ -140,12 +145,20 @@
 int kge_transe_forward_counts(const kge_model_desc *m, const float *d_ent, const float *d_rel, const int32_t *d_h,
                               const int32_t *d_t, const int32_t *d_r, INT n_pos, INT n_neg, INT stride, INT denom,
                               int32_t *d_counts, float *d_resid_ent, float *d_resid_rel, float *d_loss, void *stream);
+int kge_transe_forward_counts_packed(const kge_model_desc *m, const float *d_ent, const float *d_rel, const int32_t *d_h,
+                                     const int32_t *d_t, const int32_t *d_r, const int32_t *d_pack, INT n_pos, INT n_neg, INT stride,
+                                     INT denom, int32_t *d_counts, float *d_loss, void *stream);
 int kge_transe_apply_counts(float *d_p, float *d_m, float *d_v, int32_t *d_counts, float *d_resid, int64_t rows, int32_t dim,
                             INT denom, int32_t adam, float lr, float beta1, float beta2, float eps, void *stream);
 int kge_transe_train_step_counts(const kge_model_desc *m, float *const d_p[2], float *const d_m[2], float *const d_v[2], const int32_t *d_h,
                                  const int32_t *d_t, const int32_t *d_r, INT n_pos, INT n_neg, INT stride, INT denom, int32_t *d_counts,
                                  float *const d_resid[2], int32_t sampler_shaped, int32_t adam, float lr, float beta1, float beta2, float eps,
                                  float *d_loss, void *stream);
+int kge_transe_train_step_counts_packed(const kge_model_desc *m, float *const d_p[2], float *const d_m[2], float *const d_v[2],
+                                        const int32_t *d_h, const int32_t *d_t, const int32_t *d_r, const int32_t *d_pack, INT n_pos,
+                                        INT n_neg, INT stride, INT denom, int32_t *d_counts, float *const d_resid[2],
+                                        int32_t sampler_shaped, int32_t adam, float lr, float beta1, float beta2, float eps, float *d_loss,
+                                        void *stream);
 int kge_transe_apply_counts_tables(const kge_model_desc *m, float *const d_p[2], float *const d_m[2], float *const d_v[2],
                                    int32_t *d_counts, float *const d_resid[2], INT denom, int32_t adam, float lr, float beta1,
                                    float beta2, float eps, void *stream);
diff --git a/openkeonspark_amd/Config.py b/openkeonspark_amd/Config.py
--- a/openkeonspark_amd/Config.py
+++ b/openkeonspark_amd/Config.py
@@ -234,6 +234,9 @@
         self._refresh_pointers()
         self._dist_ready = 0
         self._dev_batch = None
+        self._dev_pack = None
+        self._batch_pack = 0
+        self._prefetched_pack = 0
         self._dev_batch2 = None
         self._side_stream = None
         self._prefetched = None
@@ -448,14 +451,29 @@
             self._dev_batch = torch.zeros((2, 3, n), dtype=torch.int32, device=self.device)
         return self._dev_batch
 
+    def _pack_for(self, slot):
+        import torch
+        n_neg = self.negative_ent + self.negative_rel
+        if not (self.use_counts and not self.sparse_rows and not self.sparse_inplace and
+                self.batch_size * (3 + n_neg) >= self.counts_min_records * self.world_size):
+            return 0
+        words = int(self.lib.kge_emit_pack_words(self._n_local, self.negative_ent, self.negative_rel, self.hidden_size))
+        if words <= 0:
+            return 0
+        if self._dev_pack is None or self._dev_pack.shape[1] != words:
+            self._dev_pack = torch.zeros((2, words), dtype=torch.int32, device=self.device)
+        return self._dev_pack[slot].data_ptr()
+
     def sample_device(self, slot=0):
         stride = max(self._n_local, 1)
         buf = self._ensure_dev_batch(stride)[slot]
         nl = ctypes.c_int64(0)
-        _lib.check(self.lib.kge_sampling_device(buf[0].data_ptr(), buf[1].data_ptr(), buf[2].data_ptr(),
-                                                self.batch_size, self.negative_ent, self.negative_rel,
-                                                self._thread_lo, self._thread_hi, stride, ctypes.byref(nl),
-                                                self._stream()), self.lib)
+        pack = self._pack_for(slot)
+        _lib.check(self.lib.kge_sampling_device_packed(buf[0].data_ptr(), buf[1].data_ptr(), buf[2].data_ptr(), pack or None,
+                                                       self.batch_size, self.negative_ent, self.negative_rel,
+                                                       self._thread_lo, self._thread_hi, stride, ctypes.byref(nl),
+                                                       self._stream()), self.lib)
+        self._batch_pack = pack
         return buf, nl.value
 
     def _next_sampled_batch(self):
@@ -469,6 +487,7 @@
             dev, n_pos = self.sample_device(self._slot)
         else:
             dev, n_pos, ev = self._prefetched
+            self._batch_pack = self._prefetched_pack
             if ev is not None:
                 torch.cuda.current_stream().wait_event(ev)
         return dev, n_pos
@@ -478,10 +497,12 @@
         self._slot ^= 1
         buf = self._ensure_dev_batch(stride)[self._slot]
         nl = ctypes.c_int64(0)
-        _lib.check(self.lib.kge_sampling_attach(buf[0].data_ptr(), buf[1].data_ptr(), buf[2].data_ptr(), self.batch_size,
-                                                self.negative_ent, self.negative_rel, self._thread_lo, self._thread_hi, stride,
-                                                ctypes.byref(nl), self._stream()), self.lib)
+        pack = self._pack_for(self._slot)
+        _lib.check(self.lib.kge_sampling_attach_packed(buf[0].data_ptr(), buf[1].data_ptr(), buf[2].data_ptr(), pack or None,
+                                                       self.batch_size, self.negative_ent, self.negative_rel, self._thread_lo,
+                                                       self._thread_hi, stride, ctypes.byref(nl), self._stream()), self.lib)
         self._prefetched = (buf, nl.value, None)
+        self._prefetched_pack = pack
 
     def _flush_next_batch(self):
         _lib.check(self.lib.kge_sampling_flush(self._stream()), self.lib)
@@ -506,6 +527,7 @@
             ev = torch.cuda.Event()
             ev.record(self._side_stream)
         self._prefetched = (dev, n_pos, ev)
+        self._prefetched_pack = self._batch_pack
 
     def forward_backward(self, dev_batch, n_pos, stride, denom, sampler_shaped=False):
         fn = self.lib.kge_forward_backward_sampled if sampler_shaped else self.lib.kge_forward_backward
@@ -672,7 +694,9 @@
         if batch_h is None:
             dev, n_pos = self._next_sampled_batch() if self.prefetch_sampling else self.sample_device()
             stride = max(self._n_local, 1)
+            pack = self._batch_pack
         else:
+            pack = 0
             if self._dp:
                 raise KgeError("feeding a host batch is single-process only")
             host = np.stack([np.asarray(batch_h), np.asarray(batch_t), np.asarray(batch_r)]).astype(np.int32)
@@ -725,9 +749,9 @@
             one_call = not self._dp and bool(getattr(self, "fused_counts", True))
             try:
                 if one_call:
-                    self.step_counts(dev, n_pos, stride, denom, sampler_shaped=batch_h is None)
+                    self.step_counts(dev, n_pos, stride, denom, sampler_shaped=batch_h is None, pack=pack)
                 else:
-                    self.forward_counts(dev, n_pos, stride, denom, sampler_shaped=batch_h is None)
+                    self.forward_counts(dev, n_pos, stride, denom, sampler_shaped=batch_h is None, pack=pack)
             finally:
                 if ahead:
                     self._flush_next_batch()
@@ -1042,7 +1066,14 @@
         n = int(self._sparse_buf["n_rows"].item())
         return self._sparse_buf["rows"][:n], self._sparse_buf["row_counts"][:n]
 
-    def forward_counts(self, dev_batch, n_pos, stride, denom, sampler_shaped=False):
+    def forward_counts(self, dev_batch, n_pos, stride, denom, sampler_shaped=False, pack=0):
+        if sampler_shaped and pack:
+            _lib.check(self.lib.kge_transe_forward_counts_packed(
+                ctypes.byref(self._desc), self._tables[0].data_ptr(), self._tables[1].data_ptr(),
+                dev_batch[0].data_ptr(), dev_batch[1].data_ptr(), dev_batch[2].data_ptr(), pack, n_pos,
+                self.negative_ent + self.negative_rel, stride, denom, self._counts.data_ptr(),
+                self._loss.data_ptr(), self._stream()), self.lib)
+            return
         resid = (None, None) if sampler_shaped else (self._grads[0].data_ptr(), self._grads[1].data_ptr())
         _lib.check(self.lib.kge_transe_forward_counts(
             ctypes.byref(self._desc), self._tables[0].data_ptr(), self._tables[1].data_ptr(),
@@ -1050,11 +1081,12 @@
             self.negative_ent + self.negative_rel, stride, denom, self._counts.data_ptr(),
             resid[0], resid[1], self._loss.data_ptr(), self._stream()), self.lib)
 
-    def step_counts(self, dev_batch, n_pos, stride, denom, sampler_shaped=False):
+    def step_counts(self, dev_batch, n_pos, stride, denom, sampler_shaped=False, pack=0):
         lr = float(self._adam_lr_t()) if self._adam else float(self.alpha)
-        _lib.check(self.lib.kge_transe_train_step_counts(
+        _lib.check(self.lib.kge_transe_train_step_counts_packed(
             ctypes.byref(self._desc), self._tab_ptrs, self._adam_m_ptrs if self._adam else None, self._adam_v_ptrs if self._adam else None,
-            dev_batch[0].data_ptr(), dev_batch[1].data_ptr(), dev_batch[2].data_ptr(), n_pos, self.negative_ent + self.negative_rel,
+            dev_batch[0].data_ptr(), dev_batch[1].data_ptr(), dev_batch[2].data_ptr(), (pack if sampler_shaped else 0) or None, n_pos,
+            self.negative_ent + self.negative_rel,
             stride, denom, self._counts.data_ptr(), self._grad_ptrs, 1 if sampler_shaped else 0, 1 if self._adam else 0, lr,
             self.adam_beta1, self.adam_beta2, self.adam_epsilon, self._loss.data_ptr(), self._stream()), self.lib)
         if self._adam:
diff --git a/openkeonspark_amd/_lib.py b/openkeonspark_amd/_lib.py
--- a/openkeonspark_amd/_lib.py
+++ b/openkeonspark_amd/_lib.py
@@ -58,6 +58,10 @@
     L.kge_set_stream_states.argtypes = [vp, i64]
     L.kge_sampling_device.argtypes = [vp, vp, vp, i64, i64, i64, i64, i64, i64, ctypes.POINTER(i64), vp]
     L.kge_sampling_attach.argtypes = [vp, vp, vp, i64, i64, i64, i64, i64, i64, ctypes.POINTER(i64), vp]
+    L.kge_sampling_device_packed.argtypes = [vp, vp, vp, vp, i64, i64, i64, i64, i64, i64, ctypes.POINTER(i64), vp]
+    L.kge_sampling_attach_packed.argtypes = [vp, vp, vp, vp, i64, i64, i64, i64, i64, i64, ctypes.POINTER(i64), vp]
+    L.kge_emit_pack_words.argtypes = [i64, i64, i64, i64]
+    L.kge_emit_pack_words.restype = i64
     L.kge_sampling_flush.argtypes = [vp]
     L.kge_slice_positions.restype = i64
     L.kge_slice_positions.argtypes = [i64, i64, i64, ctypes.POINTER(i64)]
@@ -96,12 +100,15 @@
     L.kge_test_entity_ids.argtypes = [i64, i64, vp, vp]
     L.kge_transe_counts_supported.argtypes = [ctypes.POINTER(ModelDesc), i64]
     L.kge_transe_forward_counts.argtypes = [ctypes.POINTER(ModelDesc), vp, vp, vp, vp, vp, i64, i64, i64, i64, vp, vp, vp, vp, vp]
+    L.kge_transe_forward_counts_packed.argtypes = [ctypes.POINTER(ModelDesc), vp, vp, vp, vp, vp, vp, i64, i64, i64, i64, vp, vp, vp]
     L.kge_transe_apply_counts.argtypes = [vp, vp, vp, vp, vp, i64, i32, i64, i32, f32, f32, f32, f32, vp]
     L.kge_transe_deferred_groups.argtypes = [ctypes.POINTER(ctypes.c_int32)]
     L.kge_transe_step_scratch_read.argtypes = [ctypes.c_int, i64, i64, vp]
     L.kge_transe_apply_counts_tables.argtypes = [ctypes.POINTER(ModelDesc), vp, vp, vp, vp, vp, i64, i32, f32, f32, f32, f32, vp]
     L.kge_transe_train_step_counts.argtypes = [ctypes.POINTER(ModelDesc), vp, vp, vp, vp, vp, vp, i64, i64, i64, i64, vp, vp, i32, i32,
                                                f32, f32, f32, f32, vp, vp]
+    L.kge_transe_train_step_counts_packed.argtypes = [ctypes.POINTER(ModelDesc), vp, vp, vp, vp, vp, vp, vp, i64, i64, i64, i64, vp, vp,
+                                                      i32, i32, f32, f32, f32, f32, vp, vp]
     L.kge_transe_lazy_row_live.argtypes = [vp]
     L.kge_transe_record_dwords.restype = i64
     L.kge_transe_record_dwords.argtypes = [ctypes.POINTER(ModelDesc)]
diff --git a/openkeonspark_amd/csrc/abi.hip b/openkeonspark_amd/csrc/abi.hip
--- a/openkeonspark_amd/csrc/abi.hip
+++ b/openkeonspark_amd/csrc/abi.hip
@@ -118,6 +118,7 @@
     return "";
 }
 
+void transe_team_shape(int D, int &L, int &C);
 }
 
 using namespace kge;
@@ -227,6 +228,7 @@
     if (n == "counts_krel") { int k = 1; while (k * 2 <= value && k < 64) k *= 2; engine().counts_krel = k; return KGE_OK; }
     if (n == "inv_carry") { engine().inv_carry = value != 0; tables_written(); return KGE_OK; }
     if (n == "emit_rounds") { engine().emit_rounds = value != 0; return KGE_OK; }
+    if (n == "emit_pack") { engine().emit_pack = value != 0; return KGE_OK; }
     if (n == "float_records") { engine().float_records = value != 0; return KGE_OK; }
     if (n == "float_records_min") { engine().float_records_min = value; return KGE_OK; }
     if (n == "index_device_min") { engine().index_device_min = value; return KGE_OK; }
@@ -339,19 +341,40 @@
 
 int kge_sampling_attach(int32_t *d_h, int32_t *d_t, int32_t *d_r, INT batchSize, INT negRate, INT negRelRate,
                         INT thread_lo, INT thread_hi, INT out_stride, INT *n_local, void *stream) {
+    return kge_sampling_attach_packed(d_h, d_t, d_r, nullptr, batchSize, negRate, negRelRate, thread_lo, thread_hi, out_stride, n_local, stream);
+}
+
+int kge_sampling_attach_packed(int32_t *d_h, int32_t *d_t, int32_t *d_r, int32_t *d_pack, INT batchSize, INT negRate, INT negRelRate,
+                               INT thread_lo, INT thread_hi, INT out_stride, INT *n_local, void *stream) {
     int64_t nl = 0;
-    int rc = attach_sampler(d_h, d_t, d_r, batchSize, negRate, negRelRate, thread_lo, thread_hi, out_stride, &nl, (hipStream_t)stream);
+    int rc = attach_sampler(d_h, d_t, d_r, batchSize, negRate, negRelRate, thread_lo, thread_hi, out_stride, &nl, (hipStream_t)stream, d_pack);
     if (n_local) *n_local = nl;
     return rc;
 }
 
+INT kge_emit_pack_words(INT n_positions, INT negRate, INT negRelRate, INT dim) {
+    const KgIndex &ix = engine().index;
+    if (n_positions <= 0 || negRate < 0 || negRelRate < 0 || !emit_pack_shape(ix.ent_total, ix.rel_total, negRate, negRelRate)) return 0;
+    if (dim > 0) {
+        int L = 0, C = 0;
+        transe_team_shape((int)dim, L, C);
+        if (dim % 4 != 0 || L != 64 || C > 4) return 0;
+    }
+    return n_positions << sampler_kshift(negRate, negRelRate);
+}
+
 int kge_sampling_flush(void *stream) { return flush_attached_sampler((hipStream_t)stream); }
 
 int kge_sampling_device(int32_t *d_h, int32_t *d_t, int32_t *d_r, INT batchSize, INT negRate, INT negRelRate,
                         INT thread_lo, INT thread_hi, INT out_stride, INT *n_local, void *stream) {
+    return kge_sampling_device_packed(d_h, d_t, d_r, nullptr, batchSize, negRate, negRelRate, thread_lo, thread_hi, out_stride, n_local, stream);
+}
+
+int kge_sampling_device_packed(int32_t *d_h, int32_t *d_t, int32_t *d_r, int32_t *d_pack, INT batchSize, INT negRate, INT negRelRate,
+                               INT thread_lo, INT thread_hi, INT out_stride, INT *n_local, void *stream) {
     int64_t nl = 0;
     int rc = launch_sampler(d_h, d_t, d_r, batchSize, negRate, negRelRate, thread_lo, thread_hi, out_stride, &nl,
-                            (hipStream_t)stream);
+                            (hipStream_t)stream, d_pack);
     if (n_local) *n_local = nl;
     return rc;
 }
diff --git a/openkeonspark_amd/csrc/engine.hpp b/openkeonspark_amd/csrc/engine.hpp
--- a/openkeonspark_amd/csrc/engine.hpp
+++ b/openkeonspark_amd/csrc/engine.hpp
@@ -58,6 +58,7 @@
     int counts_krel = 4;
     int inv_carry = 1;
     int emit_rounds = 1;
+    int emit_pack = 1;
     int64_t inv_table_max_bytes = int64_t(256) << 20;
     int float_records = 1;
     int64_t float_records_min = 1 << 16;
@@ -94,7 +95,7 @@
 bool take_attached_sampler(SamplerArgs &a, unsigned &blocks, float share = 1.0f);
 int flush_attached_sampler(hipStream_t stream);
 int attach_sampler(int32_t *d_h, int32_t *d_t, int32_t *d_r, int64_t B, int64_t neg, int64_t negrel, int64_t thread_lo,
-                   int64_t thread_hi, int64_t out_stride, int64_t *n_local_out, hipStream_t stream);
+                   int64_t thread_hi, int64_t out_stride, int64_t *n_local_out, hipStream_t stream, int32_t *d_pack = nullptr);
 void set_error(const std::string &msg);
 int fail(int code, const std::string &msg);
 bool device_ok();
@@ -150,7 +151,13 @@
                                const int64_t *t, const int64_t *r);
 
 int launch_sampler(int32_t *d_h, int32_t *d_t, int32_t *d_r, int64_t B, int64_t neg, int64_t negrel, int64_t thread_lo,
-                   int64_t thread_hi, int64_t out_stride, int64_t *n_local, hipStream_t stream);
+                   int64_t thread_hi, int64_t out_stride, int64_t *n_local, hipStream_t stream, int32_t *d_pack = nullptr);
+inline int sampler_kshift(int64_t neg, int64_t negrel) { int k = 0; while ((int64_t(1) << k) < 1 + neg + negrel) k++; return k; }
+constexpr int kPackRowBits = 28;
+inline bool emit_pack_shape(int64_t ent_total, int64_t rel_total, int64_t neg, int64_t negrel) {
+    return engine().emit_pack && sampler_kshift(neg, negrel) <= 6 && neg + negrel >= 1 && ent_total < (int64_t(1) << kPackRowBits) &&
+           rel_total < (int64_t(1) << kPackRowBits);
+}
 int launch_widen(const int32_t *src3, int64_t *dst3_and_y, int64_t B, int64_t total, hipStream_t stream);
 int launch_forward_backward(const kge_model_desc &m, const float *const tables[4], const int32_t *d_h, const int32_t *d_t,
                             const int32_t *d_r, int64_t n_pos, int64_t n_neg, int64_t stride, int64_t denom,
diff --git a/openkeonspark_amd/csrc/models.hip b/openkeonspark_amd/csrc/models.hip
--- a/openkeonspark_amd/csrc/models.hip
+++ b/openkeonspark_amd/csrc/models.hip
@@ -398,7 +398,7 @@
 typedef float f32x4 __attribute__((ext_vector_type(4)));
 template <int V> struct IntC { static constexpr int value = V; };
 
-template <bool INV_TAB, bool REC2>
+template <bool INV_TAB, bool REC2, bool PACK = false>
 __device__ __forceinline__ void transe_emit_rounds_body(const FbArgs &a) {
     constexpr int L = 64, TEAMS = 256 / L;
     __shared__ float red[TEAMS];
@@ -422,6 +422,14 @@
         int my_code = 0, my_row = 0;
         float my_f = 0.f;
         bool bad = false;
+        if constexpr (PACK) {
+            if (lane < n_neg) {
+                const int w = a.neg_pack[(b << a.pack_shift) + lane + 1];
+                my_row = w & ((1 << kPackRowBits) - 1);
+                my_code = (w >> kPackRowBits) & 3;
+                bad = w < 0;
+            }
+        } else
         for (int k = lane; k < n_neg; k += L) {
             const long long j = b + (long long)(k + 1) * a.stride;
             const int nh = a.bh[j], nt = a.bt[j], nr = a.br[j];
@@ -470,7 +478,7 @@
         s16x2 Ah_lo = 0, Ah_hi = 0, At_lo = 0, At_hi = 0, Ar_lo = 0, Ar_hi = 0;
         int cnt = 0;
         for (int k0 = 0; k0 < n_neg; k0 += L) {
-            if (k0 > 0) {
+            if (!PACK && k0 > 0) {
                 const int my_k = k0 + lane;
                 my_code = 0; my_row = 0; my_f = 0.f;
                 if (my_k < n_neg) {
@@ -583,6 +591,9 @@
     if constexpr (L == 64 && Q == 1) transe_emit_rounds_body<INV_TAB, REC2>(a);
     else transe_emit_vec_body<L, Q, K, INV_TAB, REC2>(a);
 }
+
+template <bool INV_TAB, bool REC2>
+__global__ __launch_bounds__(256, 1) void transe_emit_pack_kernel(FbArgs a) { transe_emit_rounds_body<INV_TAB, REC2, true>(a); }
 
 template <int L, int Q, int K, int WPE, bool INV_TAB, bool REC2 = false>
 __global__ __launch_bounds__(256, WPE) void transe_emit_vec_v1_kernel(FbArgs a) { transe_emit_vec_body<L, Q, K, INV_TAB, REC2>(a); }
@@ -654,7 +665,18 @@
                 else hipLaunchKernelGGL((transe_emit_vec_v1_kernel<L, Q, 4, 1, false>), grid, block, 0, stream, a);
             }
         }
-        if (v1) {
+        bool packed = false;
+        if constexpr (L == 64 && Q == 1) {
+            if (!v1 && a.neg_pack && a.n_neg < L) {
+                packed = true;
+                if (a.rec2) {
+                    if (inv_tab) hipLaunchKernelGGL((transe_emit_pack_kernel<true, true>), grid, block, 0, stream, a);
+                    else hipLaunchKernelGGL((transe_emit_pack_kernel<false, true>), grid, block, 0, stream, a);
+                } else if (inv_tab) hipLaunchKernelGGL((transe_emit_pack_kernel<true, false>), grid, block, 0, stream, a);
+                else hipLaunchKernelGGL((transe_emit_pack_kernel<false, false>), grid, block, 0, stream, a);
+            }
+        }
+        if (v1 || packed) {
         } else if (a.rec2) {
             if (inv_tab) hipLaunchKernelGGL((transe_emit_vec_kernel<L, Q, 4, 1, true, true>), grid, block, 0, stream, a);
             else hipLaunchKernelGGL((transe_emit_vec_kernel<L, Q, 4, 1, false, true>), grid, block, 0, stream, a);
@@ -718,7 +740,7 @@
 int launch_transe_emit(const kge_model_desc &m, const float *ent, const float *rel, float *resid_ent, float *resid_rel,
                        const int32_t *d_h, const int32_t *d_t, const int32_t *d_r, int64_t n_pos, int64_t n_neg, int64_t stride,
                        int64_t denom, uint32_t *rec, int32_t *dst, int krel, float *d_loss, hipStream_t stream, bool track_deferred,
-                       uint8_t *rec2) {
+                       uint8_t *rec2, const int32_t *neg_pack) {
     Engine &e = engine();
     { int rc = ensure_loss_buffers(); if (rc) return rc; }
     int32_t *&defer_list = g_defer_list, *&defer_count = g_defer_count;
@@ -755,6 +777,10 @@
     a.rec = rec; a.rec2 = (m.ent_dim % 4 == 0) ? rec2 : nullptr; a.dst = dst; a.ent_total = (int)m.ent_total; a.rel_total = (int)m.rel_total; a.krel = 1;
     a.loss_limbs = track_deferred ? nullptr : e.loss_limbs;
     while (a.krel * 2 <= krel) a.krel *= 2;
+    if (neg_pack && e.emit_pack && !track_deferred && emit_pack_shape(m.ent_total, m.rel_total, n_neg, 0) &&
+        m.ent_total + (int64_t)a.krel * m.rel_total < (int64_t(1) << kPackRowBits)) {
+        a.neg_pack = neg_pack; a.pack_shift = sampler_kshift(n_neg, 0);
+    }
     if (!for_transe_team_shape(a.D, [&](auto t) { launch_emit<decltype(t)::L, decltype(t)::C>(a, d_loss, stream); }))
         return fail(KGE_ERR_UNSUPPORTED, "embedding dimension > 1024");
     return hip_check(hipGetLastError(), "transe emit launch");
diff --git a/openkeonspark_amd/csrc/models_dev.hpp b/openkeonspark_amd/csrc/models_dev.hpp
--- a/openkeonspark_amd/csrc/models_dev.hpp
+++ b/openkeonspark_amd/csrc/models_dev.hpp
@@ -33,6 +33,8 @@
     int32_t *skipped;
     int32_t *loss_limbs;
     int loss_blocks;
+    const int32_t *neg_pack;
+    int pack_shift;
 };
 
 int ensure_loss_buffers();
diff --git a/openkeonspark_amd/csrc/sampler.hip b/openkeonspark_amd/csrc/sampler.hip
--- a/openkeonspark_amd/csrc/sampler.hip
+++ b/openkeonspark_amd/csrc/sampler.hip
@@ -34,7 +34,7 @@
     }
 }
 
-static int build_sampler(int32_t *d_h, int32_t *d_t, int32_t *d_r, int64_t B, int64_t neg, int64_t negrel, int64_t thread_lo,
+static int build_sampler(int32_t *d_h, int32_t *d_t, int32_t *d_r, int32_t *d_pack, int64_t B, int64_t neg, int64_t negrel, int64_t thread_lo,
                          int64_t thread_hi, int64_t out_stride, int64_t *n_local_out, SamplerArgs &a, unsigned &blocks, bool &wide) {
     Engine &e = engine();
     int rc = ensure_device_index();
@@ -62,9 +62,9 @@
     a.neg = (int)neg; a.negrel = (int)negrel; a.bern = e.bern ? 1 : 0;
     a.pick_div = (unsigned long long)(a.new_batch > 0 ? a.new_batch : a.train_dup);
     a.pick_magic = ~0ull / a.pick_div;
-    int kshift = 0;
-    while ((1 << kshift) < 1 + neg + negrel) kshift++;
+    const int kshift = sampler_kshift(neg, negrel);
     a.kshift = kshift;
+    a.pack = emit_pack_shape(a.ent_total, a.rel_total, neg, negrel) ? d_pack : nullptr;
     a.streams_next = e.dev.streams_next; a.W = W; a.B = B;
     wide = kshift > 6;
     int64_t nb = n_local > 0 ? ((n_local << kshift) + 255) / 256 : 0;
@@ -104,12 +104,12 @@
 }
 
 int attach_sampler(int32_t *d_h, int32_t *d_t, int32_t *d_r, int64_t B, int64_t neg, int64_t negrel, int64_t thread_lo,
-                   int64_t thread_hi, int64_t out_stride, int64_t *n_local_out, hipStream_t stream) {
+                   int64_t thread_hi, int64_t out_stride, int64_t *n_local_out, hipStream_t stream, int32_t *d_pack) {
     Engine &e = engine();
     int rc = flush_attached_sampler(stream);
     if (rc) return rc;
     SamplerArgs a; unsigned blocks; bool wide;
-    if ((rc = build_sampler(d_h, d_t, d_r, B, neg, negrel, thread_lo, thread_hi, out_stride, n_local_out, a, blocks, wide))) return rc;
+    if ((rc = build_sampler(d_h, d_t, d_r, d_pack, B, neg, negrel, thread_lo, thread_hi, out_stride, n_local_out, a, blocks, wide))) return rc;
     if (blocks == 0) {
         hipLaunchKernelGGL(advance_streams_kernel, dim3((unsigned)((a.W + 63) / 64)), dim3(64), 0, stream, e.dev.streams,
                            (long long)a.W, (long long)B, (long long)a.per_thread, (unsigned long long)(1 + 2 * neg + negrel));
@@ -123,12 +123,12 @@
 }
 
 int launch_sampler(int32_t *d_h, int32_t *d_t, int32_t *d_r, int64_t B, int64_t neg, int64_t negrel, int64_t thread_lo,
-                   int64_t thread_hi, int64_t out_stride, int64_t *n_local_out, hipStream_t stream) {
+                   int64_t thread_hi, int64_t out_stride, int64_t *n_local_out, hipStream_t stream, int32_t *d_pack) {
     Engine &e = engine();
     int rc = flush_attached_sampler(stream);
     if (rc) return rc;
     SamplerArgs a; unsigned blocks; bool wide;
-    if ((rc = build_sampler(d_h, d_t, d_r, B, neg, negrel, thread_lo, thread_hi, out_stride, n_local_out, a, blocks, wide))) return rc;
+    if ((rc = build_sampler(d_h, d_t, d_r, d_pack, B, neg, negrel, thread_lo, thread_hi, out_stride, n_local_out, a, blocks, wide))) return rc;
     if (blocks > 0) {
         if (!wide) hipLaunchKernelGGL(sample_kernel, dim3(blocks), dim3(256), 0, stream, a);
         else hipLaunchKernelGGL(sample_kernel_wide, dim3(blocks), dim3(256), 0, stream, a);
diff --git a/openkeonspark_amd/csrc/sampler_dev.hpp b/openkeonspark_amd/csrc/sampler_dev.hpp
--- a/openkeonspark_amd/csrc/sampler_dev.hpp
+++ b/openkeonspark_amd/csrc/sampler_dev.hpp
@@ -23,6 +23,7 @@
     uint64_t *streams_next;
     long long W, B;
     int32_t *out_h, *out_t, *out_r;
+    int32_t *pack;
     long long per_thread;
     long long pos_lo;
     long long n_local;
@@ -213,6 +214,16 @@
             const long long o = b + (long long)k * a.out_stride;
             a.out_h[o] = oh; a.out_t[o] = ot; a.out_r[o] = orr;
         }
+        if (a.pack && g < total) {
+            int w = 0;
+            if (live && k >= 1) {
+                const NegClass nc = classify_negative<KGE_TRANSE>(tr.x, tr.y, tr.z, oh, ot, orr, 0);
+                const int code = !nc.same_h ? 0 : (!nc.same_t ? 1 : 2);
+                const int row = !nc.same_h ? oh : (!nc.same_t ? ot : orr);
+                w = row | (code << kPackRowBits) | (nc.fast ? 0 : (int)0x80000000u);
+            }
+            a.pack[g] = w;
+        }
     }
 }
 
diff --git a/openkeonspark_amd/csrc/transe_counts.hip b/openkeonspark_amd/csrc/transe_counts.hip
--- a/openkeonspark_amd/csrc/transe_counts.hip
+++ b/openkeonspark_amd/csrc/transe_counts.hip
@@ -15,7 +15,7 @@
 int launch_transe_emit(const kge_model_desc &m, const float *ent, const float *rel, float *resid_ent, float *resid_rel,
                        const int32_t *d_h, const int32_t *d_t, const int32_t *d_r, int64_t n_pos, int64_t n_neg, int64_t stride,
                        int64_t denom, uint32_t *rec, int32_t *dst, int krel, float *d_loss, hipStream_t stream, bool track_deferred,
-                       uint8_t *rec2 = nullptr);
+                       uint8_t *rec2 = nullptr, const int32_t *neg_pack = nullptr);
 
 int transe_deferred_groups(int32_t *out);
 
@@ -1514,7 +1514,8 @@
 
 static int forward_counts_impl(const kge_model_desc *m, const float *d_ent, const float *d_rel, const int32_t *d_h,
                                const int32_t *d_t, const int32_t *d_r, INT n_pos, INT n_neg, INT stride, INT denom,
-                               int32_t *d_counts, float *d_resid_ent, float *d_resid_rel, float *d_loss, void *stream_, FusedOpt *fo) {
+                               int32_t *d_counts, float *d_resid_ent, float *d_resid_rel, float *d_loss, void *stream_, FusedOpt *fo,
+                               const int32_t *d_pack = nullptr) {
     hipStream_t stream = (hipStream_t)stream_;
     if (!device_ok()) return fail(KGE_ERR_NO_DEVICE, "kge_transe_forward_counts: no usable HIP device");
     if (!m || !kge_transe_counts_supported(m, n_neg)) return fail(KGE_ERR_UNSUPPORTED, "sign-count path: TransE, dim <= 1024, 1..63 negatives");
@@ -1541,7 +1542,7 @@
                        (uint64_t)M * rd * 4 < (uint64_t(1) << 32) && rows2 < (1 << 30);
     uint8_t *rec2 = fused ? reinterpret_cast<uint8_t *>(g_c.rec + (size_t)3 * (size_t)n_pos * rd) : nullptr;
     rc = launch_transe_emit(*m, d_ent, d_rel, d_resid_ent, d_resid_rel, d_h, d_t, d_r, n_pos, n_neg, stride, denom, g_c.rec, g_c.dst,
-                            krel, d_loss, stream, d_resid_ent != nullptr && d_resid_rel != nullptr, rec2);
+                            krel, d_loss, stream, d_resid_ent != nullptr && d_resid_rel != nullptr, rec2, d_pack);
     if (rc) return rc;
     FuseArgs fold = FuseArgs();
     if (krel > 1) { fold.fold_E = (int)m->ent_total; fold.fold_R = (int)m->rel_total; }
@@ -1613,10 +1614,26 @@
                                stream_, nullptr);
 }
 
+int kge_transe_forward_counts_packed(const kge_model_desc *m, const float *d_ent, const float *d_rel, const int32_t *d_h,
+                                     const int32_t *d_t, const int32_t *d_r, const int32_t *d_pack, INT n_pos, INT n_neg, INT stride,
+                                     INT denom, int32_t *d_counts, float *d_loss, void *stream_) {
+    return forward_counts_impl(m, d_ent, d_rel, d_h, d_t, d_r, n_pos, n_neg, stride, denom, d_counts, nullptr, nullptr, d_loss, stream_,
+                               nullptr, d_pack);
+}
+
 int kge_transe_train_step_counts(const kge_model_desc *m, float *const d_p[2], float *const d_m[2], float *const d_v[2], const int32_t *d_h,
                                  const int32_t *d_t, const int32_t *d_r, INT n_pos, INT n_neg, INT stride, INT denom, int32_t *d_counts,
                                  float *const d_resid[2], int32_t sampler_shaped, int32_t adam, float lr, float beta1, float beta2, float eps,
                                  float *d_loss, void *stream_) {
+    return kge_transe_train_step_counts_packed(m, d_p, d_m, d_v, d_h, d_t, d_r, nullptr, n_pos, n_neg, stride, denom, d_counts, d_resid,
+                                               sampler_shaped, adam, lr, beta1, beta2, eps, d_loss, stream_);
+}
+
+int kge_transe_train_step_counts_packed(const kge_model_desc *m, float *const d_p[2], float *const d_m[2], float *const d_v[2],
+                                        const int32_t *d_h, const int32_t *d_t, const int32_t *d_r, const int32_t *d_pack, INT n_pos,
+                                        INT n_neg, INT stride, INT denom, int32_t *d_counts, float *const d_resid[2],
+                                        int32_t sampler_shaped, int32_t adam, float lr, float beta1, float beta2, float eps, float *d_loss,
+                                        void *stream_) {
     if (!m || !d_p || !d_p[0] || !d_p[1] || !d_counts || !d_resid || !d_resid[0] || !d_resid[1] || denom <= 0)
         return fail(KGE_ERR_BAD_ARG, "kge_transe_train_step_counts: bad arguments");
     if (adam && (!d_m || !d_v || !d_m[0] || !d_m[1] || !d_v[0] || !d_v[1]))
@@ -1627,7 +1644,7 @@
     fo.adam = adam; fo.lr = lr; fo.b1 = beta1; fo.b2 = beta2; fo.eps = eps;
     const bool fed = !sampler_shaped;
     int rc = forward_counts_impl(m, d_p[0], d_p[1], d_h, d_t, d_r, n_pos, n_neg, stride, denom, d_counts, fed ? d_resid[0] : nullptr,
-                                 fed ? d_resid[1] : nullptr, d_loss, stream_, &fo);
+                                 fed ? d_resid[1] : nullptr, d_loss, stream_, &fo, fed ? nullptr : d_pack);
     if (rc || fo.done) return rc;
     return kge_transe_apply_counts_range(m, d_p, d_m, d_v, d_counts, d_resid, 0, m->ent_total + m->rel_total, denom, adam, lr, beta1, beta2,
                                          eps, stream_);
```

Result: faster. 159.5 million (median of 6 runs) (+7.8%).
